# Team766/ros_vision

Measured on AMD Instinct MI355X. Metric: frames/sec + p50 per-frame latency, 1280x720 AprilTag detect at 1/2/4/8 MI355X, higher is better.
Workload: dtype u8

## Files before the change

ros_vision_amd/csrc/at_api.cpp:

```cpp
#include <hip/hip_runtime.h>

#include <algorithm>
#include <chrono>
#include <cmath>
#include <cstdio>
#include <cstdlib>
#include <cstring>
#include <map>
#include <string>
#include <thread>
#include <vector>

#include "../../include/at_api.h"
#include "at_common.h"
#include "at_gp.h"
#include "at_mjpg.h"
#include "at_mjpg_entropy.h"
#include "at_preview.h"
#include "at_rigcal.h"
#include "at_camcal.h"

namespace at {
hipError_t launch_tap_sizes(const uint8_t* thr, const uint32_t* par, const uint32_t* size, uint32_t* out, int Wd,
                            int Hd, hipStream_t st);
// ... 184 lines not shown
  int mj_ent_timed;
  at::JpgBufs jpg;
  size_t jpg_out_cap;
  uint32_t* h_jpg_total;
  uint8_t jpg_hdr[at::kJpgHeaderMax];
  size_t jpg_hdr_len;
  int jpg_hdr_q, jpg_hdr_s, jpg_hdr_w, jpg_hdr_h;
  uint64_t jpg_stats[2];
  hipEvent_t ev_jpg[2];
  at::GpParseBufs gp;
  at::GpBox* h_gp_out;
  uint32_t* h_gp_info;
  uint64_t gp_stats[4];
  hipEvent_t ev_gp[2];
  uint8_t* d_pv;
  uint64_t pv_stats[6];
  hipEvent_t ev_pv[2];
  FieldLaunch field;
  int field_on;
  int last_field;
  int field_timed;
  FpRecord* h_field;
  hipEvent_t ev_field[2];
  uint64_t field_ns;
};

static const char* knob(const char* name) {
#ifdef AT_EXPERIMENTS
  return getenv(name);
#else
  (void)name;
  return nullptr;
#endif
}
static int knob_int(const char* name, int dflt) {
  const char* v = knob(name);
  return v ? atoi(v) : dflt;
}

static int hip_fail(hipError_t e) {
  if (e != hipSuccess) {
    fprintf(stderr, "at_api: HIP error %s\n", hipGetErrorString(e));
    return AT_E_HIP;
  }
  return AT_OK;
}
#define HIPCHK(x)                          \
  do {                                     \
    hipError_t e_ = (x);                   \
    if (e_ != hipSuccess) return hip_fail(e_); \
  } while (0)

extern "C" {

int at_abi_version(void) { return AT_ABI_VERSION; }

const char* at_strerror(int code) {
  switch (code) {
    case AT_OK: return "ok";
    case AT_E_INVALID: return "invalid argument or unsupported frame geometry";
    case AT_E_HIP: return "HIP runtime error";
    case AT_E_CAPACITY: return "frame exceeded a fixed capacity";
    case AT_E_FAMILY: return "unknown tag family";
    case AT_E_NOMEM: return "out of memory";
    case AT_E_UNSUPPORTED: return "unsupported JPEG stream (not baseline 8-bit 4:4:4 / 4:2:2 / 4:2:0 / gray)";
    default: return "unknown error";
  }
}

int at_family_num_known(const char* family) {
  const FamilyInfo* f = find_family(family);
  return f ? f->ncodes : AT_E_FAMILY;
}

int at_family_entry(const char* family, int i, int* id, uint64_t* code) {
  const FamilyInfo* f = find_family(family);
  if (!f) return AT_E_FAMILY;
  if (i < 0 || i >= f->ncodes) return AT_E_INVALID;
  if (id) *id = f->codes[i].id;
  if (code) *code = f->codes[i].code;
  return AT_OK;
}

int at_config_default(at_config* cfg, int width, int height) {
  if (!cfg) return AT_E_INVALID;
  memset(cfg, 0, sizeof(*cfg));
  cfg->width = width;
  cfg->height = height;
  cfg->family = "tag36h11";
  cfg->quad_decimate = 2.0f;
  cfg->refine_edges = 1;
  cfg->decode_sharpening = 0.25;
  cfg->min_white_black_diff = 5;
  cfg->min_cluster_pixels = 5;
  cfg->max_nmaxima = 10;
  cfg->max_line_fit_mse = 10.0f;
  cfg->cos_critical_rad = cos(10.0 * M_PI / 180.0);
  cfg->device = 0;
  cfg->max_batch = 1;
  cfg->tag_size = 0.1651;
  return AT_OK;
}

void at_destroy(at_detector* d) {
  if (!d) return;
  (void)hipSetDevice(d->device);
  if (d->st) (void)hipStreamSynchronize(d->st);
  if (d->st2) (void)hipStreamSynchronize(d->st2);
  for (auto& kv : d->graphs) (void)hipGraphExecDestroy(kv.second);
  d->graphs.clear();
  for (auto& kv : d->split_graphs)
    for (auto* g : kv.second.seg) (void)hipGraphExecDestroy(g);
  d->split_graphs.clear();
  for (void* p : d->allocs) (void)hipFree(p);
  if (d->h_ftab) (void)hipHostFree(d->h_ftab);
  if (d->h_ctrl) (void)hipHostFree(d->h_ctrl);
  if (d->h_dets) (void)hipHostFree(d->h_dets);
  if (d->d_prims) (void)hipFree(d->d_prims);
  if (d->d_last) (void)hipFree(d->d_last);
  for (uint8_t* p : d->mj_host)
    if (p) (void)hipHostFree(p);
  for (hipEvent_t e : d->ev_mj)
    if (e) (void)hipEventDestroy(e);
  for (uint8_t* p : d->mj_ent_host)
    if (p) (void)hipHostFree(p);
  if (d->h_ent_info) (void)hipHostFree(d->h_ent_info);
  for (hipEvent_t e : d->ev_ent)
    if (e) (void)hipEventDestroy(e);
  for (hipEvent_t e : d->ev_jpg)
    if (e) (void)hipEventDestroy(e);
  if (d->h_jpg_total) (void)hipHostFree(d->h_jpg_total);
  for (hipEvent_t e : d->ev_gp)
    if (e) (void)hipEventDestroy(e);
  for (hipEvent_t e : d->ev_pv)
    if (e) (void)hipEventDestroy(e);
  if (d->d_pv) (void)hipFree(d->d_pv);
  for (hipEvent_t e : d->ev_field)
    if (e) (void)hipEventDestroy(e);
  if (d->h_field) (void)hipHostFree(d->h_field);
  if (d->h_gp_out) (void)hipHostFree(d->h_gp_out);
  if (d->h_gp_info) (void)hipHostFree(d->h_gp_info);
  if (d->ev_done) (void)hipEventDestroy(d->ev_done);
  if (d->ev_ext) (void)hipEventDestroy(d->ev_ext);
  for (int i = 0; i <= kNumStages; i++)
    if (d->ev_stage[i]) (void)hipEventDestroy(d->ev_stage[i]);
  if (d->kt.t0) (void)hipEventDestroy(d->kt.t0);
  if (d->kt.t1) (void)hipEventDestroy(d->kt.t1);
  if (d->ev_fork) (void)hipEventDestroy(d->ev_fork);
  if (d->ev_join) (void)hipEventDestroy(d->ev_join);
  if (d->st2) (void)hipStreamDestroy(d->st2);
  if (d->st) (void)hipStreamDestroy(d->st);
  delete d;
}

int at_create(const at_config* cfg, const at_camera* cam, at_detector** out) {
  if (!cfg || !cam || !out) return AT_E_INVALID;
  *out = nullptr;
  const FamilyInfo* fam = find_family(cfg->family);
  if (!fam || fam->ncodes > kMaxCodes) return AT_E_FAMILY;
  const int W = cfg->width, H = cfg->height;
  if (W <= 16 || H <= 16 || W % 8 || H % 8 || (long)W * H >= (1L << 22)) return AT_E_INVALID;
  if (cfg->quad_decimate != 2.0f || cfg->max_nmaxima != 10 || cfg->max_batch < 1 || cfg->max_batch > kMaxBatch)
    return AT_E_INVALID;
  if (2 * (W + H) > kSortCap) return AT_E_INVALID;
  int ndev = 0;
  if (hipGetDeviceCount(&ndev) != hipSuccess || ndev <= cfg->device) return AT_E_HIP;
  at_detector* d = new at_detector();
  d->cfg = *cfg;
  d->cfg.family = fam->name;
  d->cam = *cam;
  d->device = cfg->device;
  d->B = cfg->max_batch;
  d->mj_threads = 1;
  d->mj_subseq = at::kEntSubseqDefault;
  Geom& g = d->g;
  g.W = W; g.H = H; g.Wd = W / 2; g.Hd = H / 2;
  g.TW = g.Wd / 4; g.TH = g.Hd / 4;
  g.BW = g.Wd / 2; g.BH = g.Hd / 2;
  g.ctw = d->B < kWideBlobMaxBatch ? 32 : 64;
  if (knob("AT_CCL_TILE")) g.ctw = knob_int("AT_CCL_TILE", 64) == 32 ? 32 : 64;
  g.nlarge = g.ctw == 32 ? std::max(kNumLargeCls, std::min(kNumCls, knob_int("AT_NLARGE", kNumLargeCls)))
                        : kNumLargeCls;
  g.CTX = (g.Wd + g.ctw - 1) / g.ctw;
  g.CTY = (g.Hd + kCclTileH - 1) / kCclTileH;
  g.merge_cap = g.ctw == 64 ? std::min(kMergeCapMax, 80 * g.CTX * g.CTY) : 0;
  g.merge_lds = std::min(g.merge_cap * 12 + 8192, kMergeLdsMax);
  if (g.CTX * g.CTY > kMaxCclTiles) {
    at_destroy(d);
    return AT_E_INVALID;
  }
  g.cap_pts = 4 * (g.Wd - 2) * (g.Hd - 2);
  g.BTX = (g.Wd - 2 + 63) / 64;
  g.BTY = (g.Hd - 2 + 4 * kBndRows - 1) / (4 * kBndRows);
  g.ntb = g.BTX * g.BTY;
  g.bnd_region = kBndPts;
  g.bnd_region = std::max(kBndStage, std::min(kBndPts, knob_int("AT_BND_REGION", kBndPts)));
  if (g.ntb > kMaxTilesPerFrame) {
    at_destroy(d);
    return AT_E_INVALID;
  }
  g.min_cluster = (uint32_t)std::max(24, cfg->min_cluster_pixels);
  g.max_cluster = (uint32_t)(2 * (W + H));
  g.min_tag_width = std::max(3, (fam->d + 2) / 2);
  Params& p = d->prm;
  p.min_white_black_diff = cfg->min_white_black_diff;
  p.max_line_fit_mse = cfg->max_line_fit_mse;
  p.cos_critical_rad = cfg->cos_critical_rad;
  p.decode_sharpening = cfg->decode_sharpening;
  p.refine_edges = cfg->refine_edges;
  p.fx = cam->fx; p.fy = cam->fy; p.cx = cam->cx; p.cy = cam->cy;
  p.k1 = cam->k1; p.k2 = cam->k2; p.p1 = cam->p1; p.p2 = cam->p2; p.k3 = cam->k3;
  p.diag_stop = knob_int("AT_DIAG_BLOB_STOP", 0);
  p.probe = knob_int("AT_PHASE_PROBE", 0);
  p.taps = 0;
  p.wide_blob = knob_int("AT_WIDE_BLOB", 0);
  p.pipe_stop = knob_int("AT_DIAG_PIPE_STOP", 0);
  p.lblob_wg = knob("AT_LBLOB_WG") ? std::max(16, knob_int("AT_LBLOB_WG", 0)) : 0;
  p.sblob_wg = knob("AT_SBLOB_WG") ? std::max(16, knob_int("AT_SBLOB_WG", 0)) : 0;
  p.dec_wg = knob("AT_DEC_WG") ? std::max(16, knob_int("AT_DEC_WG", 0)) : 0;
  p.dec_lpq = knob_int("AT_DEC_LPQ", 0) == 64 ? 64 : 0;
  p.fam = family_desc(*fam);
  d->use_graphs = !knob_int("AT_NO_GRAPH", 0);
  if (!(cfg->tag_size >= 0) || !std::isfinite(cfg->tag_size)) {
    at_destroy(d);
    return AT_E_INVALID;
  }
  p.tag_size = cfg->tag_size;

  auto fail = [&](int code) {
    at_destroy(d);
    return code;
  };
  if (hipSetDevice(d->device) != hipSuccess) return fail(AT_E_HIP);
  if (hipStreamCreateWithFlags(&d->st, hipStreamNonBlocking) != hipSuccess) return fail(AT_E_HIP);
  if (hipEventCreateWithFlags(&d->ev_done, hipEventDisableTiming) != hipSuccess) return fail(AT_E_HIP);
  if (hipEventCreateWithFlags(&d->ev_ext, hipEventDisableTiming) != hipSuccess) return fail(AT_E_HIP);
  const bool fork = d->B < kWideBlobMaxBatch && !knob_int("AT_NO_FORK", 0);
  if (fork && hipStreamCreateWithFlags(&d->st2, hipStreamNonBlocking) != hipSuccess) return fail(AT_E_HIP);
  if (hipEventCreateWithFlags(&d->ev_fork, hipEventDisableTiming) != hipSuccess) return fail(AT_E_HIP);
  if (hipEventCreateWithFlags(&d->ev_join, hipEventDisableTiming) != hipSuccess) return fail(AT_E_HIP);
  d->kt.stage = -1;
  d->kt.split = nullptr;
  d->kt.ctx = nullptr;
  if (hipEventCreateWithFlags(&d->kt.t0, kTimingEventFlags) != hipSuccess ||
      hipEventCreateWithFlags(&d->kt.t1, kTimingEventFlags) != hipSuccess)
    return fail(AT_E_HIP);
  int ncu = 0;
  (void)hipDeviceGetAttribute(&ncu, hipDeviceAttributeMultiprocessorCount, d->device);
  int wclk = 0;
  (void)hipDeviceGetAttribute(&wclk, hipDeviceAttributeWallClockRate, d->device);
  d->wclk_khz = wclk > 0 ? (double)wclk : 100000.0;
  d->nblobwg = std::max(64, ncu * 2);
  if (knob("AT_BLOB_WG")) d->nblobwg = std::max(16, knob_int("AT_BLOB_WG", 0));

  const size_t B = (size_t)d->B;
  const size_t npix = (size_t)W * H, nd = (size_t)g.Wd * g.Hd, nt = (size_t)g.TW * g.TH * 2;
  bool oom = false;
  auto dalloc = [&](size_t bytes) -> void* {
    void* ptr = nullptr;
    if (hipMalloc(&ptr, std::max<size_t>(bytes, 256)) != hipSuccess) {
      oom = true;
      return nullptr;
    }
    d->allocs.push_back(ptr);
    return ptr;
  };
  d->in_stride = (npix * 3 + 255) & ~(size_t)255;
  d->d_in = (uint8_t*)dalloc(B * d->in_stride);
  DevBufs& b = d->d;
  b.gray = (uint8_t*)dalloc(B * npix);
  b.dec = (uint8_t*)dalloc(B * nd);
  b.mm = (uint8_t*)dalloc(B * nt);
  b.thr = (uint8_t*)dalloc(B * nd);
  b.par = (uint32_t*)dalloc(B * nd * 4);
  b.lroot = (uint32_t*)dalloc(B * (size_t)g.CTX * g.CTY * kCclTileNodesMax * 4);
  b.nlroot = (uint32_t*)dalloc(B * (size_t)g.CTX * g.CTY * 4);
  b.lcnt = (uint32_t*)dalloc(B * (size_t)g.CTX * g.CTY * kCclTileNodesMax * 4);
  b.cdesc = (uint32_t*)dalloc(B * (size_t)g.CTX * g.CTY * CclDesc::kWords * 4);
  b.size = (uint32_t*)dalloc(B * nd * 4);
  const size_t ntb = (size_t)g.ntb;
  b.pts = (uint64_t*)dalloc(B * ntb * (size_t)g.bnd_region * 8);
  b.tcnt = (uint32_t*)dalloc(B * ntb * 4);
  b.tent = (uint32_t*)dalloc(B * ntb * 4);
  b.grp = (uint32_t*)dalloc(B * g.cap_pts * 4);
  b.keys = (uint64_t*)dalloc(B * g.cap_pts * 8);
  b.pent_key = (uint64_t*)dalloc(B * ntb * kLdsPairSlots * 8);
  b.pent_cnt = (uint32_t*)dalloc(B * ntb * kLdsPairSlots * 4);
  b.povf_key = (uint64_t*)dalloc(B * kPairEntCap * 8);
  b.povf_cnt = (uint32_t*)dalloc(B * kPairEntCap * 4);
  b.ht_key = (uint64_t*)dalloc(B * kHashSlots * 8);
  b.ht_cnt = (uint32_t*)dalloc(B * kHashSlots * 4);
  b.ht_rank = (uint32_t*)dalloc(B * kHashSlots * 4);
  b.ht_off = (uint32_t*)dalloc(B * kHashSlots * 4);
  b.ht_cur = (uint32_t*)dalloc(B * kHashSlots * 4);
  b.pair_cnt = (uint32_t*)dalloc(B * kMaxPairs * 4);
  b.pair_off = (uint32_t*)dalloc(B * kMaxPairs * 4);
  b.pair_sel = (uint32_t*)dalloc(B * kMaxPairs * 4);
  b.wcap = (uint32_t)(B * kMaxPairs);
  b.work = (uint32_t*)dalloc((size_t)kNumCls * B * kMaxPairs * 4);
  b.probe = (uint64_t*)dalloc(kProbeWords * 8);
  b.dets = (DevDetection*)dalloc(B * kMaxDets * sizeof(DevDetection));
  b.det_work = (uint32_t*)dalloc(B * kMaxDets * 4);
  b.quads = (QuadRecord*)dalloc(B * kMaxPairs * sizeof(QuadRecord));
  b.qpend = (QuadPend*)dalloc(B * kMaxPairs * sizeof(QuadPend));
  d->kstamp_word = (kCtlPerFrame * B + kCtlScalars + 1) & ~(size_t)1;
  d->ctrl_words = d->kstamp_word + 5;
  d->d_ctrl = (uint32_t*)dalloc(((d->ctrl_words * 4 + 15) / 16) * 16);
  b.npts = d->d_ctrl + kCtlNpts * B;
  b.npairs = d->d_ctrl + kCtlNpairs * B;
  b.ndets = d->d_ctrl + kCtlNdets * B;
  b.nquads = d->d_ctrl + kCtlNquads * B;
  b.status = d->d_ctrl + kCtlStatus * B;
  b.npent = d->d_ctrl + kCtlNpent * B;
  b.qc_words = (uint32_t)(B * kQcStride);
  b.nqcand = (uint32_t*)dalloc((size_t)b.qc_words * 4);
  b.ccl_ovf = d->d_ctrl + kCtlCclOvf * B;
  b.nlr_tot = d->d_ctrl + kCtlNlr * B;
  uint32_t* sc = d->d_ctrl + kCtlPerFrame * B;
  b.workhead = sc + kCtlWorkhead;
  b.qhead = sc + kCtlQhead;
  b.workhead_small = sc + kCtlWorkheadSmall;
  b.workhead_mid = sc + kCtlWorkheadMid;
  b.blob_pts = sc + kCtlBlobPts;
  b.ncls = sc + kCtlNcls;
  b.det_head = sc + kCtlDetHead;
  b.dec_done = sc + kCtlDecDone;
  b.kt_stage = -1;
  b.kstamp = reinterpret_cast<uint64_t*>(d->d_ctrl + d->kstamp_word);
  b.kgrid = d->d_ctrl + d->kstamp_word + 4;
  b.kwg_cap = (uint32_t)(B * 1024 + 4096);
  b.kwg = (uint64_t*)dalloc((size_t)b.kwg_cap * 2 * 8);
  b.qcand_cap = (uint32_t)(B * kQuadCandPerFrame);
  b.qcand = (QuadCand*)dalloc((size_t)b.qcand_cap * sizeof(QuadCand));
  b.s_pk = (uint64_t*)dalloc((size_t)2 * d->nblobwg * (kSortCap / 2) * 8);
  b.rsamp = (double*)dalloc(decode_scratch_doubles(d->nblobwg, d->B, g.ctw == 64) * 8);
  if (oom) return fail(AT_E_NOMEM);
  if (prepare_kernels(g) != hipSuccess) return fail(AT_E_HIP);
  if (hipHostMalloc((void**)&d->h_ftab, B * sizeof(void*), hipHostMallocMapped | hipHostMallocCoherent) != hipSuccess)
    return fail(AT_E_NOMEM);
  if (hipHostGetDevicePointer((void**)&b.frames, (void*)d->h_ftab, 0) != hipSuccess) return fail(AT_E_HIP);
  d->res_idx.assign(B * kMaxDets, 0);
  d->res_n.assign(B, 0);
  d->res_base.assign(B, nullptr);
  d->res_ovf.resize(B);
  if (hipHostMalloc((void**)&d->h_ctrl, d->ctrl_words * 4, hipHostMallocMapped) != hipSuccess) return fail(AT_E_NOMEM);
  if (hipHostMalloc((void**)&d->h_dets, B * kDetPoolPerFrame * sizeof(DevDetection), hipHostMallocMapped) != hipSuccess)
    return fail(AT_E_NOMEM);
  if (hipHostGetDevicePointer((void**)&b.hdets, d->h_dets, 0) != hipSuccess ||
      hipHostGetDevicePointer((void**)&b.hctrl, d->h_ctrl, 0) != hipSuccess)
    return fail(AT_E_HIP);
  b.ctrl = d->d_ctrl;
  b.ctrl_words = (uint32_t)d->ctrl_words;
  {
    std::vector<uint64_t> codes(fam->ncodes);
    std::vector<int32_t> ids(fam->ncodes);
    for (int i = 0; i < fam->ncodes; i++) {
      codes[i] = fam->codes[i].code;
      ids[i] = fam->codes[i].id;
    }
    uint64_t* dc = (uint64_t*)dalloc(codes.size() * 8);
    int32_t* di = (int32_t*)dalloc(ids.size() * 4);
    if (oom) return fail(AT_E_NOMEM);
    if (hipMemcpy(dc, codes.data(), codes.size() * 8, hipMemcpyHostToDevice) != hipSuccess ||
        hipMemcpy(di, ids.data(), ids.size() * 4, hipMemcpyHostToDevice) != hipSuccess)
      return fail(AT_E_HIP);
    b.book_code = dc;
    b.book_id = di;
  }
  if (hipMemsetAsync(b.size, 0, B * nd * 4, d->st) != hipSuccess) return fail(AT_E_HIP);
  if (hipStreamSynchronize(d->st) != hipSuccess) return fail(AT_E_HIP);
  *out = d;
  return AT_OK;
}

}

static bool seg_intersect(const double* a0, const double* a1, const double* b0, const double* b1) {
  const double ux = a1[0] - a0[0], uy = a1[1] - a0[1];
  const double vx = b1[0] - b0[0], vy = b1[1] - b0[1];
  const double den = ux * vy - uy * vx;
  if (fabs(den) < 1e-12) return false;
  const double t = ((b0[0] - a0[0]) * vy - (b0[1] - a0[1]) * vx) / den;
  const double w = ((b0[0] - a0[0]) * uy - (b0[1] - a0[1]) * ux) / den;
  return t >= 0 && t <= 1 && w >= 0 && w <= 1;
}
static bool poly_contains(const double poly[4][2], const double* pt) {
  bool inside = false;
  for (int i = 0, j = 3; i < 4; j = i++) {
    if (((poly[i][1] > pt[1]) != (poly[j][1] > pt[1])) &&
        (pt[0] < (poly[j][0] - poly[i][0]) * (pt[1] - poly[i][1]) / (poly[j][1] - poly[i][1]) + poly[i][0]))
      inside = !inside;
  }
  return inside;
}
static bool poly_overlap(const double a[4][2], const double b[4][2]) {
  for (int i = 0; i < 4; i++)
    for (int j = 0; j < 4; j++)
      if (seg_intersect(a[i], a[(i + 1) & 3], b[j], b[(j + 1) & 3])) return true;
  return poly_contains(a, b[0]) || poly_contains(b, a[0]);
}
static int prefer_smaller(int pref, double q0, double q1) {
  if (pref) return pref;
  if (q0 < q1) return -1;
  if (q1 < q0) return 1;
  return 0;
}

static void write_detection(const DevDetection& v, at_detection* o) {
  o->id = v.id;
  o->hamming = v.hamming;
  o->decision_margin = v.decision_margin;
  memcpy(o->H, v.H, sizeof(o->H));
  memcpy(o->c, v.c, sizeof(o->c));
  memcpy(o->p, v.p, sizeof(o->p));
}

static int host_tail(const DevDetection* cand, int* idx, int ncand, at_detection* out, int cap) {
  std::stable_sort(idx, idx + ncand, [&](int a, int b) { return cand[a].blob_rank < cand[b].blob_rank; });
  int n = ncand;
  for (int i0 = 0; i0 < n; i0++) {
    for (int i1 = i0 + 1; i1 < n; i1++) {
      const DevDetection& a = cand[idx[i0]];
      const DevDetection& b = cand[idx[i1]];
      if (a.id != b.id) continue;
      if (!poly_overlap(a.p, b.p)) continue;
      int pref = 0;
      pref = prefer_smaller(pref, a.hamming, b.hamming);
      pref = prefer_smaller(pref, -a.decision_margin, -b.decision_margin);
      for (int k = 0; k < 3; k++) pref = prefer_smaller(pref, a.H[k], b.H[k]);
      if (pref < 0) {
        if (i1 < n - 1) idx[i1] = idx[n - 1];
        n--;
        i1--;
      } else {
        if (i0 < n - 1) idx[i0] = idx[n - 1];
        n--;
        i0--;
        break;
      }
    }
  }
  std::stable_sort(idx, idx + n, [&](int a, int b) { return cand[a].id < cand[b].id; });
  for (int i = 0; i < n && i < cap; i++) write_detection(cand[idx[i]], out + i);
  return n;
}

static hipError_t record_sequence(at_detector* d, int nframes, int fmt, hipStream_t st, hipEvent_t* ev,
                                  const KernelTimer* kt) {
  hipError_t e;
  DevBufs b = d->d;
  b.kt_stage = kt ? kt->stage : -1;
  FieldLaunch fl = d->field;
  fl.ev[0] = ev ? d->ev_field[0] : nullptr;
  fl.ev[1] = ev ? d->ev_field[1] : nullptr;
  if ((e = launch_pipeline(b, d->g, d->prm, nframes, fmt, d->nblobwg, st, ev, d->st2, d->ev_fork, d->ev_join, kt,
                           d->field_on ? &fl : nullptr)))
    return e;
  if (d->prm.tag_size > 0) return hipSuccess;
  return hipMemcpyAsync(d->h_ctrl, d->d_ctrl, d->ctrl_words * 4, hipMemcpyDeviceToHost, st);
}

static hipError_t split_capture(void* ctx, int ) {
  at_detector* d = (at_detector*)ctx;
  hipGraph_t g = nullptr;
  hipError_t e = hipStreamEndCapture(d->st, &g);
  if (e != hipSuccess) return e;
  d->cap_segs.push_back(g);
  return hipStreamBeginCapture(d->st, hipStreamCaptureModeThreadLocal);
}

static hipError_t instantiate(hipGraph_t g, hipGraphExec_t* exec) {
  const hipError_t e = hipGraphInstantiate(exec, g, nullptr, nullptr, 0);
  (void)hipGraphDestroy(g);
  return e;
}

static int enqueue_split(at_detector* d, int nframes, int fmt) {
  hipStream_t st = d->st;
  const int key = (nframes * 4 + fmt) * 32 + d->kt.stage;
  auto it = d->split_graphs.find(key);
  if (it == d->split_graphs.end()) {
    d->cap_segs.clear();
    KernelTimer kt = d->kt;
    kt.split = split_capture;
    kt.ctx = d;
    HIPCHK(hipStreamBeginCapture(st, hipStreamCaptureModeThreadLocal));
    hipError_t rec = record_sequence(d, nframes, fmt, st, nullptr, &kt);
    hipGraph_t last = nullptr;
    const hipError_t end = hipStreamEndCapture(st, &last);
    if (last) d->cap_segs.push_back(last);
    if (rec == hipSuccess && end == hipSuccess && d->cap_segs.size() != 3) rec = hipErrorInvalidValue;
    if (rec != hipSuccess || end != hipSuccess) {
      for (auto* g : d->cap_segs) (void)hipGraphDestroy(g);
      d->cap_segs.clear();
      HIPCHK(rec);
      HIPCHK(end);
    }
    at_detector::SplitGraphs sg{};
    hipError_t inst = hipSuccess;
    for (int i = 0; i < 3; i++) {
      const hipError_t r = instantiate(d->cap_segs[i], &sg.seg[i]);
      if (r != hipSuccess && inst == hipSuccess) inst = r;
    }
    d->cap_segs.clear();
    if (inst != hipSuccess) {
      for (auto* g : sg.seg)
        if (g) (void)hipGraphExecDestroy(g);
      HIPCHK(inst);
    }
    it = d->split_graphs.emplace(key, sg).first;
  }
  HIPCHK(hipGraphLaunch(it->second.seg[0], st));
  HIPCHK(hipEventRecord(d->kt.t0, st));
  HIPCHK(hipGraphLaunch(it->second.seg[1], st));
  HIPCHK(hipEventRecord(d->kt.t1, st));
  HIPCHK(hipGraphLaunch(it->second.seg[2], st));
  return AT_OK;
}

static int enqueue(at_detector* d, int nframes, int fmt) {
  hipStream_t st = d->st;
  const bool timed = d->kt.stage >= 0;
  const bool timed_on_fork = timed && d->st2 && (d->kt.stage == 8 || d->kt.stage == 9);
  if (d->profiling || !d->use_graphs || timed_on_fork) {
    HIPCHK(record_sequence(d, nframes, fmt, st, d->profiling ? d->ev_stage : nullptr, timed ? &d->kt : nullptr));
  } else if (timed) {
    const int rc = enqueue_split(d, nframes, fmt);
    if (rc != AT_OK) return rc;
  } else {
    const int key = nframes * 4 + fmt;
    auto it = d->graphs.find(key);
    if (it == d->graphs.end()) {
      hipGraph_t graph = nullptr;
      HIPCHK(hipStreamBeginCapture(st, hipStreamCaptureModeThreadLocal));
      const hipError_t rec = record_sequence(d, nframes, fmt, st, nullptr, nullptr);
      const hipError_t end = hipStreamEndCapture(st, &graph);
      HIPCHK(rec);
      HIPCHK(end);
      hipGraphExec_t exec = nullptr;
      HIPCHK(instantiate(graph, &exec));
      it = d->graphs.emplace(key, exec).first;
    }
    HIPCHK(hipGraphLaunch(it->second, st));
  }
  HIPCHK(hipEventRecord(d->ev_done, st));
  d->last_nframes = nframes;
  d->last_fmt = fmt;
  d->last_gray = fmt == AT_FMT_BGR8 || d->prm.taps;
  d->last_sizes = d->g.ctw == 32 || d->prm.taps;
  d->last_gp = d->prm.gp_c && fmt == AT_FMT_BGR8;
  d->last_mj_color = 0;
  d->mj_ent_batch = 0;
  d->last_field = d->field_on && d->prm.tag_size > 0;
  d->field_timed = d->last_field && d->profiling;
  d->pending = 1;
  return AT_OK;
}

static double now_us() {
  return std::chrono::duration<double, std::micro>(std::chrono::steady_clock::now().time_since_epoch()).count();
}

static int collect(at_detector* d, at_detection* out, int cap_per_frame, int* n_per_frame) {
  if (!d->pending) return AT_E_INVALID;
  const double t0 = now_us();
  HIPCHK(hipEventSynchronize(d->ev_done));
  const double t1 = now_us();
  d->host_wait_us += t1 - t0;
  d->pending = 0;
  if (d->profiling) {
    for (int i = 0; i < kNumStages; i++) {
      float ms = 0;
      HIPCHK(hipEventElapsedTime(&ms, d->ev_stage[i], d->ev_stage[i + 1]));
      d->stage_ms[i] += ms;
    }
    d->stage_batches++;
  }
  if (d->mj_timed) {
    float ms = 0;
    HIPCHK(hipEventElapsedTime(&ms, d->ev_mj[0], d->ev_mj[1]));
    d->mj_stats[4] = (uint64_t)((double)ms * 1e6);
    if (d->mj_timed == 2) {
      HIPCHK(hipEventElapsedTime(&ms, d->ev_mj[1], d->ev_mj[2]));
      d->mj_stats[5] = (uint64_t)((double)ms * 1e6);
    }
    d->mj_timed = 0;
  }
  d->field_ns = 0;
  if (d->field_timed) {
    float ms = 0;
    HIPCHK(hipEventElapsedTime(&ms, d->ev_field[0], d->ev_field[1]));
    d->field_ns = (uint64_t)((double)ms * 1e6);
    d->field_timed = 0;
  }
  if (d->mj_ent_timed) {
    float ms = 0;
    HIPCHK(hipEventElapsedTime(&ms, d->ev_ent[0], d->ev_ent[1]));
    d->mj_stats[6] = (uint64_t)((double)ms * 1e6);
    d->mj_ent_timed = 0;
  }
  if (d->mj_ent_batch) {
    uint32_t most = 0;
    for (int f = 0; f < d->last_nframes; f++) most = std::max(most, d->h_ent_info[(size_t)f * at::kEntInfoWords + 1]);
    d->mj_stats[8] = most;
  }
  if (d->kt.stage >= 0) {
    float ms = 0;
// ... 1811 lines not shown
```

ros_vision_amd/csrc/at_common.h:

```cpp
#pragma once

#include <hip/hip_runtime.h>
#include <stdint.h>

#include "at_detmath.h"
#include "at_fieldpose.h"
#include "at_rigpose.h"
#include "at_preview.h"

namespace at {

template <int TW>
struct CclTile {
  static constexpr int W = TW, H = 32;
  static constexpr int BW = TW / 2, BH = H / 2;
  static constexpr int NT = BW * BH;
  static constexpr int NODES = 3 * NT;
  static constexpr int ROW_NODES = 3 * BW;
};
constexpr int kCclTileH = 32;
constexpr int kCclTileNodesMax = CclTile<64>::NODES;
constexpr int kHashSlots = 4096;
constexpr int kHashBits = 12;
constexpr int kPairEntCap = 65536;
constexpr int kBndRows = 4;
constexpr int kBndPts = 64 * 4 * kBndRows * 4;
constexpr int kBndStage = 2048;
constexpr int kLdsPairSlots = 512;
constexpr uint32_t kTileNarrow = 0x80000000u;
constexpr int kMaxTilesPerFrame = 1024;
constexpr int kMaxCclTiles = 1024;
struct CclDesc {
  static constexpr int Tthr = 0, Bthr = 16, Lthr = 32, Rthr = 40;
  static constexpr int TsF = 48, TsL = 64, TsR = 80, BsF = 96, BsL = 112, BsR = 128;
  static constexpr int LsF = 144, LsL = 152, RsF = 160, RsR = 168;
  static constexpr int kWords = 176;
};
constexpr int kMergeCapMax = 15360;
constexpr int kMergeLdsMax = kMergeCapMax * 10;
constexpr int kMaxPairs = 4096;
constexpr int kSortCap = 8192;
constexpr int kBlobThreads = 256;
constexpr int kWideBlobMaxBatch = 8;
constexpr int kSmallBlob = 512;
constexpr int kNMaxima = 10;
constexpr int kMaxRefineSamples = 1536;
#ifndef AT_LDS_REFINE
#define AT_LDS_REFINE 256
#endif
constexpr int kLdsRefine = AT_LDS_REFINE;
constexpr int kDecodeGridPerBlobWg = 8;
inline int decode_grid(int nblobwg, int B) {
  const int hi = nblobwg * kDecodeGridPerBlobWg, want = 64 * B;
  return nblobwg * 2 > (want < hi ? want : hi) ? nblobwg * 2 : (want < hi ? want : hi);
}
constexpr int kDecRowLanes = 16;
constexpr int kRowRefine = 64;
inline size_t decode_scratch_doubles(int nblobwg, int B, bool packed) {
  const size_t one = 2 * (size_t)(kMaxRefineSamples - kLdsRefine);
  const size_t rows = (64 / kDecRowLanes) * 2 * (size_t)(kMaxRefineSamples - kRowRefine);
  return (size_t)decode_grid(nblobwg, B) * (packed && rows > one ? rows : one);
}

constexpr int kNumStages = 12;
constexpr const char* kStageNames[kNumStages] = {"k_pre",   "k_thr_ccl", "k_ccl_merge", "k_ccl_roots",
                                                 "k_boundary", "k_pairs", "k_group",     "k_extents",
                                                 "k_blob_small", "k_blob", "k_decode",   "k_pose"};

constexpr int kNumCls = 7;
constexpr int kNumLargeCls = 3;

constexpr uint32_t kStatusPairsOverflow = 1u;
constexpr uint32_t kStatusHashFull = 2u;
constexpr uint32_t kStatusDetsOverflow = 4u;
constexpr uint32_t kStatusPointsOverflow = 8u;
constexpr uint32_t kStatusQuadsOverflow = 16u;
constexpr uint32_t kStatusPairsCapped = 32u;
constexpr int kMaxBatch = 256;
constexpr int kQcStride = 32;
constexpr int kQuadCandPerFrame = kMaxPairs;
constexpr int kMaxDets = kQuadCandPerFrame;
constexpr int kDetPoolPerFrame = 128;
constexpr int kMaxCodes = 1024;
constexpr int kMaxFamilyBits = 64;

struct FamilyDesc {
  int nbits;
  int width_at_border;
  int total_width;
  int reversed_border;
  int ncodes;
  int8_t bitx[kMaxFamilyBits], bity[kMaxFamilyBits];
};

struct Geom {
  int W, H, Wd, Hd;
  int TW, TH;
  int BW, BH;
  int CTX, CTY;
  int ctw;
  int merge_cap;
  int merge_lds;
  int nlarge;
  int bnd_region;
  int cap_pts;
  int BTX, BTY, ntb;
  uint32_t min_cluster;
  uint32_t max_cluster;
  int min_tag_width;
};

struct Params {
  int min_white_black_diff;
  float max_line_fit_mse;
  double cos_critical_rad;
  double decode_sharpening;
  int refine_edges;
  double fx, fy, cx, cy, k1, k2, p1, p2, k3;
  int diag_stop;
  double tag_size;
  int probe;
  int taps;
  int wide_blob;
  int pipe_stop;
  int lblob_wg;
  int sblob_wg;
  int dec_wg;
  int dec_lpq;
  FamilyDesc fam;
  int gp_w, gp_h, gp_c;
};
constexpr int kProbeWords = 256;

#ifdef AT_EXPERIMENTS
#define AT_DIAG_STOP(prm, n) ((prm).diag_stop == (n))
#define AT_PIPE_STOP(prm) ((prm).pipe_stop)
#define AT_PROBE_ON(prm) ((prm).probe != 0)
#define AT_DIAG_ANY(prm) ((prm).diag_stop != 0)
#else
#define AT_DIAG_STOP(prm, n) false
#define AT_PIPE_STOP(prm) 0
#define AT_PROBE_ON(prm) false
#define AT_DIAG_ANY(prm) false
#endif

struct KernelTimer {
  int stage;
  hipEvent_t t0, t1;
  hipError_t (*split)(void* ctx, int which);
  void* ctx;
};

struct DevDetection {
  int32_t id;
  int16_t hamming;
  uint16_t frame;
  float decision_margin;
  int32_t blob_rank;
  double H[9];
  double c[2];
  double p[4][2];
  double pose_R[9];
  double pose_t[3];
  double pose_err[2];
};

struct QuadCand {
  uint32_t frame, rank;
  float p[4][2];
};

struct QuadRecord {
  uint32_t blob_index, valid, accepted;
  uint16_t indices[4];
  float corners[4][2];
};

struct Moments {
  int32_t Mx, My, W;
  int64_t Mxx, Myy, Mxy;
  int32_t N;
};

struct QuadPend {
  float fit[4][4];
  uint32_t blob_index, valid;
  uint16_t indices[4];
};
static_assert(sizeof(QuadPend) == 80, "QuadPend: 80 B per kept blob");


struct JpgBufs {
  int16_t* coef;
  const uint32_t* tab;
  uint32_t* blen;
  uint32_t* bits;
  size_t row_words;
  uint32_t* row_raw;
  uint32_t* row_len;
  uint8_t* out;
  uint32_t* total;
};

struct FieldBufs {
  FpLayout lay;
  FpRecord* out;
  FpRecord* hout;
};
struct FieldLaunch {
  FieldBufs b;
  hipEvent_t ev[2];
};

struct RigCamView {
  const DevDetection* dets;
  const uint32_t* ndets;
  RigCam cam;
};
struct RigBufs {
  RigCamView view[kRigMaxCams];
  FpLayout lay;
  RigRecord* out;
  RigRecord* hout;
  double tag_size;
  int n_cams;
};

struct DevBufs {
  const uint8_t* const* frames;
  uint8_t* gray;
  uint8_t* dec;
  uint8_t* mm;
  uint8_t* thr;
  uint32_t* par;
  uint32_t* lroot;
  uint32_t* nlroot;
  uint32_t* lcnt;
  uint32_t* cdesc;
  uint32_t* ccl_ovf;
  uint32_t* nlr_tot;
  uint32_t* size;
  uint64_t* pts;
  uint32_t* tcnt;
  uint32_t* tent;
  uint32_t* grp;
  uint64_t* keys;
  uint64_t* pent_key;
  uint32_t* pent_cnt;
  uint64_t* povf_key;
  uint32_t* povf_cnt;
  uint32_t* npent;
  uint64_t* ht_key;
  uint32_t* ht_cnt;
  uint32_t* ht_rank;
  uint32_t* ht_off;
  uint32_t* ht_cur;
  uint32_t* pair_cnt;
  uint32_t* pair_off;
  uint32_t* pair_sel;
  uint32_t* work;
  uint32_t wcap;
  DevDetection* dets;
  uint32_t* det_work;
  uint32_t* det_head;
  uint32_t* dec_done;
  DevDetection* hdets;
  uint32_t* hctrl;
  uint32_t* ctrl;
  uint32_t ctrl_words;
  QuadRecord* quads;
  QuadPend* qpend;
  uint32_t* npts;
  uint32_t* npairs;
  uint32_t* ndets;
  uint32_t* nquads;
  uint32_t* status;
  uint32_t* ncls;
  uint32_t* workhead;
  uint64_t* probe;
  uint32_t* blob_pts;
  uint32_t* workhead_small;
  uint32_t* workhead_mid;
  uint32_t* nqcand;
  uint32_t qc_words;
  uint32_t* qhead;
  QuadCand* qcand;
  uint32_t qcand_cap;
  double* rsamp;
  const uint64_t* book_code;
  const int32_t* book_id;
  float* gp_out;
  int32_t kt_stage;
  uint64_t* kstamp;
  uint32_t* kgrid;
  uint64_t* kwg;
  uint32_t kwg_cap;
  uint64_t* s_pk;
};

}
```

ros_vision_amd/csrc/at_kernels.hip:

```cpp
#include <limits>
#include <hip/hip_runtime.h>

#include <float.h>
#include <math.h>
#include <stdint.h>

#include "at_common.h"
#include "at_gp.h"
#include "at_mjpg.h"
#include "at_mjpg_entropy.h"
#include "at_pose.h"
#include "at_rigcal.h"
#include "at_camcal.h"


namespace at {

__device__ __forceinline__ uint32_t lane_id() { return __lane_id(); }
__device__ __attribute__((noinline)) float det_atan2f_call(float y, float x) { return det_atan2f(y, x); }

__device__ __forceinline__ uint64_t mix_hash(uint64_t k) {
  return (k * 0x9E3779B97F4A7C15ull) >> (64 - kHashBits);
}

__device__ __forceinline__ int dx_of(int dxy) { return dxy == 3 ? -1 : (dxy == 2 ? 0 : 1); }
__device__ __forceinline__ int dy_of(int dxy) { return dxy == 0 ? 0 : 1; }

template <int CTRL, int ROW_MASK, typename T>
__device__ __forceinline__ T dpp_move(T v, T old) {
  static_assert(sizeof(T) == 4 || sizeof(T) == 8, "dpp_move: 32- or 64-bit values");
  if constexpr (sizeof(T) == 4) {
    return __builtin_bit_cast(T, __builtin_amdgcn_update_dpp(__builtin_bit_cast(int, old), __builtin_bit_cast(int, v),
                                                             CTRL, ROW_MASK, 0xf, false));
  } else {
    const uint64_t u = __builtin_bit_cast(uint64_t, v), o = __builtin_bit_cast(uint64_t, old);
    const uint32_t lo = (uint32_t)__builtin_amdgcn_update_dpp((int)(uint32_t)o, (int)(uint32_t)u, CTRL, ROW_MASK, 0xf, false);
    const uint32_t hi = (uint32_t)__builtin_amdgcn_update_dpp((int)(uint32_t)(o >> 32), (int)(uint32_t)(u >> 32), CTRL,
                                                              ROW_MASK, 0xf, false);
    return __builtin_bit_cast(T, (uint64_t)lo | ((uint64_t)hi << 32));
  }
}

template <typename T, typename Op>
__device__ __forceinline__ T wave_incl_scan(T x, Op op, T id) {
  x = op(x, dpp_move<0x111, 0xf>(x, id));
  x = op(x, dpp_move<0x112, 0xf>(x, id));
  x = op(x, dpp_move<0x114, 0xf>(x, id));
  x = op(x, dpp_move<0x118, 0xf>(x, id));
  x = op(x, dpp_move<0x142, 0xa>(x, id));
  x = op(x, dpp_move<0x143, 0xc>(x, id));
  return x;
}

__device__ __forceinline__ uint32_t wave_shr1(uint32_t v, uint32_t fill) {
  return (uint32_t)__builtin_amdgcn_update_dpp((int)fill, (int)v, 0x138, 0xf, 0xf, false);
}

__device__ __forceinline__ uint32_t lanes_below(uint64_t mask) {
  return __builtin_amdgcn_mbcnt_hi((uint32_t)(mask >> 32), __builtin_amdgcn_mbcnt_lo((uint32_t)mask, 0u));
}

__device__ __forceinline__ void wave_sync() {
  __builtin_amdgcn_fence(__ATOMIC_RELEASE, "wavefront");
  __builtin_amdgcn_wave_barrier();
  __builtin_amdgcn_fence(__ATOMIC_ACQUIRE, "wavefront");
}

__device__ __forceinline__ uint32_t wave_read_next(uint32_t v) {
  return (uint32_t)__builtin_amdgcn_update_dpp(0, (int)v, 0x130, 0xf, 0xf, false);
}

template <typename T>
__device__ __forceinline__ T wave_read(T v, int l) {
  if constexpr (sizeof(T) == 4) {
    return __builtin_bit_cast(T, __builtin_amdgcn_readlane(__builtin_bit_cast(int, v), l));
  } else {
    const uint64_t u = __builtin_bit_cast(uint64_t, v);
    const uint32_t lo = (uint32_t)__builtin_amdgcn_readlane((int)(uint32_t)u, l);
    const uint32_t hi = (uint32_t)__builtin_amdgcn_readlane((int)(uint32_t)(u >> 32), l);
    return __builtin_bit_cast(T, (uint64_t)lo | ((uint64_t)hi << 32));
  }
}

struct MinOp {
  template <typename T> __device__ T operator()(T a, T c) const { return a < c ? a : c; }
  template <typename T> __device__ static T identity() { return std::numeric_limits<T>::max(); }
};
struct MaxOp {
  template <typename T> __device__ T operator()(T a, T c) const { return a > c ? a : c; }
  template <typename T> __device__ static T identity() { return std::numeric_limits<T>::lowest(); }
};
struct AddOp {
  template <typename T> __device__ T operator()(T a, T c) const { return a + c; }
  template <typename T> __device__ static T identity() { return T(0); }
};

__device__ __forceinline__ uint32_t run_len(uint64_t same_mask, uint32_t lane) {
  if (lane == 63) return 1;
  const uint64_t rest = ~(same_mask >> (lane + 1));
  return 1 + (uint32_t)__builtin_ctzll(rest);
}

template <typename T, typename Op>
__device__ T wave_reduce(T v, Op op) {
  return wave_read(wave_incl_scan(v, op, Op::template identity<T>()), 63);
}

template <typename T, typename Op>
__device__ T block_reduce(T v, Op op, T* s_tmp , int NW) {
  v = wave_reduce(v, op);
  const int w = threadIdx.x >> 6;
  __syncthreads();
  if (lane_id() == 0) s_tmp[w] = v;
  __syncthreads();
  T r = s_tmp[0];
  for (int i = 1; i < NW; i++) r = op(r, s_tmp[i]);
  return r;
}

template <typename T>
__device__ T block_incl_scan(T v, T* s_tmp, T* total, int NW) {
  const uint32_t lane = lane_id();
  v = wave_incl_scan(v, AddOp(), T(0));
  const int w = threadIdx.x >> 6;
  __syncthreads();
  if (lane == 63) s_tmp[w] = v;
  __syncthreads();
  T base = 0, tot = 0;
  for (int i = 0; i < NW; i++) {
    if (i < w) base = base + s_tmp[i];
    tot = tot + s_tmp[i];
  }
  *total = tot;
  return base + v;
}


#ifndef AT_XCD_PRE
#define AT_XCD_PRE 1
#endif
#ifndef AT_XCD_THR
#define AT_XCD_THR 1
#endif
#ifndef AT_XCD_BND
#define AT_XCD_BND 0
#endif
#ifndef AT_XCD_GRP
#define AT_XCD_GRP 0
#endif
struct TileIdx {
  int x, y, z;
};
__device__ __forceinline__ uint32_t udiv24(uint32_t a, uint32_t d) {
  uint32_t q = (uint32_t)((float)a * __builtin_amdgcn_rcpf((float)d));
  int32_t r = (int32_t)(a - q * d);
#pragma unroll
  for (int k = 0; k < 2; k++) {
    if (r < 0) { q--; r += (int32_t)d; }
    if (r >= (int32_t)d) { q++; r -= (int32_t)d; }
  }
  return q;
}
template <int MODE>
__device__ __forceinline__ TileIdx xcd_block() {
  if constexpr (MODE == 0) return TileIdx{(int)blockIdx.x, (int)blockIdx.y, (int)blockIdx.z};
  const uint32_t gx = gridDim.x, gxy = gridDim.x * gridDim.y, n = gxy * gridDim.z;
  const uint32_t lid = blockIdx.x + gx * blockIdx.y + gxy * blockIdx.z;
  uint32_t t;
  if constexpr (MODE == 1) {
    const uint32_t q = n >> 3, r = n & 7, xcd = lid & 7;
    t = xcd * q + min(xcd, r) + (lid >> 3);
  } else {
    const uint32_t rows = gridDim.y * gridDim.z, n8 = (rows & ~7u) * gx;
    if (lid < n8) {
      const uint32_t k = lid >> 3, j = udiv24(k, gx);
      t = ((j << 3) + (lid & 7)) * gx + (k - j * gx);
    } else {
      t = lid;
    }
  }
  const uint32_t z = udiv24(t, gxy), rem = t - z * gxy, y = udiv24(rem, gx);
  return TileIdx{(int)(rem - y * gx), (int)y, (int)z};
}

__device__ __forceinline__ uint32_t kt_wg_id() {
  return blockIdx.x + gridDim.x * (blockIdx.y + gridDim.y * blockIdx.z);
}
__device__ __forceinline__ void kt_begin(const DevBufs& b, int stage) {
  if (b.kt_stage != stage || threadIdx.x != 0 || threadIdx.y != 0) return;
  const uint32_t id = kt_wg_id();
  if (id == 0) *b.kgrid = gridDim.x * gridDim.y * gridDim.z;
  if (id < b.kwg_cap) b.kwg[id] = wall_clock64();
}
__device__ __forceinline__ void kt_end(const DevBufs& b, int stage) {
  if (b.kt_stage != stage) return;
  const uint32_t id = kt_wg_id();
  if (id < b.kwg_cap) b.kwg[b.kwg_cap + id] = wall_clock64();
}
constexpr int kKtSpanWgs = 32;
__global__ __launch_bounds__(256) void k_kt_span(DevBufs b) {
  const uint32_t n = min(*b.kgrid, b.kwg_cap);
  uint64_t mn = ~0ull, mx = 0;
  for (uint32_t i = blockIdx.x * 256 + threadIdx.x; i < n; i += kKtSpanWgs * 256) {
    mn = min(mn, b.kwg[i]);
    mx = max(mx, b.kwg[b.kwg_cap + i]);
  }
  mn = wave_reduce(mn, MinOp());
  mx = wave_reduce(mx, MaxOp());
  if (lane_id() == 0 && mx) {
    atomicMax((unsigned long long*)&b.kstamp[0], (unsigned long long)~mn);
    atomicMax((unsigned long long*)&b.kstamp[1], (unsigned long long)mx);
  }
}

__constant__ float c_filter[7] = {0.01110899634659290314f, 0.13533528149127960205f, 0.60653066635131835938f,
                                  1.00000000000000000000f, 0.60653066635131835938f, 0.13533528149127960205f,
                                  0.01110899634659290314f};

template <int FMT>
__device__ __forceinline__ void load_y8(const uint8_t* in, int W, int row, int x, uint32_t (&y)[8]) {
  if (FMT == 0) {
    const uint4 v = *reinterpret_cast<const uint4*>(in + ((size_t)row * W + x) * 2);
    const uint32_t w[4] = {v.x, v.y, v.z, v.w};
#pragma unroll
    for (int k = 0; k < 4; k++) {
      y[2 * k] = w[k] & 0xff;
      y[2 * k + 1] = (w[k] >> 16) & 0xff;
    }
  } else if (FMT == 1) {
    const uint8_t* p = in + ((size_t)row * W + x) * 3;
    const uint2 v0 = *reinterpret_cast<const uint2*>(p);
    const uint2 v1 = *reinterpret_cast<const uint2*>(p + 8);
    const uint2 v2 = *reinterpret_cast<const uint2*>(p + 16);
    uint8_t bytes[24];
    *reinterpret_cast<uint2*>(bytes) = v0;
    *reinterpret_cast<uint2*>(bytes + 8) = v1;
    *reinterpret_cast<uint2*>(bytes + 16) = v2;
#pragma unroll
    for (int k = 0; k < 8; k++) {
      const int bb = bytes[3 * k], gg = bytes[3 * k + 1], rr = bytes[3 * k + 2];
      y[k] = (uint32_t)((269484 * rr + 528482 * gg + 102760 * bb + (1 << 19) + (16 << 20)) >> 20);
    }
  } else {
    const uint2 v = *reinterpret_cast<const uint2*>(in + (size_t)row * W + x);
#pragma unroll
    for (int k = 0; k < 4; k++) {
      y[k] = (v.x >> (8 * k)) & 0xff;
      y[4 + k] = (v.y >> (8 * k)) & 0xff;
    }
  }
}

template <int FMT>
__global__ __launch_bounds__(256) void k_pre(DevBufs b, Geom g, int wgray) {
  const TileIdx bi = xcd_block<AT_XCD_PRE>();
  const int f = bi.z;
  const int tx = bi.x * 64 + threadIdx.x;
  const int ty = bi.y * 4 + threadIdx.y;
  if (blockIdx.x == 0 && blockIdx.y == 0 && blockIdx.z == 0) {
    for (uint32_t w = threadIdx.y * 64 + threadIdx.x; w < b.ctrl_words; w += 256) b.ctrl[w] = 0;
    for (uint32_t w = threadIdx.y * 64 + threadIdx.x; w < b.qc_words; w += 256) b.nqcand[w] = 0;
  }
  if (tx >= g.TW || ty >= g.TH) return;
  const uint8_t* in = b.frames[f];
  uint8_t* gray = b.gray + (size_t)f * g.W * g.H;
  uint8_t* dec = b.dec + (size_t)f * g.Wd * g.Hd;
  uint32_t mn = 255, mx = 0;
  const int x0 = tx * 8;
#pragma unroll
  for (int r = 0; r < 8; r++) {
    const int row = ty * 8 + r;
    uint32_t y[8];
    load_y8<FMT>(in, g.W, row, x0, y);
    if (FMT == 1 || wgray) {
      uint2 gw;
      gw.x = y[0] | (y[1] << 8) | (y[2] << 16) | (y[3] << 24);
      gw.y = y[4] | (y[5] << 8) | (y[6] << 16) | (y[7] << 24);
      *reinterpret_cast<uint2*>(gray + (size_t)row * g.W + x0) = gw;
    }
    if ((r & 1) == 0) {
      const uint32_t d = y[0] | (y[2] << 8) | (y[4] << 16) | (y[6] << 24);
      *reinterpret_cast<uint32_t*>(dec + (size_t)(row >> 1) * g.Wd + (x0 >> 1)) = d;
#pragma unroll
      for (int k = 0; k < 8; k += 2) {
        mn = min(mn, y[k]);
        mx = max(mx, y[k]);
      }
    }
  }
  uint8_t* mm = b.mm + (size_t)f * g.TW * g.TH * 2;
  *reinterpret_cast<uint16_t*>(mm + 2 * ((size_t)ty * g.TW + tx)) = (uint16_t)(mn | (mx << 8));
}

__device__ __forceinline__ uint32_t node_F(const Geom& g, int BY, int BX) { return (uint32_t)(BY * 3 * g.BW + BX); }
__device__ __forceinline__ uint32_t node_L(const Geom& g, int BY, int BX) {
  return (uint32_t)(BY * 3 * g.BW + g.BW + 2 * BX);
}
__device__ __forceinline__ uint32_t node_pixel(int BW, int Wd, uint32_t n) {
  const uint32_t by = n / (uint32_t)(3 * BW), r = n - by * (uint32_t)(3 * BW);
  return r < (uint32_t)BW ? 2 * by * (uint32_t)Wd + 2 * r : (2 * by + 1) * (uint32_t)Wd + (r - (uint32_t)BW);
}

__device__ __forceinline__ uint32_t lds_load(uint32_t* p) {
  return __hip_atomic_load(p, __ATOMIC_RELAXED, __HIP_MEMORY_SCOPE_WORKGROUP);
}
__device__ __forceinline__ uint32_t lds_find(uint32_t* par, uint32_t n) {
  uint32_t p = lds_load(par + n);
  while (p != n) {
    const uint32_t gp = lds_load(par + p);
    if (gp != p) atomicMin(&par[n], gp);
    n = p;
    p = gp;
  }
  return n;
}

__device__ __forceinline__ void lds_union(uint32_t* par, uint32_t a, uint32_t b) {
  while (true) {
    a = lds_find(par, a);
    b = lds_find(par, b);
    if (a == b) return;
    if (a < b) {
      const uint32_t old = atomicMin(&par[b], a);
      if (old == b) return;
      b = old;
    } else {
      const uint32_t old = atomicMin(&par[a], b);
      if (old == a) return;
      a = old;
    }
  }
}

template <int TW>
__device__ __forceinline__ uint32_t slot_of(int ty, int tx, int type) {
  using T = CclTile<TW>;
  return (uint32_t)(ty * T::ROW_NODES + (type == 0 ? tx : T::BW + 2 * tx + (type - 1)));
}

template <int TW>
struct BorderRoles {
  static constexpr int Top = 5 * CclTile<TW>::BW, Left = 3 * CclTile<TW>::BH, Right = CclTile<TW>::BH - 1;
  static constexpr int NT = (Top + Left + Right + 63) / 64 * 64;
};

constexpr uint32_t kKeptBit = 0x80000000u;
constexpr uint32_t kListBit = 0x40000000u;
constexpr uint32_t kTouchBit = 0x80000000u;

#ifndef AT_THR_SGPRS
#define AT_THR_SGPRS 80
#endif
template <int TWD, int PRE>
__device__ __forceinline__ void thr_ccl_tile(const DevBufs& b, const Geom& g, const Params& prm, const TileIdx bi) {
  using CT = CclTile<TWD>;
  constexpr int NT = CT::NT;
  constexpr int kCclTileW = CT::W, kCclBW = CT::BW, kCclTileNodes = CT::NODES;
  constexpr int kTW = kCclTileW / 4, kTH = kCclTileH / 4;
  constexpr int kHR = kCclTileH + 1, kHC = kCclTileW + 2;
  const int f = bi.z;
  const int tid = threadIdx.x;
  const int y0 = bi.y * kCclTileH, x0 = bi.x * kCclTileW;
  const uint8_t* dec = b.dec + (size_t)f * g.Wd * g.Hd;
  const uint8_t* mm = b.mm + (size_t)f * g.TW * g.TH * 2;
  uint8_t* thr = b.thr + (size_t)f * g.Wd * g.Hd;

  __shared__ uint8_t s_umn[kTH + 3][kTW + 4], s_umx[kTH + 3][kTW + 4];
  __shared__ uint8_t s_fmn[kTH + 1][kTW + 2], s_fmx[kTH + 1][kTW + 2];
  __shared__ __attribute__((aligned(4))) uint8_t s_t[kHR][kHC + 2];
  __shared__ uint32_t s_par[kCclTileNodes];
  __shared__ uint32_t s_cnt[kCclTileNodes];
  __shared__ uint32_t s_nlr;
// ... 1748 lines not shown
}


__device__ void redistort(const Params& p, double* x, double* y) {
  const double xP = (*x - p.cx) / p.fx, yP = (*y - p.cy) / p.fy;
  const double rSq = xP * xP + yP * yP;
  const double lin = 1 + p.k1 * rSq + p.k2 * rSq * rSq + p.k3 * rSq * rSq * rSq;
  const double xPP = xP * lin + 2 * p.p1 * xP * yP + p.p2 * (rSq + 2 * xP * xP);
  const double yPP = yP * lin + p.p1 * (rSq + 2 * yP * yP) + 2 * p.p2 * xP * yP;
  *x = xPP * p.fx + p.cx;
  *y = yPP * p.fy + p.cy;
}

__device__ void undistort(const Params& p, double* u, double* v) {
  const double xPP = (*u - p.cx) / p.fx, yPP = (*v - p.cy) / p.fy;
  double xP = xPP, yP = yPP;
  const double x0 = xP, y0 = yP;
  double prev_x, prev_y;
  int it = 0;
  do {
    prev_x = xP;
    prev_y = yP;
    const double rSq = xP * xP + yP * yP;
    const double rad = 1 + (p.k1 * rSq) + (p.k2 * rSq * rSq) + (p.k3 * rSq * rSq * rSq);
    const double rinv = 1 / rad;
    const double tdx = 2 * p.p1 * xP * yP + p.p2 * (rSq + p.k3 * rSq * rSq * rSq);
    const double tdy = p.p1 * (rSq + 2 * yP * yP) + 2 * p.p2 * xP * yP;
    xP = (x0 - tdx) * rinv;
    yP = (y0 - tdy) * rinv;
    if (it > 100) break;
    it++;
  } while (fabs(xP - prev_x) > 1e-6 || fabs(yP - prev_y) > 1e-6);
  *u = xP * p.fx + p.cx;
  *v = yP * p.fy + p.cy;
}

__device__ void hproject(const double* H, double x, double y, double* ox, double* oy) {
  const double xx = H[0] * x + H[1] * y + H[2];
  const double yy = H[3] * x + H[4] * y + H[5];
  const double zz = H[6] * x + H[7] * y + H[8];
  *ox = xx / zz;
  *oy = yy / zz;
}

__device__ int homography_wave(const float (*qc)[2], double* A, double* H) {
  const int lane = (int)lane_id();
  for (int e = lane; e < 72; e += 64) {
    const int row = e / 9, col = e % 9, i = row >> 1;
    const double c0 = (i == 0 || i == 3) ? -1 : 1, c1 = (i == 0 || i == 1) ? -1 : 1;
    const double c2 = qc[i][0], c3 = qc[i][1];
    const int k = (row & 1) ? col - 3 : col;
    const double cz = (row & 1) ? c3 : c2;
    double v = 0;
    if (k == 0) v = c0;
    else if (k == 1) v = c1;
    else if (k == 2) v = 1;
    if (col == 6) v = -c0 * cz;
    else if (col == 7) v = -c1 * cz;
    else if (col == 8) v = cz;
    A[e] = v;
  }
  team_sync<64>();
  for (int col = 0; col < 8; col++) {
    double v = -1.0;
    int row = 64;
    if (lane < 8 - col) {
      row = col + lane;
      v = fabs(A[row * 9 + col]);
      if (!(v > 0.0)) { v = -1.0; row = 64; }
    }
#pragma unroll
    for (int d = 1; d < 8; d <<= 1) {
      const double ov = __shfl_xor(v, d);
      const int orow = __shfl_xor(row, d);
      if (ov > v || (ov == v && orow < row)) { v = ov; row = orow; }
    }
    v = __shfl(v, 0);
    row = __shfl(row, 0);
    if (!(v >= 1e-10)) return -1;
    if (row != col && lane <= 8 - col) {
      const int i = col + lane;
      const double t = A[col * 9 + i];
      A[col * 9 + i] = A[row * 9 + i];
      A[row * 9 + i] = t;
    }
    team_sync<64>();
    const int nc = 8 - col;
    if (lane < (7 - col) * nc) {
      const int i = col + 1 + lane / nc, j = col + 1 + lane % nc;
      const double fct = A[i * 9 + col] / A[col * 9 + col];
      A[i * 9 + j] -= fct * A[col * 9 + j];
    }
    team_sync<64>();
  }
  double x[8];
#pragma unroll
  for (int col = 7; col >= 0; col--) {
    double sum = 0;
#pragma unroll
    for (int i = col + 1; i < 8; i++) sum += A[col * 9 + i] * x[i];
    x[col] = (A[col * 9 + 8] - sum) / A[col * 9 + col];
  }
#pragma unroll
  for (int k = 0; k < 8; k++)
    if (lane == k) H[k] = x[k];
  if (lane == 8) H[8] = 1;
  team_sync<64>();
  return 0;
}

template <int LPQ>
__device__ bool homography_rows(bool live, int rl, const float (*qc)[2], double* A, double* H) {
  static_assert(LPQ >= 16 && 64 % LPQ == 0, "a row holds the 9 lanes of a swap and of H");
  if (live) {
    for (int e = rl; e < 72; e += LPQ) {
      const int row = e / 9, col = e % 9, i = row >> 1;
      const double c0 = (i == 0 || i == 3) ? -1 : 1, c1 = (i == 0 || i == 1) ? -1 : 1;
      const double c2 = qc[i][0], c3 = qc[i][1];
      const int k = (row & 1) ? col - 3 : col;
      const double cz = (row & 1) ? c3 : c2;
      double v = 0;
      if (k == 0) v = c0;
      else if (k == 1) v = c1;
      else if (k == 2) v = 1;
      if (col == 6) v = -c0 * cz;
      else if (col == 7) v = -c1 * cz;
      else if (col == 8) v = cz;
      A[e] = v;
    }
  }
  team_sync<64>();
  for (int col = 0; col < 8; col++) {
    double v = -1.0;
    int row = 64;
    if (live && rl < 8 - col) {
      row = col + rl;
      v = fabs(A[row * 9 + col]);
      if (!(v > 0.0)) { v = -1.0; row = 64; }
    }
#pragma unroll
    for (int d = 1; d < 8; d <<= 1) {
      const double ov = __shfl_xor(v, d);
      const int orow = __shfl_xor(row, d);
      if (ov > v || (ov == v && orow < row)) { v = ov; row = orow; }
    }
    v = __shfl(v, 0, LPQ);
    row = __shfl(row, 0, LPQ);
    if (!(v >= 1e-10)) live = false;
    if (live && row != col && rl <= 8 - col) {
      const int i = col + rl;
      const double t = A[col * 9 + i];
      A[col * 9 + i] = A[row * 9 + i];
      A[row * 9 + i] = t;
    }
    team_sync<64>();
    if (live && (rl >> 1) < 7 - col) {
      const int i = col + 1 + (rl >> 1);
      const double fct = A[i * 9 + col] / A[col * 9 + col];
#pragma unroll
      for (int q = 0; q < 4; q++) {
        const int j = col + 1 + 4 * (rl & 1) + q;
        if (j <= 8) A[i * 9 + j] -= fct * A[col * 9 + j];
      }
    }
    team_sync<64>();
  }
  double x[8];
#pragma unroll
  for (int col = 7; col >= 0; col--) {
    double sum = 0;
#pragma unroll
    for (int i = col + 1; i < 8; i++) sum += A[col * 9 + i] * x[i];
    x[col] = (A[col * 9 + 8] - sum) / A[col * 9 + col];
  }
  if (live) {
#pragma unroll
    for (int k = 0; k < 8; k++)
      if (rl == k) H[k] = x[k];
    if (rl == 8) H[8] = 1;
  }
  team_sync<64>();
  return live;
}

struct GrayModel {
  double A[3][3], B[3], C[3];
};
__device__ void gm_add(GrayModel& g, double x, double y, double gray) {
  g.A[0][0] += x * x; g.A[0][1] += x * y; g.A[0][2] += x;
  g.A[1][1] += y * y; g.A[1][2] += y; g.A[2][2] += 1;
  g.B[0] += x * gray; g.B[1] += y * gray; g.B[2] += gray;
}
__device__ void gm_solve(GrayModel& g) {
  const double* A = &g.A[0][0];
  double L[9], M[9];
  L[0] = sqrt(A[0]); L[3] = A[1] / L[0]; L[6] = A[2] / L[0];
  L[4] = sqrt(A[4] - L[3] * L[3]); L[7] = (A[5] - L[3] * L[6]) / L[4];
  L[8] = sqrt(A[8] - L[6] * L[6] - L[7] * L[7]);
  M[0] = 1 / L[0]; M[3] = -L[3] * M[0] / L[4]; M[4] = 1 / L[4];
  M[6] = (-L[6] * M[0] - L[7] * M[3]) / L[8]; M[7] = -L[7] * M[4] / L[8]; M[8] = 1 / L[8];
  const double t0 = M[0] * g.B[0];
  const double t1 = M[3] * g.B[0] + M[4] * g.B[1];
  const double t2 = M[6] * g.B[0] + M[7] * g.B[1] + M[8] * g.B[2];
  g.C[0] = M[0] * t0 + M[3] * t1 + M[6] * t2;
  g.C[1] = M[4] * t1 + M[7] * t2;
  g.C[2] = M[8] * t2;
}
__device__ __forceinline__ double gm_interp(const GrayModel& g, double x, double y) {
  return g.C[0] * x + g.C[1] * y + g.C[2];
}

__constant__ uint8_t c_combo[210][4] = {{0,1,2,3},{0,1,2,4},{0,1,2,5},{0,1,2,6},{0,1,2,7},{0,1,2,8},{0,1,2,9},{0,1,3,4},{0,1,3,5},{0,1,3,6},{0,1,3,7},{0,1,3,8},{0,1,3,9},{0,1,4,5},{0,1,4,6},{0,1,4,7},{0,1,4,8},{0,1,4,9},{0,1,5,6},{0,1,5,7},{0,1,5,8},{0,1,5,9},{0,1,6,7},{0,1,6,8},{0,1,6,9},{0,1,7,8},{0,1,7,9},{0,1,8,9},{0,2,3,4},{0,2,3,5},{0,2,3,6},{0,2,3,7},{0,2,3,8},{0,2,3,9},{0,2,4,5},{0,2,4,6},{0,2,4,7},{0,2,4,8},{0,2,4,9},{0,2,5,6},{0,2,5,7},{0,2,5,8},{0,2,5,9},{0,2,6,7},{0,2,6,8},{0,2,6,9},{0,2,7,8},{0,2,7,9},{0,2,8,9},{0,3,4,5},{0,3,4,6},{0,3,4,7},{0,3,4,8},{0,3,4,9},{0,3,5,6},{0,3,5,7},{0,3,5,8},{0,3,5,9},{0,3,6,7},{0,3,6,8},{0,3,6,9},{0,3,7,8},{0,3,7,9},{0,3,8,9},{0,4,5,6},{0,4,5,7},{0,4,5,8},{0,4,5,9},{0,4,6,7},{0,4,6,8},{0,4,6,9},{0,4,7,8},{0,4,7,9},{0,4,8,9},{0,5,6,7},{0,5,6,8},{0,5,6,9},{0,5,7,8},{0,5,7,9},{0,5,8,9},{0,6,7,8},{0,6,7,9},{0,6,8,9},{0,7,8,9},{1,2,3,4},{1,2,3,5},{1,2,3,6},{1,2,3,7},{1,2,3,8},{1,2,3,9},{1,2,4,5},{1,2,4,6},{1,2,4,7},{1,2,4,8},{1,2,4,9},{1,2,5,6},{1,2,5,7},{1,2,5,8},{1,2,5,9},{1,2,6,7},{1,2,6,8},{1,2,6,9},{1,2,7,8},{1,2,7,9},{1,2,8,9},{1,3,4,5},{1,3,4,6},{1,3,4,7},{1,3,4,8},{1,3,4,9},{1,3,5,6},{1,3,5,7},{1,3,5,8},{1,3,5,9},{1,3,6,7},{1,3,6,8},{1,3,6,9},{1,3,7,8},{1,3,7,9},{1,3,8,9},{1,4,5,6},{1,4,5,7},{1,4,5,8},{1,4,5,9},{1,4,6,7},{1,4,6,8},{1,4,6,9},{1,4,7,8},{1,4,7,9},{1,4,8,9},{1,5,6,7},{1,5,6,8},{1,5,6,9},{1,5,7,8},{1,5,7,9},{1,5,8,9},{1,6,7,8},{1,6,7,9},{1,6,8,9},{1,7,8,9},{2,3,4,5},{2,3,4,6},{2,3,4,7},{2,3,4,8},{2,3,4,9},{2,3,5,6},{2,3,5,7},{2,3,5,8},{2,3,5,9},{2,3,6,7},{2,3,6,8},{2,3,6,9},{2,3,7,8},{2,3,7,9},{2,3,8,9},{2,4,5,6},{2,4,5,7},{2,4,5,8},{2,4,5,9},{2,4,6,7},{2,4,6,8},{2,4,6,9},{2,4,7,8},{2,4,7,9},{2,4,8,9},{2,5,6,7},{2,5,6,8},{2,5,6,9},{2,5,7,8},{2,5,7,9},{2,5,8,9},{2,6,7,8},{2,6,7,9},{2,6,8,9},{2,7,8,9},{3,4,5,6},{3,4,5,7},{3,4,5,8},{3,4,5,9},{3,4,6,7},{3,4,6,8},{3,4,6,9},{3,4,7,8},{3,4,7,9},{3,4,8,9},{3,5,6,7},{3,5,6,8},{3,5,6,9},{3,5,7,8},{3,5,7,9},{3,5,8,9},{3,6,7,8},{3,6,7,9},{3,6,8,9},{3,7,8,9},{4,5,6,7},{4,5,6,8},{4,5,6,9},{4,5,7,8},{4,5,7,9},{4,5,8,9},{4,6,7,8},{4,6,7,9},{4,6,8,9},{4,7,8,9},{5,6,7,8},{5,6,7,9},{5,6,8,9},{5,7,8,9},{6,7,8,9}};

__constant__ uint8_t c_colex[210] = {0,1,7,28,84,2,8,29,85,13,34,90,49,105,140,3,9,30,86,14,35,91,50,106,141,18,39,95,54,110,145,64,120,155,175,4,10,31,87,15,36,92,51,107,142,19,40,96,55,111,146,65,121,156,176,22,43,99,58,114,149,68,124,159,179,74,130,165,185,195,5,11,32,88,16,37,93,52,108,143,20,41,97,56,112,147,66,122,157,177,23,44,100,59,115,150,69,125,160,180,75,131,166,186,196,25,46,102,61,117,152,71,127,162,182,77,133,168,188,198,80,136,171,191,201,205,6,12,33,89,17,38,94,53,109,144,21,42,98,57,113,148,67,123,158,178,24,45,101,60,116,151,70,126,161,181,76,132,167,187,197,26,47,103,62,118,153,72,128,163,183,78,134,169,189,199,81,137,172,192,202,206,27,48,104,63,119,154,73,129,164,184,79,135,170,190,200,82,138,173,193,203,207,83,139,174,194,204,208,209};

struct LineFitOut {
  double err, mse;
  double p01[2], p23[2];
};

template <bool kP01, bool kP23>
__device__ __forceinline__ LineFitOut fit_line_v(const Moments& m) {
  LineFitOut o;
  fit_line(m, kP01 ? o.p01 : nullptr, kP23 ? o.p23 : nullptr, &o.err, &o.mse);
  return o;
}

struct Mom6 {
  uint32_t Mx, My, W;
  uint64_t Mxx, Myy, Mxy;
};
__device__ __forceinline__ Mom6 mom_zero() { return Mom6{0, 0, 0, 0, 0, 0}; }
__device__ __forceinline__ void mom_add(Mom6& a, const Mom6& c) {
  a.Mx += c.Mx; a.My += c.My; a.W += c.W; a.Mxx += c.Mxx; a.Myy += c.Myy; a.Mxy += c.Mxy;
}
__device__ __forceinline__ void mom_sub(Mom6& a, const Mom6& c) {
  a.Mx -= c.Mx; a.My -= c.My; a.W -= c.W; a.Mxx -= c.Mxx; a.Myy -= c.Myy; a.Mxy -= c.Mxy;
}
__device__ __forceinline__ Mom6 mom_shfl(const Mom6& m, int src) {
  Mom6 r;
  r.Mx = __shfl(m.Mx, src); r.My = __shfl(m.My, src); r.W = __shfl(m.W, src);
  r.Mxx = __shfl(m.Mxx, src); r.Myy = __shfl(m.Myy, src); r.Mxy = __shfl(m.Mxy, src);
  return r;
}
__device__ __forceinline__ Mom6 mom_shfl_up(const Mom6& m, int d) {
  Mom6 r;
  r.Mx = __shfl_up(m.Mx, d); r.My = __shfl_up(m.My, d); r.W = __shfl_up(m.W, d);
  r.Mxx = __shfl_up(m.Mxx, d); r.Myy = __shfl_up(m.Myy, d); r.Mxy = __shfl_up(m.Mxy, d);
  return r;
}

constexpr int kKeyTheta = 32;

__device__ __forceinline__ uint32_t compact_word(uint64_t sk) {
  return (uint32_t)((sk >> 10) & 0x3ff) | ((uint32_t)((sk >> 20) & 0x3ff) << 10) | ((uint32_t)((sk >> 30) & 3) << 20) |
         ((uint32_t)(sk & 0x1ff) << 22);
}

__device__ __forceinline__ Mom6 point_mom(uint32_t cw) {
  const int dxy = (int)((cw >> 20) & 3);
  const uint32_t ix2 = (cw & 0x3ff) * 2 + dx_of(dxy) + 1;
  const uint32_t iy2 = ((cw >> 10) & 0x3ff) * 2 + dy_of(dxy) + 1;
  const uint32_t Wt = cw >> 22;
  Mom6 m;
  m.Mx = Wt * ix2;
  m.My = Wt * iy2;
  m.W = Wt;
  m.Mxx = (uint64_t)(int64_t)(int32_t)(Wt * ix2 * ix2);
  m.Mxy = (uint64_t)(int64_t)(int32_t)(Wt * ix2 * iy2);
  m.Myy = (uint64_t)(int64_t)(int32_t)(Wt * iy2 * iy2);
  return m;
}

__device__ __forceinline__ Moments to_moments(const Mom6& s, int32_t N) {
  Moments m;
  m.Mx = (int32_t)s.Mx; m.My = (int32_t)s.My; m.W = (int32_t)s.W;
  m.Mxx = (int64_t)s.Mxx; m.Myy = (int64_t)s.Myy; m.Mxy = (int64_t)s.Mxy;
  m.N = N;
  return m;
}

__device__ __forceinline__ float window_err(const Mom6& s, int32_t N) {
  const Moments m = to_moments(s, N);
  const uint64_t Wl = (uint32_t)m.W;
  const int64_t Cxx = (int64_t)((uint64_t)m.Mxx * Wl - (uint64_t)((int64_t)m.Mx * (int64_t)m.Mx));
  const int64_t Cxy = (int64_t)((uint64_t)m.Mxy * Wl - (uint64_t)((int64_t)m.Mx * (int64_t)m.My));
  const int64_t Cyy = (int64_t)((uint64_t)m.Myy * Wl - (uint64_t)((int64_t)m.My * (int64_t)m.My));
  auto tof = [](int64_t v) { return (float)(double)v; };
  const float h = det_hypotf(tof(Cxx - Cyy), tof(2 * Cxy));
  const float eig = (tof(Cxx + Cyy) - h) / (float)(8u * (uint32_t)Wl * (uint32_t)Wl);
  return (float)m.N * eig;
}


template <int NT, int CAP>
constexpr int kKeySlots = (NT >= 512 && CAP <= 4096) ? 2 * CAP
                          : CAP < 400 ? 400
                                      : CAP;

struct SegFits {
  double err[kNMaxima][kNMaxima];
  double mse[kNMaxima][kNMaxima];
  double p[kNMaxima][kNMaxima][2];
};

template <int NT, int CAP>
struct BlobShared {
  uint64_t keys[kKeySlots<NT, CAP>];
  uint32_t bcnt[kKeySlots<NT, CAP> / 4];
  uint64_t pks[16];
  uint64_t wtop[NT > 64 ? NT / 64 * 10 : 1];
  uint32_t tMx[21], tMy[21], tW[21];
  uint64_t tMxx[21], tMyy[21], tMxy[21];
  uint32_t bMx[NT > 64 ? NT : 1], bMy[NT > 64 ? NT : 1], bW[NT > 64 ? NT : 1];
  uint64_t bMxx[NT > 64 ? NT : 1], bMyy[NT > 64 ? NT : 1], bMxy[NT > 64 ? NT : 1];
  Mom6 wsum[NT / 64];
  int64_t red7[NT / 64][8];
  double red_f64[16];
  uint32_t red_u32[16];
  uint32_t red_idx[16];
  uint32_t item, nwork, npeaks;
  int32_t pi[16];
  double lines[4][4];
  uint32_t pacc[22];
  uint32_t ph[10];
  uint32_t slow_dt, slow_n, slow_ph[10];
  uint64_t t_last, t_item;
};

constexpr uint64_t kThetaSpan = 50265600;

template <int NT, int CAP>
__device__ bool team_bucket_sort(BlobShared<NT, CAP>& S, int n) {
  constexpr int KEYS = kKeySlots<NT, CAP>;
  if (n < 64 || 2 * n > KEYS) return false;
  const int tid = team_rank<NT>();
  int nb = 32;
  while (2 * nb < n) nb <<= 1;
  auto bucket = [&](uint64_t k) { return (uint32_t)(((k >> kKeyTheta) * (uint64_t)nb) / kThetaSpan); };
  uint32_t* bcnt = S.bcnt;
  for (int i = tid; i < nb / 2; i += NT) bcnt[i] = 0;
  team_sync<NT>();
  for (int t = tid; t < n; t += NT) {
    const uint32_t bk = bucket(S.keys[t]);
    atomicAdd(&bcnt[bk >> 1], 1u << ((bk & 1) * 16));
  }
  team_sync<NT>();
  const int per = nb >= NT ? nb / NT : 1;
  const int b0 = tid * per;
  uint32_t loc = 0, mx = 0;
  uint32_t cval[16];
#pragma unroll
  for (int j = 0; j < 16; j++) {
    cval[j] = 0;
    if (j < per && b0 + j < nb) {
      const uint32_t bb = (uint32_t)(b0 + j);
      cval[j] = (bcnt[bb >> 1] >> ((bb & 1) * 16)) & 0xffffu;
      loc += cval[j];
      mx = cval[j] > mx ? cval[j] : mx;
    }
  }
  uint32_t tot;
  const uint32_t incl = team_incl_scan<NT>(loc, S.red_u32, &tot);
  mx = team_reduce<NT>(mx, MaxOp(), S.red_u32);
  if (mx > 32) return false;
  team_sync<NT>();
  uint32_t run = incl - loc;
#pragma unroll
  for (int j = 0; j < 16; j++) {
    if (j < per && b0 + j < nb && (j & 1) == 0) {
      const uint32_t bb = (uint32_t)(b0 + j);
      if (per >= 2) {
        const uint32_t s0 = run, s1 = run + cval[j];
        bcnt[bb >> 1] = s0 | (s1 << 16);
      }
    }
    if (j < per && b0 + j < nb) run += cval[j];
  }
  if (per == 1 && b0 < nb) {
    const uint32_t mine = incl - loc;
    const uint32_t other = __shfl_down(mine, 1);
    if ((b0 & 1) == 0) bcnt[b0 >> 1] = mine | (other << 16);
  }
  team_sync<NT>();
  uint64_t* T = S.keys + KEYS / 2;
  for (int t = tid; t < n; t += NT) {
    const uint64_t k = S.keys[t];
    const uint32_t bk = bucket(k);
    const uint32_t old = atomicAdd(&bcnt[bk >> 1], 1u << ((bk & 1) * 16));
    T[(old >> ((bk & 1) * 16)) & 0xffffu] = k;
  }
  team_sync<NT>();
  for (int s = tid; s < n; s += NT) {
    const uint64_t k = T[s];
    const uint32_t bk = bucket(k);
    int lo = s, hi = s + 1;
    while (lo > 0 && bucket(T[lo - 1]) == bk) lo--;
    while (hi < n && bucket(T[hi]) == bk) hi++;
    int r = lo;
    for (int j = lo; j < hi; j++) r += T[j] < k;
    S.keys[r] = k;
  }
  team_sync<NT>();
  return true;
}

template <bool kGlob>
__device__ __forceinline__ uint64_t pk_get(const uint64_t* lds, const uint64_t* gpk, int cap, int i) {
  if constexpr (kGlob) return i < cap ? lds[i] : gpk[i - cap];
  else return lds[i];
}
template <bool kGlob>
__device__ __forceinline__ void pk_put(uint64_t* lds, uint64_t* gpk, int cap, int i, uint64_t v) {
  if constexpr (kGlob) {
    if (i < cap) lds[i] = v;
    else gpk[i - cap] = v;
  } else {
    lds[i] = v;
  }
}
template <int NT, bool kGlob>
__device__ void team_bitonic_sort_pk(uint64_t* lds, uint64_t* gpk, int cap, int n) {
  const int r = team_rank<NT>();
  for (int k = 2; k <= n; k <<= 1) {
    for (int j = k >> 1; j > 0; j >>= 1) {
      for (int i = r; i < n; i += NT) {
        const int ixj = i ^ j;
        if (ixj > i) {
          const uint64_t a = pk_get<kGlob>(lds, gpk, cap, i), c = pk_get<kGlob>(lds, gpk, cap, ixj);
          const bool up = (i & k) == 0;
          if ((a > c) == up) {
            pk_put<kGlob>(lds, gpk, cap, i, c);
            pk_put<kGlob>(lds, gpk, cap, ixj, a);
          }
        }
      }
      team_sync<NT>();
    }
  }
}

template <int NT, int CAP>
__device__ __forceinline__ void team_extents(BlobShared<NT, CAP>& S, uint32_t& mnx, uint32_t& mxx, uint32_t& mny,
                                             uint32_t& mxy, int32_t& sgx, int32_t& sgy, int64_t& spg) {
  mnx = wave_reduce(mnx, MinOp()); mxx = wave_reduce(mxx, MaxOp());
  mny = wave_reduce(mny, MinOp()); mxy = wave_reduce(mxy, MaxOp());
  sgx = wave_reduce(sgx, AddOp()); sgy = wave_reduce(sgy, AddOp());
  spg = wave_reduce(spg, AddOp());
  if constexpr (NT > 64) {
    const int w = threadIdx.x >> 6;
    team_sync<NT>();
    if (lane_id() == 0) {
      S.red7[w][0] = mnx; S.red7[w][1] = mxx; S.red7[w][2] = mny; S.red7[w][3] = mxy;
      S.red7[w][4] = sgx; S.red7[w][5] = sgy; S.red7[w][6] = spg;
    }
    team_sync<NT>();
    for (int i = 0; i < NT / 64; i++) {
      mnx = min(mnx, (uint32_t)S.red7[i][0]); mxx = max(mxx, (uint32_t)S.red7[i][1]);
      mny = min(mny, (uint32_t)S.red7[i][2]); mxy = max(mxy, (uint32_t)S.red7[i][3]);
    }
    int32_t gx = 0, gy = 0;
    int64_t pg = 0;
    for (int i = 0; i < NT / 64; i++) {
      gx += (int32_t)S.red7[i][4]; gy += (int32_t)S.red7[i][5]; pg += S.red7[i][6];
    }
    sgx = gx; sgy = gy; spg = pg;
  }
}

template <int NT, int CAP>
__device__ __forceinline__ Mom6 team_excl_scan_mom(BlobShared<NT, CAP>& S, const Mom6& v, Mom6* total) {
  const uint32_t lane = lane_id();
  Mom6 incl;
  incl.Mx = wave_incl_scan(v.Mx, AddOp(), 0u);
  incl.My = wave_incl_scan(v.My, AddOp(), 0u);
  incl.W = wave_incl_scan(v.W, AddOp(), 0u);
  incl.Mxx = wave_incl_scan(v.Mxx, AddOp(), (uint64_t)0);
  incl.Myy = wave_incl_scan(v.Myy, AddOp(), (uint64_t)0);
  incl.Mxy = wave_incl_scan(v.Mxy, AddOp(), (uint64_t)0);
  Mom6 ex = incl;
  mom_sub(ex, v);
  if constexpr (NT > 64) {
    const int w = threadIdx.x >> 6;
    team_sync<NT>();
    if (lane == 63) S.wsum[w] = incl;
    team_sync<NT>();
    Mom6 tot = mom_zero();
    for (int i = 0; i < NT / 64; i++) {
      if (i < w) mom_add(ex, S.wsum[i]);
      mom_add(tot, S.wsum[i]);
    }
    *total = tot;
  } else {
    *total = Mom6{wave_read(incl.Mx, 63), wave_read(incl.My, 63), wave_read(incl.W, 63),
                  wave_read(incl.Mxx, 63), wave_read(incl.Myy, 63), wave_read(incl.Mxy, 63)};
  }
  return ex;
}

constexpr uint32_t kRegSortMaxBucket = 512;

template <int CAP>
__device__ bool wave_bucket_sort_kv(BlobShared<64, CAP>& S, uint64_t (&kv)[CAP / 64], int n) {
  static_assert(CAP % 64 == 0 && CAP <= 1024, "wave sort: at most 16 keys per lane");
  constexpr int PB = CAP > 512 ? 8 : 4;
  static_assert(kThetaSpan <= (1ull << 26), "theta fits 26 bits");
  constexpr int KPL = CAP / 64;
  const uint32_t lane = lane_id();
  int nb = 32;
  while (2 * nb < n) nb <<= 1;
  const int sh = 26 - __builtin_ctz((unsigned)nb);
  auto bucket = [&](uint64_t k) { return (uint32_t)((k >> kKeyTheta) >> sh); };
  uint32_t* bcnt = S.bcnt;
  for (int i = (int)lane; i < nb / 2; i += 64) bcnt[i] = 0;
  team_sync<64>();
#pragma unroll
  for (int j = 0; j < KPL; j++) {
    if (j * 64 + (int)lane < n) {
      const uint32_t bk = bucket(kv[j]);
      atomicAdd(&bcnt[bk >> 1], 1u << ((bk & 1) * 16));
    }
  }
  team_sync<64>();
  const int per = nb >= 64 ? nb / 64 : 1;
  const int b0 = (int)lane * per;
  uint32_t cval[PB], loc = 0, mx = 0;
#pragma unroll
  for (int j = 0; j < PB; j++) {
    cval[j] = 0;
    if (j < per && b0 + j < nb) {
      const uint32_t bb = (uint32_t)(b0 + j);
      cval[j] = (bcnt[bb >> 1] >> ((bb & 1) * 16)) & 0xffffu;
      loc += cval[j];
      mx = cval[j] > mx ? cval[j] : mx;
    }
  }
  const uint32_t incl = wave_incl_scan(loc, AddOp(), 0u);
  mx = wave_reduce(mx, MaxOp());
  if (mx > kRegSortMaxBucket) {
#pragma unroll
    for (int j = 0; j < KPL; j++) {
      const int t = j * 64 + (int)lane;
      if (t < n) S.keys[t] = kv[j];
    }
    team_sync<64>();
    return false;
  }
  team_sync<64>();
  uint32_t run = incl - loc;
  uint32_t st[PB];
#pragma unroll
  for (int j = 0; j < PB; j++) {
    st[j] = run;
    if (j < per && b0 + j < nb) run += cval[j];
  }
  if (per >= 2) {
#pragma unroll
    for (int j = 0; j < PB; j += 2)
      if (j < per) bcnt[(b0 + j) >> 1] = st[j] | (st[j + 1] << 16);
  } else if (b0 < nb) {
    const uint32_t other = wave_read_next(st[0]);
    if ((b0 & 1) == 0) bcnt[b0 >> 1] = st[0] | (other << 16);
  }
  team_sync<64>();
#pragma unroll
  for (int j = 0; j < KPL; j++) {
    if (j * 64 + (int)lane < n) {
      const uint32_t bk = bucket(kv[j]);
      const uint32_t old = atomicAdd(&bcnt[bk >> 1], 1u << ((bk & 1) * 16));
      S.keys[(old >> ((bk & 1) * 16)) & 0xffffu] = kv[j];
    }
  }
  team_sync<64>();
  uint32_t rk[KPL];
#pragma unroll
  for (int j = 0; j < KPL; j++) {
    rk[j] = 0;
    if (j * 64 + (int)lane < n) {
      const uint32_t bk = bucket(kv[j]);
      const uint32_t hi = (bcnt[bk >> 1] >> ((bk & 1) * 16)) & 0xffffu;
      const uint32_t lo = bk ? (bcnt[(bk - 1) >> 1] >> (((bk - 1) & 1) * 16)) & 0xffffu : 0u;
      uint32_t r = lo;
      for (uint32_t i = lo; i < hi; i++) r += S.keys[i] < kv[j];
      rk[j] = r;
    }
  }
  team_sync<64>();
#pragma unroll
  for (int j = 0; j < KPL; j++)
    if (j * 64 + (int)lane < n) S.keys[rk[j]] = kv[j];
  team_sync<64>();
  return true;
}

template <int CAP>
__device__ bool wave_bucket_sort(BlobShared<64, CAP>& S, const uint64_t* keys, int n) {
  constexpr int KPL = CAP / 64;
  const uint32_t lane = lane_id();
  uint64_t kv[KPL];
#pragma unroll
  for (int j = 0; j < KPL; j++) {
    const int t = j * 64 + (int)lane;
    kv[j] = t < n ? keys[t] : ~0ull;
  }
  return wave_bucket_sort_kv<CAP>(S, kv, n);
}

// ... 269 lines not shown
    const float theta = (float)(((double)det_atan2f(dyf, dxf) + 3.14159265358979323846) * 8e6);
    long long ti = (long long)rintf(theta);
    if (ti < 0) ti = 0;
    const int32_t ix = (int32_t)(px + 1) / 2, iy = (int32_t)(py + 1) / 2;
    int32_t Wt = 1;
    if (ix > 0 && ix + 1 < g.Wd && iy > 0 && iy + 1 < g.Hd) {
      const int32_t gxv = (int32_t)((gp[u] >> 8) & 0xff) - (int32_t)(gp[u] & 0xff);
      const int32_t gyv = (int32_t)(gp[u] >> 24) - (int32_t)((gp[u] >> 16) & 0xff);
      Wt = lf_weight(gxv, gyv);
    }
    kv[u] = ((uint64_t)(ti & 0xfffffff) << kKeyTheta) | ((uint64_t)dxy << 30) | ((uint64_t)by << 20) |
            ((uint64_t)bx << 10) | (((k >> 3) & 1) << 9) | (uint64_t)Wt;
  }
  return true;
}

struct PairInfo {
  uint32_t n, off, sel;
};
__device__ __forceinline__ PairInfo load_pair_info(const DevBufs& b, uint32_t w) {
  const size_t i = (size_t)(w >> 16) * kMaxPairs + (w & 0xffff);
  return PairInfo{b.pair_cnt[i], b.pair_off[i], b.pair_sel[i]};
}


template <int NT, int CAP, bool FUSE = false>
__device__ void blob_item(const DevBufs& b, const Geom& g, const Params& prm, BlobShared<NT, CAP>& S, uint64_t* gpk,
                          const uint32_t* combo, uint32_t w, PairInfo pi_, uint32_t* pacc) {
  constexpr int kC = (CAP + NT - 1) / NT;
  static_assert(kC <= 32, "chunk too long");
  const int tid = team_rank<NT>();
  const uint32_t lane = lane_id();
  if (AT_PROBE_ON(prm) && tid == 0) S.t_last = S.t_item = wall_clock64();
  bool big = false;
  auto phase = [&](int k) {
    if (AT_PROBE_ON(prm) && tid == 0) {
      if (k == 9) __builtin_amdgcn_s_waitcnt(0);
      const uint64_t now = wall_clock64();
      pacc[k] += (uint32_t)(now - S.t_last);
      S.ph[k] = (uint32_t)(now - S.t_last);
      pacc[10 + k] += 1;
      if (NT > 64 && big) {
        atomicAdd((unsigned long long*)&b.probe[208 + k], (unsigned long long)(now - S.t_last));
        if (k == 0) atomicAdd((unsigned long long*)&b.probe[220], 1ull);
      }
      S.t_last = now;
    }
  };
  const int f = (int)(w >> 16);
  const uint32_t rank = w & 0xffff;
  const uint32_t n = pi_.n;
  big = n > 2048;
  const uint32_t* grp = b.grp + (size_t)f * g.cap_pts + pi_.off;
  uint64_t* keys = b.keys + (size_t)f * g.cap_pts + pi_.off;

  bool sorted = false, in_lds = false;
  const uint32_t bi = rank & 0xfff;
  if constexpr (NT > 64 && FUSE) {
    uint64_t kv[CAP / NT];
    if (!large_extents_keys<NT, CAP>(b, g, S, f, rank, n, grp, kv)) return;
    if (tid == 0) pacc[20] += n;
    phase(0);
    phase(1);
    sorted = team_reg_bucket_sort_kv<NT, CAP>(S, kv, (int)n);
    in_lds = true;
  } else if constexpr (NT == 64 && FUSE) {
    uint64_t kv[kSmallBlob / 64];
    if (!small_extents_keys(b, g, f, rank, n, grp, kv)) return;
    if (tid == 0) pacc[20] += n;
    phase(0);
    phase(1);
    if (n >= 64) {
      sorted = wave_bucket_sort_kv<CAP>(S, kv, (int)n);
    } else {
#pragma unroll
      for (int j = 0; j < kSmallBlob / 64; j++)
        if (j * 64 + (int)lane < (int)n) S.keys[j * 64 + lane] = kv[j];
      team_sync<NT>();
      sorted = team_bucket_sort<NT, CAP>(S, (int)n);
    }
    in_lds = true;
  } else {
  if (pi_.sel == 0) return;
  if (tid == 0) pacc[20] += n;
  phase(0);
  if constexpr (NT == 64) {
    if (n >= 64) {
      phase(1);
      sorted = wave_bucket_sort<CAP>(S, keys, (int)n);
      in_lds = true;
    }
  } else if constexpr (CAP / NT <= 16) {
    if (n >= 64) {
      phase(1);
      sorted = team_reg_bucket_sort<NT, CAP>(S, keys, (int)n);
      in_lds = true;
    }
  }
  if (!sorted && !in_lds) {
    for (uint32_t t = tid; t < n; t += NT) S.keys[t] = keys[t];
    phase(1);
    team_sync<NT>();
    sorted = team_bucket_sort<NT, CAP>(S, (int)n);
  }
  }
  if (!sorted) {
    int np2 = 64;
    while (np2 < (int)n) np2 <<= 1;
    for (int t = (int)n + tid; t < np2; t += NT) S.keys[t] = ~0ull;
    team_sync<NT>();
    team_bitonic_sort<uint64_t, NT>(S.keys, np2);
  }
  phase(2);
  if (AT_DIAG_STOP(prm, 2)) return;

  const uint32_t c = (n + NT - 1) / NT;
  const uint32_t t0 = min(n, (uint32_t)tid * c), t1 = min(n, t0 + c);
  uint32_t* cw = reinterpret_cast<uint32_t*>(S.keys);
  float* errv = reinterpret_cast<float*>(S.keys) + CAP;
  uint32_t word[kC];
  Mom6 csum = mom_zero();
#pragma unroll
  for (int k = 0; k < kC; k++) {
    word[k] = 0;
    if (k >= (int)c) break;
    const uint32_t t = t0 + k;
    if (t < t1) {
      const uint64_t sk = S.keys[t];
      word[k] = compact_word(sk);
      const uint64_t pbits = (((sk >> 10) & 0x3ff) << 14) | (((sk >> 20) & 0x3ff) << 4) | (((sk >> 9) & 1) << 3) |
                             ((sk >> 30) & 3);
      if (prm.taps) keys[t] = ((uint64_t)bi << 52) | (((sk >> kKeyTheta) & 0xfffffff) << 24) | pbits;
      mom_add(csum, point_mom(word[k]));
    }
  }
  team_sync<NT>();
#pragma unroll
  for (int k = 0; k < kC; k++) {
    if (k >= (int)c) break;
    if (t0 + k < t1) cw[t0 + k] = word[k];
  }
  Mom6 total;
  const Mom6 cbase = team_excl_scan_mom<NT, CAP>(S, csum, &total);
  if constexpr (NT > 64) {
    S.bMx[tid] = cbase.Mx; S.bMy[tid] = cbase.My; S.bW[tid] = cbase.W;
    S.bMxx[tid] = cbase.Mxx; S.bMyy[tid] = cbase.Myy; S.bMxy[tid] = cbase.Mxy;
  }
  team_sync<NT>();
  phase(3);
  if (AT_DIAG_STOP(prm, 3)) return;

  const uint32_t ksz = n / 12 < 20 ? n / 12 : 20;
  const int32_t Nw = (int32_t)(2 * ksz + 1);
  const bool act = t0 < t1;
  {
    const int lo = (int)t0 - (int)ksz, hi = (int)t0 + (int)ksz;
    const int ia = hi >= (int)n ? hi - (int)n : hi;
    const int ib = (lo >= 0 ? lo : lo + (int)n) - 1;
    const Mom6 pa = prefix_at<NT, CAP>(S, cw, cbase, c, (uint32_t)ia, act);
    const Mom6 pb = prefix_at<NT, CAP>(S, cw, cbase, c, (uint32_t)(ib >= 0 ? ib : 0), act && ib >= 0);
    Mom6 s = pa;
    mom_sub(s, pb);
    if (lo < 0 || hi >= (int)n) mom_add(s, total);
    if (act) errv[t0] = window_err(s, Nw);
    for (uint32_t t = t0 + 1; t < t1; t++) {
      uint32_t ja = t + ksz, jr = t + n - ksz - 1;
      ja -= ja >= n ? n : 0;
      jr -= jr >= n ? n : 0;
      mom_add(s, point_mom(cw[ja]));
      mom_sub(s, point_mom(cw[jr]));
      errv[t] = window_err(s, Nw);
    }
  }
  team_sync<NT>();
  phase(4);

  constexpr int kEW = kC + 8;
  float ew[kEW];
  if (t0 < t1) {
#pragma unroll
    for (int j = 0; j < kEW; j++) {
      uint32_t idx = t0 + 2 * n + j - 4;
      idx -= idx >= n ? n : 0;
      idx -= idx >= n ? n : 0;
      idx -= idx >= n ? n : 0;
      ew[j] = errv[idx];
    }
  }
  auto filt_k = [&](int k) -> double {
    double acc = 0.0;
#pragma unroll
    for (int j = 0; j < 7; j++) acc += (double)ew[k + 1 + j] * (double)c_filter[j];
    return acc;
  };
  constexpr int kPR = (kC + 1) / 2;
  uint64_t mine[kPR];
#pragma unroll
  for (int j = 0; j < kPR; j++) mine[j] = ~0ull;
  uint32_t nmine = 0;
  if (t0 < t1) {
    double fprev = filt_k(-1), fcur = filt_k(0);
#pragma unroll
    for (int k = 0; k < kC; k++) {
      const uint32_t t = t0 + k;
      if (k >= (int)c || t >= t1) break;
      const double fnext = filt_k(k + 1);
      if (fcur > fprev && fcur > fnext) {
        const float ef = (float)(-fcur);
        uint32_t u = __float_as_uint(ef);
        u = (u & 0x80000000u) ? ~u : (u | 0x80000000u);
        mine[k >> 1] = ((uint64_t)u << 32) | t;
        nmine++;
      }
      fprev = fcur;
      fcur = fnext;
    }
  }
  const uint32_t npk = team_reduce<NT>(nmine, AddOp(), S.red_u32);
  uint64_t* pks = S.pks;
  {
    const int ntop = npk < (uint32_t)kNMaxima ? (int)npk : kNMaxima;
    uint64_t last = 0;
    if constexpr (NT == 64) {
      if (npk <= 64) {
        uint64_t* pall = reinterpret_cast<uint64_t*>(errv);
        team_sync<64>();
        uint32_t pos = wave_incl_scan(nmine, AddOp(), 0u) - nmine;
#pragma unroll
        for (int j = 0; j < kPR; j++)
          if (mine[j] != ~0ull) pall[pos++] = mine[j];
        team_sync<64>();
        if (lane < npk) {
          const uint64_t pv = pall[lane];
          uint32_t r = 0;
          for (uint32_t j = 0; j < npk; j++) r += pall[j] < pv;
          if (r < (uint32_t)kNMaxima) pks[r] = pv;
        }
      } else {
      for (int r = 0; r < ntop; r++) {
        uint64_t m = ~0ull;
#pragma unroll
        for (int j = 0; j < kPR; j++) {
          const uint64_t k = mine[j];
          if ((r == 0 || k > last) && k < m) m = k;
        }
        m = wave_reduce(m, MinOp());
        if (tid == 0) pks[r] = m;
        last = m;
      }
      }
    } else {
      const int w = tid >> 6, ln = tid & 63;
      for (int r = 0; r < ntop; r++) {
        uint64_t m = ~0ull;
#pragma unroll
        for (int j = 0; j < kPR; j++) {
          const uint64_t k = mine[j];
          if ((r == 0 || k > last) && k < m) m = k;
        }
        m = wave_reduce(m, MinOp());
        if (ln == 0) S.wtop[w * kNMaxima + r] = m;
        last = m;
      }
      team_sync<NT>();
      if (w == 0) {
        constexpr int NC = NT / 64 * kNMaxima;
        uint64_t c0 = ~0ull, c1 = ~0ull;
        if (ln < NC && (ln % kNMaxima) < ntop) c0 = S.wtop[ln];
        if (ln + 64 < NC && ((ln + 64) % kNMaxima) < ntop) c1 = S.wtop[ln + 64];
        last = 0;
        for (int r = 0; r < ntop; r++) {
          uint64_t m = ~0ull;
          if ((r == 0 || c0 > last) && c0 < m) m = c0;
          if ((r == 0 || c1 > last) && c1 < m) m = c1;
          m = wave_reduce(m, MinOp());
          if (ln == 0) pks[r] = m;
          last = m;
        }
      }
    }
    team_sync<NT>();
  }
  phase(5);
  if (AT_DIAG_STOP(prm, 4)) return;
  const int cnt = (int)npk;
  if (tid < 16) {
    const int v = (tid < cnt && tid < kNMaxima) ? (int)(pks[tid] & 0xffffffffu) : 0xffff;
    int r = 0;
    for (int j = 0; j < 16; j++) {
      const int u = (j < cnt && j < kNMaxima) ? (int)(pks[j] & 0xffffffffu) : 0xffff;
      r += (u < v) || (u == v && j < tid);
    }
    S.pi[r] = v;
  }
  team_sync<NT>();
  {
    const int k = tid;
    uint32_t idx = 0;
    bool need = false;
    if (k < 10) { need = k < cnt && k < kNMaxima; idx = need ? (uint32_t)S.pi[k] : 0; }
    else if (k < 20) { need = k - 10 < cnt && k - 10 < kNMaxima && S.pi[k - 10] > 0; idx = need ? (uint32_t)S.pi[k - 10] - 1 : 0; }
    else if (k == 20) { need = true; idx = n - 1; }
    const Mom6 p = prefix_at<NT, CAP>(S, cw, cbase, c, idx, need);
    if (need) {
      S.tMx[k] = p.Mx; S.tMy[k] = p.My; S.tW[k] = p.W;
      S.tMxx[k] = p.Mxx; S.tMyy[k] = p.Myy; S.tMxy[k] = p.Mxy;
    }
  }
  team_sync<NT>();
  phase(6);
  auto seg_moments = [&](int a, int bb) -> Moments {
    const uint32_t i0 = (uint32_t)S.pi[a], i1 = (uint32_t)S.pi[bb];
    Mom6 m = Mom6{S.tMx[bb], S.tMy[bb], S.tW[bb], S.tMxx[bb], S.tMyy[bb], S.tMxy[bb]};
    const Mom6 pm = Mom6{S.tMx[10 + a], S.tMy[10 + a], S.tW[10 + a], S.tMxx[10 + a], S.tMyy[10 + a], S.tMxy[10 + a]};
    int32_t N;
    if (i0 < i1) {
      if (i0 > 0) mom_sub(m, pm);
      N = (int32_t)(i1 - i0 + 1);
    } else {
      Mom6 z = Mom6{S.tMx[20], S.tMy[20], S.tW[20], S.tMxx[20], S.tMyy[20], S.tMxy[20]};
      mom_sub(z, pm);
      mom_add(z, m);
      m = z;
      N = (int32_t)(n - i0 + i1 + 1);
    }
    return to_moments(m, N);
  };
  SegFits& seg = *reinterpret_cast<SegFits*>(S.keys);
  static_assert(sizeof(SegFits) <= sizeof(S.keys), "segment fits must fit over the keys");
  const int cn = min(cnt, kNMaxima);
  const float rcn = 1.0f / (float)max(cn, 1);
  for (int ci = tid; cnt >= 4 && ci < cn * cn; ci += NT) {
    const int a = (int)(((float)ci + 0.5f) * rcn), bb = ci - a * cn;
    if (a != bb) {
      const LineFitOut o = fit_line_v<false, true>(seg_moments(a, bb));
      seg.err[a][bb] = o.err;
      seg.mse[a][bb] = o.mse;
      seg.p[a][bb][0] = o.p23[0];
      seg.p[a][bb][1] = o.p23[1];
    }
  }
  team_sync<NT>();
  phase(7);
  if (AT_DIAG_STOP(prm, 7)) return;
  double err = DBL_MAX;
  uint32_t bt = 0xffffffffu;
  const double mse_max = (double)prm.max_line_fit_mse;
  const int ncomb = cnt < 4 ? 0 : cnt >= kNMaxima ? 210 : (cnt * (cnt - 1) * (cnt - 2) * (cnt - 3)) / 24;
  for (int cj = tid; cj < ncomb; cj += NT) {
    double e4 = DBL_MAX;
    const int ci = (int)combo[210 + cj];
    {
      const uint32_t cb = combo[ci];
      const int m0 = cb & 0xff, m1 = (cb >> 8) & 0xff, m2 = (cb >> 16) & 0xff, m3 = cb >> 24;
      if (!(seg.mse[m0][m1] > mse_max)) {
        if (!(seg.mse[m1][m2] > mse_max)) {
          const double dot =
              seg.p[m0][m1][0] * seg.p[m1][m2][0] + seg.p[m0][m1][1] * seg.p[m1][m2][1];
          if (!(fabs(dot) > prm.cos_critical_rad)) {
            if (!(seg.mse[m2][m3] > mse_max) && !(seg.mse[m3][m0] > mse_max))
              e4 = seg.err[m0][m1] + seg.err[m1][m2] + seg.err[m2][m3] + seg.err[m3][m0];
          }
        }
      }
    }
    if (bt == 0xffffffffu || e4 < err || (e4 == err && (uint32_t)ci < bt)) { err = e4; bt = (uint32_t)ci; }
  }
#pragma unroll
  for (int d = 32; d > 0; d >>= 1) {
    const double oe = __shfl_xor(err, d);
    const uint32_t ot = __shfl_xor(bt, d);
    if (oe < err || (oe == err && ot < bt)) { err = oe; bt = ot; }
  }
  if constexpr (NT > 64) {
    if (lane == 0) { S.red_f64[tid >> 6] = err; S.red_idx[tid >> 6] = bt; }
    team_sync<NT>();
    err = S.red_f64[0];
    bt = S.red_idx[0];
    for (int i = 1; i < NT / 64; i++)
      if (S.red_f64[i] < err || (S.red_f64[i] == err && S.red_idx[i] < bt)) { err = S.red_f64[i]; bt = S.red_idx[i]; }
  }
  phase(8);
  if (AT_DIAG_STOP(prm, 8)) return;
  const double best = err;
  if (bt >= 210) bt = 0;
  const bool valid = best < (double)(prm.max_line_fit_mse * (float)n);
  uint16_t qidx[4];
  const uint32_t cbt = combo[bt];
  for (int k = 0; k < 4; k++) qidx[k] = (uint16_t)S.pi[(cbt >> (8 * k)) & 0xff];
  if constexpr (!FUSE) {
    QuadPend& qp = b.qpend[(size_t)f * kMaxPairs + rank];
    if (valid && tid < 4) {
      float pre[4];
      double e_, m_;
      fit_line(seg_moments((cbt >> (8 * tid)) & 0xff, (cbt >> (8 * ((tid + 1) & 3))) & 0xff), nullptr, nullptr, &e_, &m_,
               pre);
      *reinterpret_cast<float4*>(qp.fit[tid]) = make_float4(pre[0], pre[1], pre[2], pre[3]);
    }
    if (tid == 0) {
      qp.blob_index = bi;
      qp.valid = valid;
      for (int k = 0; k < 4; k++) qp.indices[k] = qidx[k];
      pacc[21] += 1;
    }
    phase(9);
    team_sync<NT>();
    return;
  }
  if (valid && tid < 4) {
    const LineFitOut o =
        fit_line_v<true, true>(seg_moments((cbt >> (8 * tid)) & 0xff, (cbt >> (8 * ((tid + 1) & 3))) & 0xff));
    S.lines[tid][0] = o.p01[0];
    S.lines[tid][1] = o.p01[1];
    S.lines[tid][2] = o.p23[0];
    S.lines[tid][3] = o.p23[1];
  }
  team_sync<NT>();
  if (tid < 64) {
    const uint32_t ln = lane_id();
    float cxk = 0.f, cyk = 0.f;
    bool cok = true;
    if (valid && ln < 4) {
      const int k = (int)ln, k1 = (k + 1) & 3;
      const double A00 = S.lines[k][3], A01 = -S.lines[k1][3];
      const double A10 = -S.lines[k][2], A11 = S.lines[k1][2];
      const double B0 = -S.lines[k][0] + S.lines[k1][0];
      const double B1 = -S.lines[k][1] + S.lines[k1][1];
      const double det = A00 * A11 - A10 * A01;
      const double W00 = A11 / det, W01 = -A01 / det;
      cok = !(fabs(det) < 0.001);
      if (cok) {
        const double L0 = W00 * B0 + W01 * B1;
        cxk = (float)(S.lines[k][0] + L0 * A00);
        cyk = (float)(S.lines[k][1] + L0 * A10);
      }
    }
    int ok = valid && __ballot(ln < 4 && !cok) == 0;
    float qc[4][2];
#pragma unroll
    for (int k = 0; k < 4; k++) {
      qc[k][0] = wave_read(cxk, k);
      qc[k][1] = wave_read(cyk, k);
    }
    if (ok) {
      float lj = 0.f;
      if (ln < 6) {
        const int a2 = ln == 0 ? 0 : ln == 1 ? 1 : ln == 2 ? 2 : ln == 3 ? 2 : ln == 4 ? 3 : 0;
        const int b2 = ln == 0 ? 1 : ln == 1 ? 2 : ln == 2 ? 0 : ln == 3 ? 3 : ln == 4 ? 0 : 2;
        const float xa = a2 == 0 ? qc[0][0] : a2 == 1 ? qc[1][0] : a2 == 2 ? qc[2][0] : qc[3][0];
        const float ya = a2 == 0 ? qc[0][1] : a2 == 1 ? qc[1][1] : a2 == 2 ? qc[2][1] : qc[3][1];
        const float xb = b2 == 0 ? qc[0][0] : b2 == 1 ? qc[1][0] : b2 == 2 ? qc[2][0] : qc[3][0];
        const float yb = b2 == 0 ? qc[0][1] : b2 == 1 ? qc[1][1] : b2 == 2 ? qc[2][1] : qc[3][1];
        lj = det_hypotf(xb - xa, yb - ya);
      }
      float len[6];
#pragma unroll
      for (int j = 0; j < 6; j++) len[j] = wave_read(lj, j);
      float area = 0, pp;
      pp = (len[0] + len[1] + len[2]) / 2;
      area += sqrtf(pp * (pp - len[0]) * (pp - len[1]) * (pp - len[2]));
      pp = (len[3] + len[4] + len[5]) / 2;
      area += sqrtf(pp * (pp - len[3]) * (pp - len[4]) * (pp - len[5]));
      if ((double)area < 0.95 * g.min_tag_width * g.min_tag_width) ok = 0;
    }
    if (ok) {
      bool abad = false;
      if (ln < 4) {
        const int i0 = (int)ln, i1 = (i0 + 1) & 3, i2 = (i0 + 2) & 3;
        auto cx = [&](int i) { return i == 0 ? qc[0][0] : i == 1 ? qc[1][0] : i == 2 ? qc[2][0] : qc[3][0]; };
        auto cy = [&](int i) { return i == 0 ? qc[0][1] : i == 1 ? qc[1][1] : i == 2 ? qc[2][1] : qc[3][1]; };
        const float dx1 = cx(i1) - cx(i0), dy1 = cy(i1) - cy(i0);
        const float dx2 = cx(i2) - cx(i1), dy2 = cy(i2) - cy(i1);
        const float cosd = (dx1 * dx2 + dy1 * dy2) / sqrtf((dx1 * dx1 + dy1 * dy1) * (dx2 * dx2 + dy2 * dy2));
        abad = (double)fabsf(cosd) > prm.cos_critical_rad || dx1 * dy2 < dy1 * dx2;
      }
      if (__ballot(abad)) ok = 0;
    }
  if (ln == 0) {
    QuadRecord rec;
    rec.blob_index = bi;
    rec.valid = valid;
    for (int k = 0; k < 4; k++) rec.indices[k] = qidx[k];
    QuadCand qcand;
    for (int k = 0; k < 4; k++) {
      const float x = ok ? (qc[k][0] - 0.5f) * 2.0f + 0.5f : 0.f;
      const float y = ok ? (qc[k][1] - 0.5f) * 2.0f + 0.5f : 0.f;
      rec.corners[k][0] = qcand.p[k][0] = x;
      rec.corners[k][1] = qcand.p[k][1] = y;
    }
    rec.accepted = ok;
    if (prm.taps) b.quads[(size_t)f * kMaxPairs + rank] = rec;
    pacc[21] += 1;
    if (ok && !AT_DIAG_STOP(prm, 5)) {
      qcand.frame = (uint32_t)f;
      qcand.rank = rank;
      const uint32_t ci = atomicAdd(b.nqcand + (size_t)f * kQcStride, 1u);
      if (ci < (uint32_t)kQuadCandPerFrame) b.qcand[(size_t)f * kQuadCandPerFrame + ci] = qcand;
      else atomicOr(b.status + f, kStatusQuadsOverflow);
    }
  }
  }
  phase(9);
  if (AT_PROBE_ON(prm) && tid == 0) {
    const uint32_t dt = (uint32_t)(S.t_last - S.t_item);
    if (dt > S.slow_dt) {
      S.slow_dt = dt;
      S.slow_n = n;
      for (int k = 0; k < 10; k++) S.slow_ph[k] = S.ph[k];
    }
  }
  team_sync<NT>();
}

__device__ __forceinline__ void load_combos(uint32_t* s_combo, int tid, int nt) {
  for (int i = tid; i < 210; i += nt) {
    s_combo[i] = (uint32_t)c_combo[i][0] | ((uint32_t)c_combo[i][1] << 8) | ((uint32_t)c_combo[i][2] << 16) |
                 ((uint32_t)c_combo[i][3] << 24);
    s_combo[210 + i] = c_colex[i];
  }
}

__device__ __forceinline__ bool work_item(const DevBufs& b, const uint32_t* cnt, int c0, int c1, uint32_t it,
                                          uint32_t* w) {
  for (int c = c0; c < c1; c++) {
    if (it < cnt[c]) {
      *w = b.work[(size_t)c * b.wcap + it];
      return true;
    }
    it -= cnt[c];
  }
  return false;
}

template <int NT>
__device__ __forceinline__ void extents_item(const DevBufs& b, const Geom& g, uint32_t w, int64_t (*red)[8]) {
  const int tid = team_rank<NT>();
  const int f = (int)(w >> 16);
  const uint32_t rank = w & 0xffff;
  const uint32_t n = b.pair_cnt[(size_t)f * kMaxPairs + rank];
  const size_t so = (size_t)f * g.cap_pts + b.pair_off[(size_t)f * kMaxPairs + rank];
  const uint32_t* grp = b.grp + so;
  uint64_t* keys = b.keys + so;
  const uint8_t* dec = b.dec + (size_t)f * g.Wd * g.Hd;
  uint32_t mnx = 0xffff, mny = 0xffff, mxx = 0, mxy = 0;
  int32_t sgx = 0, sgy = 0;
  int64_t spg = 0;
#ifndef AT_EXT_U
#define AT_EXT_U 4
#endif
  constexpr int U = AT_EXT_U;
#ifndef AT_EXT_KEY_UNROLL
#define AT_EXT_KEY_UNROLL 4
#endif
#ifndef AT_EXT_KR
#define AT_EXT_KR 1
#endif
  uint32_t kr[U];
  for (uint32_t base = 0; base < n; base += NT * U) {
    uint32_t kk[U];
#pragma unroll
    for (int u = 0; u < U; u++) {
      const uint32_t t = base + u * NT + tid;
      kk[u] = t < n ? grp[t] : 0;
    }
#pragma unroll
    for (int u = 0; u < U; u++) {
      if (AT_EXT_KR && base == 0) kr[u] = kk[u];
      if (base + u * NT + tid >= n) continue;
      const uint64_t k = kk[u];
      const int dxy = (int)(k & 3);
      const uint32_t px = ((k >> 14) & 0x3ff) * 2 + dx_of(dxy);
      const uint32_t py = ((k >> 4) & 0x3ff) * 2 + dy_of(dxy);
      const bool b2w = (k & 8) != 0;
      const int gx = b2w ? dx_of(dxy) : -dx_of(dxy), gy = b2w ? dy_of(dxy) : -dy_of(dxy);
      mnx = min(mnx, px); mxx = max(mxx, px); mny = min(mny, py); mxy = max(mxy, py);
      sgx += gx; sgy += gy;
      spg += (int64_t)px * gx + (int64_t)py * gy;
    }
  }
  mnx = wave_reduce(mnx, MinOp()); mxx = wave_reduce(mxx, MaxOp());
  mny = wave_reduce(mny, MinOp()); mxy = wave_reduce(mxy, MaxOp());
  sgx = wave_reduce(sgx, AddOp()); sgy = wave_reduce(sgy, AddOp());
  spg = wave_reduce(spg, AddOp());
  if constexpr (NT > 64) {
    const int wv = threadIdx.x >> 6;
    if (lane_id() == 0) {
      red[wv][0] = mnx; red[wv][1] = mxx; red[wv][2] = mny; red[wv][3] = mxy;
      red[wv][4] = sgx; red[wv][5] = sgy; red[wv][6] = spg;
    }
    __syncthreads();
    int32_t gx = 0, gy = 0;
    int64_t pg = 0;
    for (int i = 0; i < NT / 64; i++) {
      mnx = min(mnx, (uint32_t)red[i][0]); mxx = max(mxx, (uint32_t)red[i][1]);
      mny = min(mny, (uint32_t)red[i][2]); mxy = max(mxy, (uint32_t)red[i][3]);
      gx += (int32_t)red[i][4]; gy += (int32_t)red[i][5]; pg += red[i][6];
    }
    sgx = gx; sgy = gy; spg = pg;
    __syncthreads();
  }
  Ext e;
  e.min_x = mnx; e.max_x = mxx; e.min_y = mny; e.max_y = mxy;
  e.gx_sum = sgx; e.gy_sum = sgy; e.pg_sum = spg;
  e.count = n;
  bool keep = (int)((e.max_x - e.min_x) * (e.max_y - e.min_y)) >= g.min_tag_width;
  keep = keep && !((double)ext_dot(e) < 0.0);
  if (!keep) return;
  if (tid == 0) b.pair_sel[(size_t)f * kMaxPairs + rank] = 1;
  const double cx = ext_cx(e), cy = ext_cy(e);
  for (uint32_t base = 0; base < n; base += NT * U) {
    uint32_t kk[U];
    uint32_t gp[U];
#pragma unroll
    for (int u = 0; u < U; u++) {
      const uint32_t t = base + u * NT + tid;
      kk[u] = (AT_EXT_KR && base == 0) ? kr[u] : (t < n ? grp[t] : 0);
    }
#pragma unroll
    for (int u = 0; u < U; u++) {
      const uint64_t k = kk[u];
      const int dxy = (int)(k & 3);
      const int32_t ix = (int32_t)(((k >> 14) & 0x3ff) * 2 + dx_of(dxy) + 1) / 2;
      const int32_t iy = (int32_t)(((k >> 4) & 0x3ff) * 2 + dy_of(dxy) + 1) / 2;
      const bool in = base + u * NT + tid < n && ix > 0 && ix + 1 < g.Wd && iy > 0 && iy + 1 < g.Hd;
      const int32_t at = in ? iy * g.Wd + ix : g.Wd + 1;
      gp[u] = (uint32_t)dec[at - 1] | ((uint32_t)dec[at + 1] << 8) | ((uint32_t)dec[at - g.Wd] << 16) |
              ((uint32_t)dec[at + g.Wd] << 24);
    }
#pragma unroll AT_EXT_KEY_UNROLL
    for (int u = 0; u < U; u++) {
      const uint32_t t = base + u * NT + tid;
      if (t >= n) continue;
      const uint64_t k = kk[u];
      const int dxy = (int)(k & 3);
      const uint32_t bx = (k >> 14) & 0x3ff, by = (k >> 4) & 0x3ff;
      const uint32_t px = bx * 2 + dx_of(dxy), py = by * 2 + dy_of(dxy);
      const float dyf = (float)((double)py - cy);
      const float dxf = (float)((double)px - cx);
      const float theta = (float)(((double)det_atan2f(dyf, dxf) + 3.14159265358979323846) * 8e6);
      long long ti = (long long)rintf(theta);
      if (ti < 0) ti = 0;
      const int32_t ix = (int32_t)(px + 1) / 2, iy = (int32_t)(py + 1) / 2;
      int32_t Wt = 1;
      if (ix > 0 && ix + 1 < g.Wd && iy > 0 && iy + 1 < g.Hd) {
        const int32_t gxv = (int32_t)((gp[u] >> 8) & 0xff) - (int32_t)(gp[u] & 0xff);
        const int32_t gyv = (int32_t)(gp[u] >> 24) - (int32_t)((gp[u] >> 16) & 0xff);
        Wt = lf_weight(gxv, gyv);
      }
      keys[t] = ((uint64_t)(ti & 0xfffffff) << kKeyTheta) | ((uint64_t)dxy << 30) | ((uint64_t)by << 20) |
               ((uint64_t)bx << 10) | (((k >> 3) & 1) << 9) | (uint64_t)Wt;
    }
  }
}

#ifndef AT_EXT_WAVES
#define AT_EXT_WAVES 5
#endif
#ifndef AT_EXT_GRID
#define AT_EXT_GRID 2560
#endif
__global__ __launch_bounds__(256) __attribute__((amdgpu_waves_per_eu(AT_EXT_WAVES))) void k_extents(DevBufs b, Geom g) {
  __shared__ int64_t s_red[4][8];
  kt_begin(b, 7);
  uint32_t cnt[kNumCls], total = 0, nlarge = 0;
#pragma unroll
  for (int c = 0; c < kNumCls; c++) {
    cnt[c] = min(b.ncls[c], b.wcap);
    total += cnt[c];
    if (c < g.nlarge) nlarge += cnt[c];
  }
  for (uint32_t it = blockIdx.x; it < nlarge; it += gridDim.x) {
    uint32_t w = 0;
    work_item(b, cnt, 0, kNumCls, it, &w);
    extents_item<256>(b, g, w, s_red);
  }
  if (g.ctw != 32) {
    const uint32_t gw = blockIdx.x * 4 + (threadIdx.x >> 6), nw = gridDim.x * 4;
    for (uint32_t it = nlarge + gw; it < total; it += nw) {
      uint32_t w = 0;
      work_item(b, cnt, 0, kNumCls, it, &w);
      extents_item<64>(b, g, w, nullptr);
    }
  }
  __syncthreads();
  if (threadIdx.x == 0) kt_end(b, 7);
}

template <int NT, int CAP>
__device__ __forceinline__ void probe_flush_slow(const DevBufs& b, const Params& prm, const BlobShared<NT, CAP>& S,
                                                 bool leader) {
  if (!AT_PROBE_ON(prm) || !leader || !S.slow_dt) return;
  atomicMax((unsigned long long*)&b.probe[NT == 64 ? 200 : 201], ((unsigned long long)S.slow_dt << 20) | S.slow_n);
  if (NT == 64) {
    for (int k = 0; k < 10; k++) atomicAdd((unsigned long long*)&b.probe[224 + k], (unsigned long long)S.slow_ph[k]);
    atomicAdd((unsigned long long*)&b.probe[234], 1ull);
  }
}

__device__ __forceinline__ void probe_flush(const DevBufs& b, const Params& prm, const uint32_t* pacc, int base,
                                            bool leader) {
  if (!AT_PROBE_ON(prm) || !leader) return;
  for (int k = 0; k < 10; k++) {
    if (pacc[k]) atomicAdd((unsigned long long*)&b.probe[base + k], (unsigned long long)pacc[k]);
    if (pacc[10 + k]) atomicAdd((unsigned long long*)&b.probe[base + 32 + k], (unsigned long long)pacc[10 + k]);
  }
}

template <int NT, int CAP, bool FUSE>
__device__ __forceinline__ void large_blob_loop(const DevBufs& b, const Geom& g, const Params& prm, BlobShared<NT, CAP>& S,
                                const uint32_t* s_combo, const uint32_t* s_cnt, uint32_t nlo, uint32_t slot,
                                int c0, int c1, int launch) {
  const int tid = threadIdx.x;
  uint32_t* pacc = S.pacc;
  if (tid < 22) pacc[tid] = 0;
  if (tid == 0) S.slow_dt = 0;
  uint64_t* gpk = b.s_pk + (size_t)slot * (kSortCap / 2);
  __syncthreads();
  uint32_t nwork = 0;
  for (int c = c0; c < c1; c++) nwork += s_cnt[c];
  uint32_t* head = launch == 0 ? b.workhead : launch == 1 ? b.workhead_small : b.workhead_mid;
  while (true) {
    if (tid == 0) S.item = atomicAdd(head, 1u);
    __syncthreads();
    const uint32_t item = S.item;
    __syncthreads();
    if (item >= nwork) break;
    uint32_t w = 0;
    work_item(b, s_cnt, c0, c1, item, &w);
    const PairInfo pi = FUSE ? PairInfo{b.pair_cnt[(size_t)(w >> 16) * kMaxPairs + (w & 0xffff)], b.pair_off[(size_t)(w >> 16) * kMaxPairs + (w & 0xffff)], 0u} : load_pair_info(b, w);
    if (pi.n > (uint32_t)CAP || pi.n <= nlo) continue;
    blob_item<NT, CAP, FUSE>(b, g, prm, S, gpk, s_combo, w, pi, pacc);
  }
  __syncthreads();
  probe_flush(b, prm, pacc, 80, tid == 0);
  probe_flush_slow(b, prm, S, tid == 0);
  if (tid == 0 && pacc[20]) atomicAdd(b.blob_pts + 1, pacc[20]);
  if (tid == 0 && pacc[21]) atomicAdd(b.nquads, pacc[21]);
}

template <bool FUSE, int CAP = kSmallBlob>
__device__ __forceinline__ void small_blob_loop(const DevBufs& b, const Geom& g, const Params& prm, BlobShared<64, CAP>& S,
                                const uint32_t* s_combo, const uint32_t* s_cnt, uint32_t wv, uint32_t nwaves,
                                int c0, int c1) {
  const uint32_t lane = lane_id();
  uint32_t* pacc = S.pacc;
  if (lane < 22) pacc[lane] = 0;
  if (lane == 0) S.slow_dt = 0;
  uint32_t nwork = 0;
  for (int c = c0; c < c1; c++) nwork += s_cnt[c];
  uint32_t item = wv;
  uint32_t w = 0, w1 = 0;
  PairInfo pi = {0, 0, 0};
  if (item < nwork) {
    work_item(b, s_cnt, c0, c1, item, &w);
    pi = load_pair_info(b, w);
  }
  if (item + nwaves < nwork) work_item(b, s_cnt, c0, c1, item + nwaves, &w1);
  for (; item < nwork; item += nwaves) {
    const bool has1 = item + nwaves < nwork;
    const PairInfo pi1 = has1 ? load_pair_info(b, w1) : PairInfo{0, 0, 0};
    uint32_t w2 = 0;
    if (item + 2 * nwaves < nwork) work_item(b, s_cnt, c0, c1, item + 2 * nwaves, &w2);
    [[clang::always_inline]] blob_item<64, CAP, FUSE>(b, g, prm, S, nullptr, s_combo, w, pi, pacc);
    w = w1;
    pi = pi1;
    w1 = w2;
  }
  probe_flush(b, prm, pacc, 64, lane == 0);
  probe_flush_slow(b, prm, S, lane == 0);
  if (lane == 0 && pacc[20]) atomicAdd(b.blob_pts + 0, pacc[20]);
  if (lane == 0 && pacc[21]) atomicAdd(b.nquads, pacc[21]);
}

template <int NT, int CAP, bool FUSE = false>
__global__ __launch_bounds__(NT) __attribute__((amdgpu_waves_per_eu(NT == 256 && CAP == 4096 && !FUSE ? 3 : 1))) void k_blob(DevBufs b, Geom g, Params prm, uint32_t nlo, int c0, int c1, int launch) {
  __shared__ BlobShared<NT, CAP> S;
  const int tid = threadIdx.x;
  uint32_t kt_slot = ~0u;
  if (!launch) {
    kt_begin(b, 9);
  } else if (b.kt_stage == 9 && tid == 0) {
    kt_slot = atomicAdd(b.kgrid, 1u);
    if (kt_slot < b.kwg_cap) b.kwg[kt_slot] = wall_clock64();
  }
  __shared__ uint32_t s_combo[420], s_cnt[kNumCls];
  load_combos(s_combo, tid, NT);
  if (tid < kNumCls) s_cnt[tid] = min(b.ncls[tid], b.wcap);
  large_blob_loop<NT, CAP, FUSE>(b, g, prm, S, s_combo, s_cnt, nlo, blockIdx.x, c0, c1, launch);
  if (tid == 0 && !launch) kt_end(b, 9);
  if (tid == 0 && launch && kt_slot < b.kwg_cap) b.kwg[b.kwg_cap + kt_slot] = wall_clock64();
}

#ifndef AT_BS_WAVES
#define AT_BS_WAVES 4
#endif

template <bool FUSE, int CAP = kSmallBlob, int WAVES = AT_BS_WAVES, int STAGE = 8>
__global__ __launch_bounds__(256) __attribute__((amdgpu_waves_per_eu(FUSE ? 2 : WAVES))) void k_blob_small(DevBufs b, Geom g, Params prm,
                                                                                                         int c0, int c1, int launch) {
  __shared__ BlobShared<64, CAP> Ss[4];
  const int wave = threadIdx.x >> 6;
  uint32_t kt_slot = ~0u;
  if (!launch) {
    kt_begin(b, STAGE);
  } else if (b.kt_stage == STAGE && threadIdx.x == 0) {
    kt_slot = atomicAdd(b.kgrid, 1u);
    if (kt_slot < b.kwg_cap) b.kwg[kt_slot] = wall_clock64();
  }
  __shared__ uint32_t s_combo[420], s_cnt[kNumCls];
  load_combos(s_combo, threadIdx.x, 256);
  if (threadIdx.x < kNumCls) s_cnt[threadIdx.x] = min(b.ncls[threadIdx.x], b.wcap);
  __syncthreads();
  small_blob_loop<FUSE, CAP>(b, g, prm, Ss[wave], s_combo, s_cnt, blockIdx.x * 4 + wave, gridDim.x * 4, c0, c1);
  if (b.kt_stage == STAGE) {
    __syncthreads();
    if (threadIdx.x == 0 && !launch) kt_end(b, STAGE);
    if (threadIdx.x == 0 && launch && kt_slot < b.kwg_cap) b.kwg[b.kwg_cap + kt_slot] = wall_clock64();
  }
}

__global__ __launch_bounds__(512) void k_blob_lat(DevBufs b, Geom g, Params prm) {
  using SL = BlobShared<512, 4096>;
  using SS = BlobShared<64, kSmallBlob>;
  static_assert(8 * sizeof(SS) <= sizeof(SL), "eight small-blob waves fit in a large team's LDS");
  __shared__ __attribute__((aligned(16))) unsigned char s_raw[sizeof(SL)];
  __shared__ uint32_t s_combo[420], s_cnt[kNumCls];
  const int tid = threadIdx.x;
  kt_begin(b, 9);
  load_combos(s_combo, tid, 512);
  if (tid < kNumCls) s_cnt[tid] = min(b.ncls[tid], b.wcap);
  const uint32_t team = blockIdx.x >> 1, nteam = gridDim.x >> 1;
  if ((blockIdx.x & 1) == 0) {
    large_blob_loop<512, 4096, true>(b, g, prm, *reinterpret_cast<SL*>(s_raw), s_combo, s_cnt, 0u, team, 0, g.nlarge, 0);
  } else {
    __syncthreads();
    const int wave = tid >> 6;
    small_blob_loop<true>(b, g, prm, reinterpret_cast<SS*>(s_raw)[wave], s_combo, s_cnt, team * 8 + wave, nteam * 8,
                          g.nlarge, kNumCls);
  }
  if (b.kt_stage == 9) {
    __syncthreads();
    if (tid == 0) kt_end(b, 9);
  }
}

__global__ __launch_bounds__(256) void k_quad_fin(DevBufs b, Geom g, Params prm, int c0, int c1) {
  __shared__ uint32_t s_cnt[kNumCls];
  if (threadIdx.x < kNumCls) s_cnt[threadIdx.x] = min(b.ncls[threadIdx.x], b.wcap);
  __syncthreads();
  uint32_t nwork = 0;
  for (int c = c0; c < c1; c++) nwork += s_cnt[c];
  const uint32_t lane = lane_id(), base = lane & ~3u;
  const int k = (int)(lane & 3);
  auto from = [&](double v, int j) { return __shfl(v, (int)base + j); };
  auto fromf = [&](float v, int j) { return __shfl(v, (int)base + j); };
  auto quad_or = [&](int v) {
    v |= __shfl_xor(v, 1);
    return v | __shfl_xor(v, 2);
  };
  for (uint32_t it = (blockIdx.x * 256 + threadIdx.x) >> 2; it < nwork; it += gridDim.x * 64) {
    uint32_t w = 0;
    work_item(b, s_cnt, c0, c1, it, &w);
    const uint32_t f = w >> 16, rank = w & 0xffff;
    const size_t slot = (size_t)f * kMaxPairs + rank;
    if (b.pair_sel[slot] == 0) continue;
    const QuadPend& qp = b.qpend[slot];
    const bool valid = qp.valid != 0;
    float cx = 0.f, cy = 0.f;
    int bad = 0;
    {
      double l[4] = {0, 0, 0, 0};
      if (valid) {
        const float4 pre = *reinterpret_cast<const float4*>(qp.fit[k]);
        l[0] = (double)pre.z;
        l[1] = (double)pre.w;
        line_normal(pre.x, pre.y, det_hypotf(pre.x, pre.y), l + 2);
      }
      double m[4];
#pragma unroll
      for (int j = 0; j < 4; j++) m[j] = from(l[j], (k + 1) & 3);
      if (valid) {
        const double A00 = l[3], A01 = -m[3];
        const double A10 = -l[2], A11 = m[2];
        const double B0 = -l[0] + m[0];
        const double B1 = -l[1] + m[1];
        const double det = A00 * A11 - A10 * A01;
        const double W00 = A11 / det, W01 = -A01 / det;
        if (fabs(det) < 0.001) {
          bad = 1;
        } else {
          const double L0 = W00 * B0 + W01 * B1;
          cx = (float)(l[0] + L0 * A00);
          cy = (float)(l[1] + L0 * A10);
        }
      }
    }
    bool ok = valid && !quad_or(bad);
    float qc[4][2];
#pragma unroll
    for (int j = 0; j < 4; j++) {
      qc[j][0] = fromf(cx, j);
      qc[j][1] = fromf(cy, j);
    }
    if (ok) {
      auto side = [&](int j) {
        const int a2 = j == 0 ? 0 : j == 1 ? 1 : j == 2 ? 2 : j == 3 ? 2 : j == 4 ? 3 : 0;
        const int b2 = j == 0 ? 1 : j == 1 ? 2 : j == 2 ? 0 : j == 3 ? 3 : j == 4 ? 0 : 2;
        return det_hypotf(qc[b2][0] - qc[a2][0], qc[b2][1] - qc[a2][1]);
      };
      const float s0 = side(k), s1 = side(4 + (k & 1));
      float len[6];
#pragma unroll
      for (int j = 0; j < 4; j++) len[j] = fromf(s0, j);
      len[4] = fromf(s1, 0);
      len[5] = fromf(s1, 1);
      float area = 0, pp;
      pp = (len[0] + len[1] + len[2]) / 2;
      area += sqrtf(pp * (pp - len[0]) * (pp - len[1]) * (pp - len[2]));
      pp = (len[3] + len[4] + len[5]) / 2;
      area += sqrtf(pp * (pp - len[3]) * (pp - len[4]) * (pp - len[5]));
      if ((double)area < 0.95 * g.min_tag_width * g.min_tag_width) ok = false;
    }
    if (ok) {
      const int i0 = k, i1 = (i0 + 1) & 3, i2 = (i0 + 2) & 3;
      const float dx1 = qc[i1][0] - qc[i0][0], dy1 = qc[i1][1] - qc[i0][1];
      const float dx2 = qc[i2][0] - qc[i1][0], dy2 = qc[i2][1] - qc[i1][1];
      const float cosd = (dx1 * dx2 + dy1 * dy2) / sqrtf((dx1 * dx1 + dy1 * dy1) * (dx2 * dx2 + dy2 * dy2));
      const int abad = (double)fabsf(cosd) > prm.cos_critical_rad || dx1 * dy2 < dy1 * dx2;
      if (quad_or(abad)) ok = false;
    }
    if (k == 0) {
      QuadRecord rec;
      rec.blob_index = qp.blob_index;
      rec.valid = valid;
      for (int j = 0; j < 4; j++) rec.indices[j] = qp.indices[j];
      QuadCand qcand;
      for (int j = 0; j < 4; j++) {
        const float x = ok ? (qc[j][0] - 0.5f) * 2.0f + 0.5f : 0.f;
        const float y = ok ? (qc[j][1] - 0.5f) * 2.0f + 0.5f : 0.f;
        rec.corners[j][0] = qcand.p[j][0] = x;
        rec.corners[j][1] = qcand.p[j][1] = y;
      }
      rec.accepted = ok;
      if (prm.taps) b.quads[slot] = rec;
      if (ok && !AT_DIAG_STOP(prm, 5)) {
        qcand.frame = f;
        qcand.rank = rank;
        const uint32_t ci = atomicAdd(b.nqcand + (size_t)f * kQcStride, 1u);
        if (ci < (uint32_t)kQuadCandPerFrame) b.qcand[(size_t)f * kQuadCandPerFrame + ci] = qcand;
        else atomicOr(b.status + f, kStatusQuadsOverflow);
      }
    }
  }
}

constexpr int kDecodeThreads = 64;
__device__ __forceinline__ void border_pattern(int p, float wab, float& x0, float& y0, float& dx, float& dy) {
  const float far_ = (p & 1) ? wab - 0.5f : wab + 0.5f;
  const float near_ = (p & 1) ? 0.5f : -0.5f;
  const int side = p >> 1;
  const float a = (side == 0 || side == 2) ? near_ : far_;
  if (side < 2) { x0 = a; y0 = 0.5f; dx = 0; dy = 1; }
  else { x0 = 0.5f; y0 = a; dx = 1; dy = 0; }
}

__device__ __forceinline__ uint64_t rotate90_n(uint64_t w, int nbits) {
  int p = nbits;
  uint64_t l = 0;
  if (nbits % 4 == 1) { p = nbits - 1; l = 1; }
  w = ((w >> l) << (p / 4 + l)) | (w >> (3 * p / 4 + l) << l) | (w & l);
  return w & ((1ull << nbits) - 1);
}
constexpr int kMaxTotalWidth = 12;

__device__ __forceinline__ double readlane_f64(double v, int l) {
  const uint64_t u = __builtin_bit_cast(uint64_t, v);
  const uint32_t lo = (uint32_t)__builtin_amdgcn_readlane((int)(uint32_t)u, l);
  const uint32_t hi = (uint32_t)__builtin_amdgcn_readlane((int)(uint32_t)(u >> 32), l);
  return __builtin_bit_cast(double, (uint64_t)lo | ((uint64_t)hi << 32));
}
__constant__ double c_rot_c[4] = {1.0, 6.123233995736766e-17, -1.0, -1.8369701987210297e-16};
__constant__ double c_rot_s[4] = {0.0, 1.0, 1.2246467991473532e-16, -1.0};

struct DecodeShared {
  double sx[kLdsRefine], sy[kLdsRefine];
  float qc[4][2];
  int nsamp[4], samp_off[4];
  float enx[4], eny[4];
  double lines[4][4];
  double H[9];
  double A[72];
  double gmx[64], gmy[64], gmv[64];
  int gmvalid[64];
  double wC[3], bC[3];
  double values[kMaxTotalWidth * kMaxTotalWidth];
  int ok;
  uint32_t item;
  uint32_t qpre[kMaxBatch + 1];
};

struct PoseHandoff {
  double H[9], p[4][2];
  double R[9], t[3], err[2];
  uint32_t seq, ack, exit;
};
__device__ void pose_worker(PoseHandoff& P, const Params& prm) {
  const uint32_t lane = lane_id();
  uint32_t seen = 0;
  while (true) {
    uint32_t sq;
    bool done = false;
    while ((sq = __hip_atomic_load(&P.seq, __ATOMIC_ACQUIRE, __HIP_MEMORY_SCOPE_WORKGROUP)) == seen) {
      if (__hip_atomic_load(&P.exit, __ATOMIC_ACQUIRE, __HIP_MEMORY_SCOPE_WORKGROUP)) { done = true; break; }
      __builtin_amdgcn_s_sleep(1);
    }
    if (done) return;
    seen = sq;
    double H[9], pc[4][2];
#pragma unroll
    for (int k = 0; k < 9; k++) H[k] = P.H[k];
#pragma unroll
    for (int k = 0; k < 4; k++) { pc[k][0] = P.p[k][0]; pc[k][1] = P.p[k][1]; }
    double R[9], t[3], err[2];
    pose::estimate_tag_pose<true>(H, pc, prm.fx, prm.fy, prm.cx, prm.cy, prm.tag_size, R, t, err, (int)(lane & 3));
    if (lane == 0) {
#pragma unroll
      for (int k = 0; k < 9; k++) P.R[k] = R[k];
#pragma unroll
      for (int k = 0; k < 3; k++) P.t[k] = t[k];
      P.err[0] = err[0];
      P.err[1] = err[1];
      __hip_atomic_store(&P.ack, seen, __ATOMIC_RELEASE, __HIP_MEMORY_SCOPE_WORKGROUP);
    }
  }
}
__device__ void decode_finish(const DevBufs& b, int lane, uint32_t nq) {
  const uint32_t nwg = min(gridDim.x, nq);
  if (blockIdx.x >= max(nwg, 1u)) return;
  uint32_t last = nwg == 0;
  if (lane == 0 && nwg) {
    __threadfence();
    last = atomicAdd(b.dec_done, 1u) == nwg - 1;
  }
  last = __shfl(last, 0);
  if (!last) return;
  __threadfence();
  for (uint32_t w = (uint32_t)lane; w < b.ctrl_words; w += 64)
    b.hctrl[w] = __hip_atomic_load(b.ctrl + w, __ATOMIC_RELAXED, __HIP_MEMORY_SCOPE_AGENT);
}

#ifndef AT_BIG_BLOB_WG
#define AT_BIG_BLOB_WG 256
#endif
#ifndef AT_BIG_NT
#define AT_BIG_NT 512
#endif
#ifndef AT_FORK_SMALL
#define AT_FORK_SMALL 1
#endif
#ifndef AT_POSE_IN_DECODE
#define AT_POSE_IN_DECODE 1
#endif
#ifndef AT_DEC_WAVES
#define AT_DEC_WAVES 4
#endif

struct DecodeRow {
  union {
    struct { double sx[kRowRefine], sy[kRowRefine]; } ref;
    double A[72];
    struct { double x[64], y[64], v[64]; uint8_t valid[64]; } gm;
    double values[kMaxTotalWidth * kMaxTotalWidth];
  } u;
  float qc[4][2];
  int nsamp[4], samp_off[4];
  float enx[4], eny[4];
  double lines[4][4];
  double H[9];
  double wC[3], bC[3];
  int f;
  uint32_t rank;
};

template <int LPQ>
__device__ __forceinline__ void decode_rows(const DevBufs& b, const Geom& g, const Params& prm, int B, int fmt) {
  constexpr int NR = 64 / LPQ;
  constexpr int RCAP = kMaxRefineSamples;
  constexpr int kBitRounds = kMaxFamilyBits / LPQ;
  __shared__ DecodeRow rows[NR];
  __shared__ uint32_t qpre[kMaxBatch + 1];
  const int tid = threadIdx.x;
  const int row = tid / LPQ, rl = tid % LPQ;
  kt_begin(b, 10);
  constexpr int kGy = kMaxRefineSamples - kRowRefine;
  {
    uint32_t c[kMaxBatch / 64], sum = 0;
#pragma unroll
    for (int k = 0; k < kMaxBatch / 64; k++) {
      const int f = tid * (kMaxBatch / 64) + k;
      c[k] = f < B ? min(b.nqcand[(size_t)f * kQcStride], (uint32_t)kQuadCandPerFrame) : 0u;
      sum += c[k];
    }
    const uint32_t incl = wave_incl_scan(sum, AddOp(), 0u);
    uint32_t acc = incl - sum;
#pragma unroll
    for (int k = 0; k < kMaxBatch / 64; k++) {
      const int f = tid * (kMaxBatch / 64) + k;
      if (f < B) qpre[f] = acc;
      acc += c[k];
    }
    if (tid == 63) qpre[B] = incl;
  }
  team_sync<64>();
  const uint32_t nq = qpre[B];

  uint32_t pacc[21] = {0};
  uint64_t t_last = 0;
  auto phase = [&](int k) {
    if (AT_PROBE_ON(prm) && tid == 0) {
      const uint64_t now = wall_clock64();
      if (k > 0) {
        pacc[k] += (uint32_t)(now - t_last);
        pacc[10 + k] += 1;
      }
      t_last = now;
    }
  };
  struct ItemPre {
    int f;
    uint32_t rank;
    float px, py;
    const uint8_t* gsrc;
  };
  auto prefetch = [&](uint32_t it, int rl) -> ItemPre {
    ItemPre p = {};
    if (it < nq) {
      int lo = 0, hi = B - 1;
      while (lo < hi) {
        const int mid = (lo + hi + 1) >> 1;
        if (qpre[mid] <= it) lo = mid;
        else hi = mid - 1;
      }
      const QuadCand* q = &b.qcand[(size_t)lo * kQuadCandPerFrame + (it - qpre[lo])];
      p.f = lo;
      p.rank = q->rank;
      p.px = rl < 4 ? q->p[rl & 3][0] : 0.f;
      p.py = rl < 4 ? q->p[rl & 3][1] : 0.f;
      p.gsrc = fmt == 1 ? b.gray + (size_t)lo * g.W * g.H : b.frames[lo];
    }
    return p;
  };
  const uint32_t G = gridDim.x;
  const int wab = prm.fam.width_at_border, tw = prm.fam.total_width, nbits = prm.fam.nbits;
  const int minc = (wab - tw) / 2;
  const uint32_t gsh = fmt == 0 ? 1 : 0, wsh = (uint32_t)g.W << gsh;
  ItemPre nxt = prefetch(NR * blockIdx.x + row, rl);
  for (uint32_t base = NR * blockIdx.x; base < nq; base += NR * G) {
    int tq = tid;
    __asm__ volatile("" : "+v"(tq));
    const int rowq = tq / LPQ;
    int rlq = tq % LPQ;
    DecodeRow& S = rows[rowq];
    auto gref = [&](int i) -> double* {
      return b.rsamp + ((size_t)blockIdx.x * NR + rowq) * (2 * kGy) + (i - kRowRefine);
    };
    const uint32_t item = base + rowq;
    const ItemPre cur = nxt;
    bool live = item < nq;
    const uint8_t* gsrc = cur.gsrc;
    typedef const __attribute__((address_space(1))) uint8_t* gbytes;
    auto pix = [&](int x, int y) -> uint32_t { return ((gbytes)gsrc)[(uint32_t)y * wsh + ((uint32_t)x << gsh)]; };
    if (live && rlq < 4) { S.qc[rlq][0] = cur.px; S.qc[rlq][1] = cur.py; }
    if (live && rlq == 0) { S.f = cur.f; S.rank = cur.rank; }
    team_sync<64>();
    phase(0);
    if (prm.refine_edges) {
      if (live && rlq < 4) {
        const int a2 = rlq, b2 = (rlq + 1) & 3;
        float nx = S.qc[b2][1] - S.qc[a2][1];
        float ny = -S.qc[b2][0] + S.qc[a2][0];
        const float mag = sqrtf(nx * nx + ny * ny);
        nx /= mag;
        ny /= mag;
        const int nsf = (int)(mag / 8);
        S.nsamp[rlq] = nsf > 16 ? nsf : 16;
        S.enx[rlq] = nx;
        S.eny[rlq] = ny;
      }
      team_sync<64>();
      if (live && rlq == 0) {
        int acc = 0;
        for (int k = 0; k < 4; k++) { S.samp_off[k] = acc; acc += S.nsamp[k]; }
      }
      team_sync<64>();
      const int want = live ? S.samp_off[3] + S.nsamp[3] : 0;
      const int total = min(want, RCAP);
      if (rlq == 0 && want > RCAP) atomicOr(b.status + S.f, kStatusQuadsOverflow);
      for (int t = rlq; t < total; t += LPQ) {
        int edge = 0;
        while (edge < 3 && t >= S.samp_off[edge + 1]) edge++;
        const int s = t - S.samp_off[edge];
        const int a2 = edge, b2 = (edge + 1) & 3;
        const int nsamples = S.nsamp[edge];
        const float nx = S.enx[edge], ny = S.eny[edge];
        const double alpha = (1.0 + s) / (nsamples + 1);
        const double x0 = alpha * S.qc[a2][0] + (1 - alpha) * S.qc[b2][0];
        const double y0 = alpha * S.qc[a2][1] + (1 - alpha) * S.qc[b2][1];
        constexpr int kSteps = 25, kPos = kSteps + 8;
        int pv[kPos];
        int xp = 0, yp = 0;
#pragma unroll
        for (int j = 0; j < kPos; j++) {
          const double m = -4.0 + 0.25 * j;
          const int x = (int)(x0 + m * nx);
          const int y = (int)(y0 + m * ny);
          const bool same = j > 0 && x == xp && y == yp;
          pv[j] = same ? -2 : -1;
          if (!same && !(x < 0 || x >= g.W || y < 0 || y >= g.H)) pv[j] = (int)pix(x, y);
          xp = x;
          yp = y;
        }
#pragma unroll
        for (int j = 1; j < kPos; j++)
          if (pv[j] == -2) pv[j] = pv[j - 1];
        double Mn = 0, Mcount = 0;
#pragma unroll
        for (int k = 0; k < kSteps; k++) {
          const double nn = -3.0 + 0.25 * k;
          const int g1 = pv[k + 8], g2 = pv[k];
          if (g1 < 0 || g2 < 0 || g1 < g2) continue;
          const double weight = (double)((g2 - g1) * (g2 - g1));
          Mn += weight * nn;
          Mcount += weight;
        }
        double bx = __longlong_as_double(0x7ff8deadbeef0000ll), by = 0;
        if (Mcount != 0) {
          const double n0 = Mn / Mcount;
          bx = x0 + n0 * nx;
          by = y0 + n0 * ny;
          undistort(prm, &bx, &by);
        }
        if (t < kRowRefine) {
          S.u.ref.sx[t] = bx;
          S.u.ref.sy[t] = by;
        } else {
          gref(t)[0] = bx;
          gref(t)[kGy] = by;
        }
      }
      team_sync<64>();
      phase(1);
      if (live && rlq < 4) {
        double Mx = 0, My = 0, Mxx = 0, Mxy = 0, Myy = 0, N = 0;
        const int o = S.samp_off[rlq];
// ... 1881 lines not shown
  hipLaunchKernelGGL(k_jpg_ff, dim3(g.mcuy), dim3(256), 0, st, b);
  hipLaunchKernelGGL(k_jpg_pack, dim3(g.mcuy), dim3(256), 0, st, b, g.mcuy);
  return hipGetLastError();
}

__global__ __launch_bounds__(256) void k_gp_cand(const float* __restrict__ raw, size_t frame_stride, int P, int C,
                                                 float conf_thr, GpParseBufs b) {
  const int f = blockIdx.y;
  const size_t i = (size_t)blockIdx.x * 256 + threadIdx.x;
  bool cand = false;
  float best = 0.0f;
  int32_t cls = 0;
  if (i < (size_t)P) {
    gp_candidate(raw + (size_t)f * frame_stride, (size_t)P, C, i, &best, &cls);
    cand = !gp_dropped(best, conf_thr);
  }
  __shared__ uint32_t s_cnt[4], s_base;
  const uint64_t m = __ballot(cand);
  const uint32_t wave = threadIdx.x >> 6;
  if (lane_id() == 0) s_cnt[wave] = (uint32_t)__popcll(m);
  __syncthreads();
  if (threadIdx.x == 0) {
    const uint32_t tot = s_cnt[0] + s_cnt[1] + s_cnt[2] + s_cnt[3];
    s_base = tot ? atomicAdd(b.cnt + (size_t)f * kGpCntStride, tot) : 0u;
  }
  __syncthreads();
  uint32_t base = s_base;
  for (uint32_t w = 0; w < wave; w++) base += s_cnt[w];
  const uint32_t slot = base + lanes_below(m);
  if (cand && slot < (uint32_t)kGpMaxCand) {
    b.key[(size_t)f * kGpMaxCand + slot] = gp_key(best, (uint32_t)i);
    b.cls[(size_t)f * kGpMaxCand + slot] = cls;
  }
}

constexpr int kGpNmsThreads = 1024;
constexpr int kGpPer = kGpMaxCand / kGpNmsThreads;
constexpr int kGpLiveWords = kGpMaxCand / 64;
constexpr int kGpWaves = kGpNmsThreads / 64;
static_assert(kGpLiveWords == 64 && kGpPer * kGpWaves == kGpLiveWords, "k_gp_nms: one live word per (k, wave)");

__global__ __launch_bounds__(kGpNmsThreads) void k_gp_nms(const float* __restrict__ raw, size_t frame_stride, int P,
                                                          float iou_thr, float sx, float sy, GpParseBufs b) {
  __shared__ uint64_t s_key[kGpMaxCand];
  __shared__ uint16_t s_slot[kGpMaxCand];
  __shared__ uint64_t s_live[kGpLiveWords];
  __shared__ uint32_t s_rank[kGpLiveWords];
  __shared__ GpCorners s_piv;
  __shared__ uint32_t s_n;
  const int f = blockIdx.x, tid = threadIdx.x;
  const uint32_t lane = lane_id(), wave = (uint32_t)tid >> 6;
  if (tid == 0) {
    const uint32_t c = b.cnt[(size_t)f * kGpCntStride];
    s_n = c;
    b.cnt[(size_t)f * kGpCntStride] = 0;
    b.info[2 * f + 1] = c;
    if (c == 0 || c > (uint32_t)kGpMaxCand) b.info[2 * f] = 0;
  }
  __syncthreads();
  const uint32_t ncand = s_n;
  if (ncand == 0 || ncand > (uint32_t)kGpMaxCand) return;

  const uint64_t* gkey = b.key + (size_t)f * kGpMaxCand;
  uint32_t n2 = 2;
  if (ncand <= (uint32_t)kGpNmsThreads) {
    const uint64_t mine = (uint32_t)tid < ncand ? gkey[tid] : ~0ull;
    if ((uint32_t)tid < ncand) s_key[tid] = mine;
    __syncthreads();
    uint32_t rank = 0;
    if ((uint32_t)tid < ncand) {
#pragma unroll 8
      for (uint32_t i = 0; i < ncand; i++) rank += s_key[i] < mine ? 1u : 0u;
    }
    __syncthreads();
    if ((uint32_t)tid < ncand) {
      s_key[rank] = mine;
      s_slot[rank] = (uint16_t)tid;
    }
    __syncthreads();
    n2 = 0;
  } else {
    while (n2 < ncand) n2 <<= 1;
    for (uint32_t j = tid; j < n2; j += kGpNmsThreads) {
      s_key[j] = j < ncand ? gkey[j] : ~0ull;
      s_slot[j] = (uint16_t)j;
    }
    __syncthreads();
  }
  for (uint32_t k = 2; k <= n2; k <<= 1) {
    for (uint32_t j = k >> 1; j > 0; j >>= 1) {
      for (uint32_t i = tid; i < n2; i += kGpNmsThreads) {
        const uint32_t ixj = i ^ j;
        if (ixj > i) {
          const uint64_t a = s_key[i], c = s_key[ixj];
          const bool up = (i & k) == 0;
          if ((a > c) == up) {
            s_key[i] = c;
            s_key[ixj] = a;
            const uint16_t t = s_slot[i];
            s_slot[i] = s_slot[ixj];
            s_slot[ixj] = t;
          }
        }
      }
      __syncthreads();
    }
  }

  const float* fr = raw + (size_t)f * frame_stride;
  const int32_t* gcls = b.cls + (size_t)f * kGpMaxCand;
  float bx[kGpPer], by[kGpPer], bw[kGpPer], bh[kGpPer], bconf[kGpPer];
  GpCorners bc[kGpPer];
  bool live[kGpPer];
#pragma unroll
  for (int k = 0; k < kGpPer; k++) {
    const uint32_t j = (uint32_t)tid + (uint32_t)k * kGpNmsThreads;
    live[k] = j < ncand;
    bx[k] = by[k] = bw[k] = bh[k] = bconf[k] = 0.0f;
    int32_t c = 0;
    if (live[k]) {
      const uint64_t key = s_key[j];
      const size_t i = gp_key_index(key);
      bconf[k] = gp_key_conf(key);
      bx[k] = fr[i];
      by[k] = fr[(size_t)P + i];
      bw[k] = fr[2 * (size_t)P + i];
      bh[k] = fr[3 * (size_t)P + i];
      c = gcls[s_slot[j]];
    }
    bc[k] = gp_corners(bx[k], by[k], bw[k], bh[k], c);
    const uint64_t m = __ballot(live[k]);
    if (lane == 0) s_live[k * kGpWaves + wave] = m;
  }

  const uint32_t nwords = (ncand + 63) >> 6;
  uint32_t pos = 0;
  for (;;) {
    __syncthreads();
    int p = -1;
    for (uint32_t w = pos >> 6; w < nwords; w++) {
      uint64_t m = s_live[w];
      if (w == (pos >> 6)) m &= ~0ull << (pos & 63);
      if (m) {
        p = (int)(w * 64 + (uint32_t)__builtin_ctzll(m));
        break;
      }
    }
    if (p < 0) break;
#pragma unroll
    for (int k = 0; k < kGpPer; k++)
      if ((uint32_t)p == (uint32_t)tid + (uint32_t)k * kGpNmsThreads) s_piv = bc[k];
    __syncthreads();
    const GpCorners a = s_piv;
#pragma unroll
    for (int k = 0; k < kGpPer; k++) {
      const uint32_t j = (uint32_t)tid + (uint32_t)k * kGpNmsThreads;
      const bool sup = live[k] && j > (uint32_t)p && gp_suppresses(a, bc[k], iou_thr);
      const uint64_t m = __ballot(sup);
      if (m && lane == 0) s_live[k * kGpWaves + wave] &= ~m;
      if (sup) live[k] = false;
    }
    pos = (uint32_t)p + 1;
  }

  if (wave == 0) {
    const uint32_t c = lane < nwords ? (uint32_t)__popcll(s_live[lane]) : 0u;
    const uint32_t incl = wave_incl_scan(c, AddOp(), 0u);
    s_rank[lane] = incl - c;
    if (lane == 63) b.info[2 * f] = incl;
  }
  __syncthreads();
  GpBox* out = b.out + (size_t)f * kGpMaxCand;
#pragma unroll
  for (int k = 0; k < kGpPer; k++) {
    if (!live[k]) continue;
    const uint32_t w = k * kGpWaves + wave;
    const uint32_t r = s_rank[w] + (uint32_t)__popcll(s_live[w] & ((1ull << lane) - 1));
    out[r] = gp_scaled(bx[k], by[k], bw[k], bh[k], bconf[k], bc[k].cls, sx, sy);
  }
}

hipError_t launch_gp_parse(const float* raw, size_t frame_stride, int nframes, int P, int C, float conf_thr,
                           float iou_thr, float sx, float sy, const GpParseBufs& b, hipStream_t st) {
  hipLaunchKernelGGL(k_gp_cand, dim3(((unsigned)P + 255u) / 256u, nframes), dim3(256), 0, st, raw, frame_stride, P, C,
                     conf_thr, b);
  hipLaunchKernelGGL(k_gp_nms, dim3(nframes), dim3(kGpNmsThreads), 0, st, raw, frame_stride, P, iou_thr, sx, sy, b);
  return hipGetLastError();
}

static size_t merge_lds_bytes(const Geom& g) { return (size_t)g.merge_lds; }

hipError_t prepare_kernels(const Geom& g) {
  if (!g.merge_cap) return hipSuccess;
  return hipFuncSetAttribute((const void*)k_ccl_merge<64>, hipFuncAttributeMaxDynamicSharedMemorySize,
                             kMergeLdsMax);
}

hipError_t launch_pipeline(const DevBufs& b, const Geom& g, const Params& prm, int B, int fmt, int nblobwg,
                           hipStream_t st, hipEvent_t* ev, hipStream_t st2, hipEvent_t fork, hipEvent_t join,
                           const KernelTimer* kt, const FieldLaunch* field) {
  int e = 0;
  auto on = [&](int stage) { return AT_PIPE_STOP(prm) <= 0 || stage < AT_PIPE_STOP(prm); };
  auto mark = [&]() {
    if (ev) (void)hipEventRecord(ev[e++], st);
  };
  hipError_t split_err = hipSuccess;
  auto tk = [&](int stage, hipStream_t s, int which) {
    if (!kt || kt->stage != stage) return;
    if (kt->split) {
      const hipError_t r = kt->split(kt->ctx, which);
      if (r != hipSuccess && split_err == hipSuccess) split_err = r;
    } else {
      (void)hipEventRecord(which ? kt->t1 : kt->t0, s);
    }
  };
  mark();
  {
    dim3 blk(64, 4), grd((g.TW + 63) / 64, (g.TH + 3) / 4, B);
    tk(0, st, 0);
    if (!on(0) || g.ctw == 32) {}
    else if (fmt == 0) hipLaunchKernelGGL(k_pre<0>, grd, blk, 0, st, b, g, prm.taps);
    else if (fmt == 1) hipLaunchKernelGGL(k_pre<1>, grd, blk, 0, st, b, g, 1);
    else hipLaunchKernelGGL(k_pre<2>, grd, blk, 0, st, b, g, prm.taps);
    tk(0, st, 1);
    if (on(0) && prm.gp_c && fmt == 1)
      hipLaunchKernelGGL(k_gp_pre, dim3((prm.gp_w + 63) / 64, (prm.gp_h + 3) / 4, B), dim3(64, 4), 0, st, b, g, prm);
  }
  mark();
  {
    dim3 grd(g.CTX, g.CTY, B);
    tk(1, st, 0);
    if (!on(1)) {}
    else if (g.ctw != 32) hipLaunchKernelGGL((k_thr_ccl<64, -1>), grd, dim3(CclTile<64>::NT), 0, st, b, g, prm);
    else if (fmt == 0) hipLaunchKernelGGL((k_thr_ccl<32, 0>), grd, dim3(CclTile<32>::NT), 0, st, b, g, prm);
    else if (fmt == 1) hipLaunchKernelGGL((k_thr_ccl<32, 1>), grd, dim3(CclTile<32>::NT), 0, st, b, g, prm);
    else hipLaunchKernelGGL((k_thr_ccl<32, 2>), grd, dim3(CclTile<32>::NT), 0, st, b, g, prm);
    tk(1, st, 1);
    mark();
    tk(2, st, 0);
    if (!on(2)) {}
    else if (g.ctw == 32) hipLaunchKernelGGL(k_ccl_border<32>, grd, dim3(BorderRoles<32>::NT), 0, st, b, g);
    else hipLaunchKernelGGL(k_ccl_merge<64>, dim3(B), dim3(1024), merge_lds_bytes(g), st, b, g, prm);
    tk(2, st, 1);
    mark();
  }
  tk(3, st, 0);
  if (on(3) && g.ctw == 32)
    hipLaunchKernelGGL(k_ccl_roots, dim3(g.CTX * g.CTY, B), dim3(64), 0, st, b, g);
  tk(3, st, 1);
  mark();
  {
    dim3 blk(64, 4), grd(g.BTX, g.BTY, B);
    tk(4, st, 0);
    if (!on(4)) {}
    else if (g.ctw != 32) hipLaunchKernelGGL(k_boundary<true>, grd, blk, 0, st, b, g);
    else hipLaunchKernelGGL(k_boundary<false>, grd, blk, 0, st, b, g);
    tk(4, st, 1);
    mark();
  }
  tk(5, st, 0);
  if (on(5)) hipLaunchKernelGGL(k_pairs, dim3(B), dim3(1024), 0, st, b, g, AT_PROBE_ON(prm));
  tk(5, st, 1);
  mark();
  tk(6, st, 0);
  if (on(6)) hipLaunchKernelGGL(k_group, dim3(g.ntb, B), dim3(256), 0, st, b, g);
  tk(6, st, 1);
  mark();
  tk(7, st, 0);
  const bool fuse_small = g.ctw == 32;
  const bool lat_fused = g.ctw == 32 && g.max_cluster <= 4096 && !ev && !kt;
  if (on(7) && !(g.ctw == 32 && g.max_cluster <= 4096)) hipLaunchKernelGGL(k_extents, dim3(std::max(16, std::min(AT_EXT_GRID, 96 * B))), dim3(256), 0, st, b, g);
  tk(7, st, 1);
  mark();
  auto blob_large = [&](hipStream_t s) {
    tk(9, s, 0);
    const bool cap4k = g.max_cluster <= 4096;
    if (!on(9)) return;
    if (lat_fused) {
      hipLaunchKernelGGL(k_blob_lat, dim3(nblobwg), dim3(512), 0, s, b, g, prm);
    } else if (g.ctw == 32 && cap4k) {
      hipLaunchKernelGGL((k_blob<512, 4096, true>), dim3(nblobwg), dim3(512), 0, s, b, g, prm, 0u, 0, g.nlarge, 0);
    } else if (B < kWideBlobMaxBatch || prm.wide_blob) {
      if (cap4k) hipLaunchKernelGGL((k_blob<512, 4096>), dim3(nblobwg), dim3(512), 0, s, b, g, prm, 0u, 0, g.nlarge, 0);
      else hipLaunchKernelGGL((k_blob<512, kSortCap>), dim3(nblobwg), dim3(512), 0, s, b, g, prm, 0u, 0, g.nlarge, 0);
    } else {
      const int lo = prm.lblob_wg ? std::min(prm.lblob_wg, nblobwg) : nblobwg;
      hipLaunchKernelGGL((k_blob<256, 4096>), dim3(lo), dim3(256), 0, s, b, g, prm, 0u, 0, g.nlarge - 1, 0);
      hipLaunchKernelGGL((k_blob_small<false, 1024, 3, 9>), dim3(nblobwg), dim3(256), 0, s, b, g, prm, g.nlarge - 1, g.nlarge, 1);
      if (!cap4k)
        hipLaunchKernelGGL((k_blob<AT_BIG_NT, kSortCap>), dim3(std::min(nblobwg, AT_BIG_BLOB_WG)), dim3(AT_BIG_NT), 0, s, b, g,
                           prm, 4096u, 0, 1, 2);
    }
    tk(9, s, 1);
  };
  auto blob_small = [&](hipStream_t s) {
    tk(8, s, 0);
    if (!on(8) || lat_fused) {}
    else if (fuse_small) hipLaunchKernelGGL(k_blob_small<true>, dim3(nblobwg * 2), dim3(256), 0, s, b, g, prm, g.nlarge, kNumCls, 0);
    else hipLaunchKernelGGL(k_blob_small<false>, dim3(prm.sblob_wg ? prm.sblob_wg : nblobwg * 2), dim3(256), 0, s, b, g, prm, g.nlarge, kNumCls, 0);
    tk(8, s, 1);
  };
  const int fin_c1 = g.ctw != 32 ? kNumCls : g.max_cluster > 4096 ? g.nlarge : 0;
  auto quad_fin = [&](hipStream_t s) {
    if (fin_c1 > 0 && on(9) && (!AT_DIAG_ANY(prm) || AT_DIAG_STOP(prm, 5)))
      hipLaunchKernelGGL(k_quad_fin, dim3(std::max(1, std::min(2048, 8 * B))), dim3(256), 0, s, b, g, prm, 0, fin_c1);
  };
  if (ev || !st2 || lat_fused) {
    blob_small(st);
    mark();
    blob_large(st);
    quad_fin(st);
    mark();
  } else {
    hipError_t e;
    if ((e = hipEventRecord(fork, st))) return e;
    if ((e = hipStreamWaitEvent(st2, fork, 0))) return e;
    if (AT_FORK_SMALL) {
      blob_large(st);
      blob_small(st2);
    } else {
      blob_small(st);
      blob_large(st2);
    }
    if ((e = hipEventRecord(join, st2))) return e;
    if ((e = hipStreamWaitEvent(st, join, 0))) return e;
    quad_fin(st);
  }
  const bool pose_fused = AT_POSE_IN_DECODE && prm.tag_size > 0 && on(11) && B < kWideBlobMaxBatch && !ev && b.kt_stage < 0 && !kt;
  tk(10, st, 0);
  {
    const dim3 grd(prm.dec_wg ? std::min(prm.dec_wg, decode_grid(nblobwg, B)) : decode_grid(nblobwg, B));
    const bool rows = g.ctw == 64 && !pose_fused && prm.dec_lpq != 64;
    if (on(10) && pose_fused) hipLaunchKernelGGL(k_decode<true>, grd, dim3(128), 0, st, b, g, prm, B, fmt);
    else if (on(10) && rows) hipLaunchKernelGGL((k_decode<false, kDecRowLanes>), grd, dim3(kDecodeThreads), 0, st, b, g, prm, B, fmt);
    else if (on(10)) hipLaunchKernelGGL(k_decode<false>, grd, dim3(kDecodeThreads), 0, st, b, g, prm, B, fmt);
  }
  tk(10, st, 1);
  mark();
  if (b.kt_stage >= 1 && b.kt_stage <= 10 && b.kt_stage != 3 && b.kt_stage != 5 && b.kt_stage != 6)
    hipLaunchKernelGGL(k_kt_span, dim3(kKtSpanWgs), dim3(256), 0, st, b);
  tk(11, st, 0);
  if (prm.tag_size > 0 && on(11) && !pose_fused) {
    if (B < kWideBlobMaxBatch) hipLaunchKernelGGL(k_pose<true>, dim3(32 * B), dim3(64), 0, st, b, prm);
    else hipLaunchKernelGGL(k_pose<false>, dim3(kPoseGroupsPerFrame * B), dim3(64), 0, st, b, prm);
  }
  tk(11, st, 1);
  mark();
  if (field && prm.tag_size > 0 && on(11)) {
    if (field->ev[0]) (void)hipEventRecord(field->ev[0], st);
    hipLaunchKernelGGL(k_field, dim3(B), dim3(64), 0, st, b, field->b, prm, B);
    if (field->ev[1]) (void)hipEventRecord(field->ev[1], st);
  }
  if (split_err != hipSuccess) return split_err;
  return hipGetLastError();
}

}
```

Before: 155,200.

## Move segment line fits and quad combo search into a new k_fit_quads kernel

In the non-fused blob path, blob_item now stops after computing the prefix moments and writes them to a per-blob FitPend record. It no longer does the segment line fits, the 4-corner combination search and the final fit in place. A new k_fit_quads kernel runs those steps with 16 lanes per blob, keeping the segment fits as float4 in LDS, and then does the corner intersection and quad validation. Separately, the extents and blob_small kernels now pass wave-uniform values through readfirstlane and use 32-bit key arithmetic. The aim is to shorten the busy blob kernel and give the fit work better lane utilisation. The cost is larger per-blob global records (800 B instead of 80 B) and reduced fit-result precision.

```diff
diff --git a/ros_vision_amd/csrc/at_api.cpp b/ros_vision_amd/csrc/at_api.cpp
--- a/ros_vision_amd/csrc/at_api.cpp
+++ b/ros_vision_amd/csrc/at_api.cpp
@@ -510,7 +510,7 @@
   b.dets = (DevDetection*)dalloc(B * kMaxDets * sizeof(DevDetection));
   b.det_work = (uint32_t*)dalloc(B * kMaxDets * 4);
   b.quads = (QuadRecord*)dalloc(B * kMaxPairs * sizeof(QuadRecord));
-  b.qpend = (QuadPend*)dalloc(B * kMaxPairs * sizeof(QuadPend));
+  b.fpend = (FitPend*)dalloc(B * kMaxPairs * sizeof(FitPend));
   d->kstamp_word = (kCtlPerFrame * B + kCtlScalars + 1) & ~(size_t)1;
   d->ctrl_words = d->kstamp_word + 5;
   d->d_ctrl = (uint32_t*)dalloc(((d->ctrl_words * 4 + 15) / 16) * 16);
diff --git a/ros_vision_amd/csrc/at_common.h b/ros_vision_amd/csrc/at_common.h
--- a/ros_vision_amd/csrc/at_common.h
+++ b/ros_vision_amd/csrc/at_common.h
@@ -182,12 +182,15 @@
   int32_t N;
 };
 
-struct QuadPend {
-  float fit[4][4];
-  uint32_t blob_index, valid;
-  uint16_t indices[4];
-};
-static_assert(sizeof(QuadPend) == 80, "QuadPend: 80 B per kept blob");
+struct alignas(16) FitPend {
+  uint32_t n, cnt, blob_index;
+  uint16_t pi[kNMaxima];
+  uint32_t tMx[21], tMy[21], tW[21];
+  uint32_t pad0;
+  uint64_t tMxx[21], tMyy[21], tMxy[21];
+  uint64_t pad1;
+};
+static_assert(sizeof(FitPend) == 800, "FitPend: 800 B per kept blob");
 
 
 struct JpgBufs {
@@ -269,7 +272,7 @@
   uint32_t* ctrl;
   uint32_t ctrl_words;
   QuadRecord* quads;
-  QuadPend* qpend;
+  FitPend* fpend;
   uint32_t* npts;
   uint32_t* npairs;
   uint32_t* ndets;
diff --git a/ros_vision_amd/csrc/at_kernels.hip b/ros_vision_amd/csrc/at_kernels.hip
--- a/ros_vision_amd/csrc/at_kernels.hip
+++ b/ros_vision_amd/csrc/at_kernels.hip
@@ -68,6 +68,10 @@
 
 __device__ __forceinline__ uint32_t wave_read_next(uint32_t v) {
   return (uint32_t)__builtin_amdgcn_update_dpp(0, (int)v, 0x130, 0xf, 0xf, false);
+}
+
+__device__ __forceinline__ uint32_t wave_uniform(uint32_t v) {
+  return (uint32_t)__builtin_amdgcn_readfirstlane((int)v);
 }
 
 template <typename T>
@@ -2422,7 +2426,63 @@
   double err[kNMaxima][kNMaxima];
   double mse[kNMaxima][kNMaxima];
   double p[kNMaxima][kNMaxima][2];
+  __device__ __forceinline__ void put(int a, int bb, const LineFitOut& o) {
+    err[a][bb] = o.err; mse[a][bb] = o.mse; p[a][bb][0] = o.p23[0]; p[a][bb][1] = o.p23[1];
+  }
+  __device__ __forceinline__ double e(int a, int bb) const { return err[a][bb]; }
+  __device__ __forceinline__ double m(int a, int bb) const { return mse[a][bb]; }
+  __device__ __forceinline__ double nx(int a, int bb) const { return p[a][bb][0]; }
+  __device__ __forceinline__ double ny(int a, int bb) const { return p[a][bb][1]; }
 };
+struct SegFitsF {
+  float4 v[kNMaxima][kNMaxima];
+  __device__ __forceinline__ void put(int a, int bb, const LineFitOut& o) {
+    v[a][bb] = make_float4((float)o.err, (float)o.mse, (float)o.p23[0], (float)o.p23[1]);
+  }
+  __device__ __forceinline__ double e(int a, int bb) const { return (double)v[a][bb].x; }
+  __device__ __forceinline__ double m(int a, int bb) const { return (double)v[a][bb].y; }
+  __device__ __forceinline__ double nx(int a, int bb) const { return (double)v[a][bb].z; }
+  __device__ __forceinline__ double ny(int a, int bb) const { return (double)v[a][bb].w; }
+};
+
+template <typename P>
+__device__ __forceinline__ Moments seg_moments(const P& S, uint32_t n, int a, int bb) {
+  const uint32_t i0 = (uint32_t)S.pi[a], i1 = (uint32_t)S.pi[bb];
+  Mom6 m = Mom6{S.tMx[bb], S.tMy[bb], S.tW[bb], S.tMxx[bb], S.tMyy[bb], S.tMxy[bb]};
+  const Mom6 pm = Mom6{S.tMx[10 + a], S.tMy[10 + a], S.tW[10 + a], S.tMxx[10 + a], S.tMyy[10 + a], S.tMxy[10 + a]};
+  int32_t N;
+  if (i0 < i1) {
+    if (i0 > 0) mom_sub(m, pm);
+    N = (int32_t)(i1 - i0 + 1);
+  } else {
+    Mom6 z = Mom6{S.tMx[20], S.tMy[20], S.tW[20], S.tMxx[20], S.tMyy[20], S.tMxy[20]};
+    mom_sub(z, pm);
+    mom_add(z, m);
+    m = z;
+    N = (int32_t)(n - i0 + i1 + 1);
+  }
+  return to_moments(m, N);
+}
+
+template <typename SF>
+__device__ __forceinline__ double combo_err(const SF& seg, uint32_t cb, double mse_max, double cos_critical) {
+  const int m0 = cb & 0xff, m1 = (cb >> 8) & 0xff, m2 = (cb >> 16) & 0xff, m3 = cb >> 24;
+  double e4 = DBL_MAX;
+  if (!(seg.m(m0, m1) > mse_max)) {
+    if (!(seg.m(m1, m2) > mse_max)) {
+      const double dot = seg.nx(m0, m1) * seg.nx(m1, m2) + seg.ny(m0, m1) * seg.ny(m1, m2);
+      if (!(fabs(dot) > cos_critical)) {
+        if (!(seg.m(m2, m3) > mse_max) && !(seg.m(m3, m0) > mse_max))
+          e4 = seg.e(m0, m1) + seg.e(m1, m2) + seg.e(m2, m3) + seg.e(m3, m0);
+      }
+    }
+  }
+  return e4;
+}
+
+__device__ __forceinline__ int num_combos(int cnt) {
+  return cnt < 4 ? 0 : cnt >= kNMaxima ? 210 : (cnt * (cnt - 1) * (cnt - 2) * (cnt - 3)) / 24;
+}
 
 template <int NT, int CAP>
 struct BlobShared {
@@ -3298,6 +3358,24 @@
     else if (k < 20) { need = k - 10 < cnt && k - 10 < kNMaxima && S.pi[k - 10] > 0; idx = need ? (uint32_t)S.pi[k - 10] - 1 : 0; }
     else if (k == 20) { need = true; idx = n - 1; }
     const Mom6 p = prefix_at<NT, CAP>(S, cw, cbase, c, idx, need);
+    if constexpr (!FUSE) {
+      FitPend& fp = b.fpend[(size_t)f * kMaxPairs + rank];
+      if (need) {
+        fp.tMx[k] = p.Mx; fp.tMy[k] = p.My; fp.tW[k] = p.W;
+        fp.tMxx[k] = p.Mxx; fp.tMyy[k] = p.Myy; fp.tMxy[k] = p.Mxy;
+      }
+      if (k < kNMaxima) fp.pi[k] = (uint16_t)S.pi[k];
+      if (tid == 0) {
+        fp.n = n;
+        fp.cnt = npk;
+        fp.blob_index = bi;
+        pacc[21] += 1;
+      }
+      phase(6);
+      phase(9);
+      team_sync<NT>();
+      return;
+    }
     if (need) {
       S.tMx[k] = p.Mx; S.tMy[k] = p.My; S.tW[k] = p.W;
       S.tMxx[k] = p.Mxx; S.tMyy[k] = p.Myy; S.tMxy[k] = p.Mxy;
@@ -3305,23 +3383,6 @@
   }
   team_sync<NT>();
   phase(6);
-  auto seg_moments = [&](int a, int bb) -> Moments {
-    const uint32_t i0 = (uint32_t)S.pi[a], i1 = (uint32_t)S.pi[bb];
-    Mom6 m = Mom6{S.tMx[bb], S.tMy[bb], S.tW[bb], S.tMxx[bb], S.tMyy[bb], S.tMxy[bb]};
-    const Mom6 pm = Mom6{S.tMx[10 + a], S.tMy[10 + a], S.tW[10 + a], S.tMxx[10 + a], S.tMyy[10 + a], S.tMxy[10 + a]};
-    int32_t N;
-    if (i0 < i1) {
-      if (i0 > 0) mom_sub(m, pm);
-      N = (int32_t)(i1 - i0 + 1);
-    } else {
-      Mom6 z = Mom6{S.tMx[20], S.tMy[20], S.tW[20], S.tMxx[20], S.tMyy[20], S.tMxy[20]};
-      mom_sub(z, pm);
-      mom_add(z, m);
-      m = z;
-      N = (int32_t)(n - i0 + i1 + 1);
-    }
-    return to_moments(m, N);
-  };
   SegFits& seg = *reinterpret_cast<SegFits*>(S.keys);
   static_assert(sizeof(SegFits) <= sizeof(S.keys), "segment fits must fit over the keys");
   const int cn = min(cnt, kNMaxima);
@@ -3329,11 +3390,7 @@
   for (int ci = tid; cnt >= 4 && ci < cn * cn; ci += NT) {
     const int a = (int)(((float)ci + 0.5f) * rcn), bb = ci - a * cn;
     if (a != bb) {
-      const LineFitOut o = fit_line_v<false, true>(seg_moments(a, bb));
-      seg.err[a][bb] = o.err;
-      seg.mse[a][bb] = o.mse;
-      seg.p[a][bb][0] = o.p23[0];
-      seg.p[a][bb][1] = o.p23[1];
+      seg.put(a, bb, fit_line_v<false, true>(seg_moments(S, n, a, bb)));
     }
   }
   team_sync<NT>();
@@ -3342,24 +3399,10 @@
   double err = DBL_MAX;
   uint32_t bt = 0xffffffffu;
   const double mse_max = (double)prm.max_line_fit_mse;
-  const int ncomb = cnt < 4 ? 0 : cnt >= kNMaxima ? 210 : (cnt * (cnt - 1) * (cnt - 2) * (cnt - 3)) / 24;
+  const int ncomb = num_combos(cnt);
   for (int cj = tid; cj < ncomb; cj += NT) {
-    double e4 = DBL_MAX;
     const int ci = (int)combo[210 + cj];
-    {
-      const uint32_t cb = combo[ci];
-      const int m0 = cb & 0xff, m1 = (cb >> 8) & 0xff, m2 = (cb >> 16) & 0xff, m3 = cb >> 24;
-      if (!(seg.mse[m0][m1] > mse_max)) {
-        if (!(seg.mse[m1][m2] > mse_max)) {
-          const double dot =
-              seg.p[m0][m1][0] * seg.p[m1][m2][0] + seg.p[m0][m1][1] * seg.p[m1][m2][1];
-          if (!(fabs(dot) > prm.cos_critical_rad)) {
-            if (!(seg.mse[m2][m3] > mse_max) && !(seg.mse[m3][m0] > mse_max))
-              e4 = seg.err[m0][m1] + seg.err[m1][m2] + seg.err[m2][m3] + seg.err[m3][m0];
-          }
-        }
-      }
-    }
+    const double e4 = combo_err(seg, combo[ci], mse_max, prm.cos_critical_rad);
     if (bt == 0xffffffffu || e4 < err || (e4 == err && (uint32_t)ci < bt)) { err = e4; bt = (uint32_t)ci; }
   }
 #pragma unroll
@@ -3384,28 +3427,9 @@
   uint16_t qidx[4];
   const uint32_t cbt = combo[bt];
   for (int k = 0; k < 4; k++) qidx[k] = (uint16_t)S.pi[(cbt >> (8 * k)) & 0xff];
-  if constexpr (!FUSE) {
-    QuadPend& qp = b.qpend[(size_t)f * kMaxPairs + rank];
-    if (valid && tid < 4) {
-      float pre[4];
-      double e_, m_;
-      fit_line(seg_moments((cbt >> (8 * tid)) & 0xff, (cbt >> (8 * ((tid + 1) & 3))) & 0xff), nullptr, nullptr, &e_, &m_,
-               pre);
-      *reinterpret_cast<float4*>(qp.fit[tid]) = make_float4(pre[0], pre[1], pre[2], pre[3]);
-    }
-    if (tid == 0) {
-      qp.blob_index = bi;
-      qp.valid = valid;
-      for (int k = 0; k < 4; k++) qp.indices[k] = qidx[k];
-      pacc[21] += 1;
-    }
-    phase(9);
-    team_sync<NT>();
-    return;
-  }
   if (valid && tid < 4) {
     const LineFitOut o =
-        fit_line_v<true, true>(seg_moments((cbt >> (8 * tid)) & 0xff, (cbt >> (8 * ((tid + 1) & 3))) & 0xff));
+        fit_line_v<true, true>(seg_moments(S, n, (cbt >> (8 * tid)) & 0xff, (cbt >> (8 * ((tid + 1) & 3))) & 0xff));
     S.lines[tid][0] = o.p01[0];
     S.lines[tid][1] = o.p01[1];
     S.lines[tid][2] = o.p23[0];
@@ -3529,12 +3553,12 @@
 }
 
 template <int NT>
-__device__ __forceinline__ void extents_item(const DevBufs& b, const Geom& g, uint32_t w, int64_t (*red)[8]) {
-  const int tid = team_rank<NT>();
+__device__ __forceinline__ void extents_item(const DevBufs& b, const Geom& g, uint32_t w, uint32_t n, uint32_t off,
+                                             int64_t (*red)[8]) {
+  const uint32_t tid = (uint32_t)team_rank<NT>();
   const int f = (int)(w >> 16);
   const uint32_t rank = w & 0xffff;
-  const uint32_t n = b.pair_cnt[(size_t)f * kMaxPairs + rank];
-  const size_t so = (size_t)f * g.cap_pts + b.pair_off[(size_t)f * kMaxPairs + rank];
+  const size_t so = (size_t)f * g.cap_pts + off;
   const uint32_t* grp = b.grp + so;
   uint64_t* keys = b.keys + so;
   const uint8_t* dec = b.dec + (size_t)f * g.Wd * g.Hd;
@@ -3604,9 +3628,11 @@
   if (!keep) return;
   if (tid == 0) b.pair_sel[(size_t)f * kMaxPairs + rank] = 1;
   const double cx = ext_cx(e), cy = ext_cy(e);
+  const uint32_t Wd = (uint32_t)g.Wd;
   for (uint32_t base = 0; base < n; base += NT * U) {
     uint32_t kk[U];
     uint32_t gp[U];
+    uint32_t pxy[U];
 #pragma unroll
     for (int u = 0; u < U; u++) {
       const uint32_t t = base + u * NT + tid;
@@ -3614,37 +3640,37 @@
     }
 #pragma unroll
     for (int u = 0; u < U; u++) {
-      const uint64_t k = kk[u];
+      const uint32_t k = kk[u];
       const int dxy = (int)(k & 3);
-      const int32_t ix = (int32_t)(((k >> 14) & 0x3ff) * 2 + dx_of(dxy) + 1) / 2;
-      const int32_t iy = (int32_t)(((k >> 4) & 0x3ff) * 2 + dy_of(dxy) + 1) / 2;
-      const bool in = base + u * NT + tid < n && ix > 0 && ix + 1 < g.Wd && iy > 0 && iy + 1 < g.Hd;
-      const int32_t at = in ? iy * g.Wd + ix : g.Wd + 1;
-      gp[u] = (uint32_t)dec[at - 1] | ((uint32_t)dec[at + 1] << 8) | ((uint32_t)dec[at - g.Wd] << 16) |
-              ((uint32_t)dec[at + g.Wd] << 24);
+      const uint32_t px = ((k >> 14) & 0x3ff) * 2 + dx_of(dxy), py = ((k >> 4) & 0x3ff) * 2 + dy_of(dxy);
+      const uint32_t ix = (px + 1) / 2, iy = (py + 1) / 2;
+      const bool img = ix > 0 && ix + 1 < Wd && iy > 0 && iy + 1 < (uint32_t)g.Hd;
+      const bool in = base + u * NT + tid < n && img;
+      pxy[u] = (px & 0xfff) | ((py & 0xfff) << 12) | ((uint32_t)img << 31);
+      const uint32_t at = in ? iy * Wd + ix : Wd + 1;
+      const uint8_t* hp = dec + (at - 1);
+      gp[u] = (uint32_t)hp[0] | ((uint32_t)hp[2] << 8) | ((uint32_t)dec[at - Wd] << 16) | ((uint32_t)dec[at + Wd] << 24);
     }
 #pragma unroll AT_EXT_KEY_UNROLL
     for (int u = 0; u < U; u++) {
       const uint32_t t = base + u * NT + tid;
       if (t >= n) continue;
-      const uint64_t k = kk[u];
-      const int dxy = (int)(k & 3);
+      const uint32_t k = kk[u];
+      const uint32_t dxy = k & 3;
       const uint32_t bx = (k >> 14) & 0x3ff, by = (k >> 4) & 0x3ff;
-      const uint32_t px = bx * 2 + dx_of(dxy), py = by * 2 + dy_of(dxy);
+      const uint32_t px = pxy[u] & 0xfff, py = (pxy[u] >> 12) & 0xfff;
       const float dyf = (float)((double)py - cy);
       const float dxf = (float)((double)px - cx);
       const float theta = (float)(((double)det_atan2f(dyf, dxf) + 3.14159265358979323846) * 8e6);
-      long long ti = (long long)rintf(theta);
-      if (ti < 0) ti = 0;
-      const int32_t ix = (int32_t)(px + 1) / 2, iy = (int32_t)(py + 1) / 2;
+      const uint32_t ti = (uint32_t)max((int32_t)rintf(theta), 0);
       int32_t Wt = 1;
-      if (ix > 0 && ix + 1 < g.Wd && iy > 0 && iy + 1 < g.Hd) {
+      if (pxy[u] >> 31) {
         const int32_t gxv = (int32_t)((gp[u] >> 8) & 0xff) - (int32_t)(gp[u] & 0xff);
         const int32_t gyv = (int32_t)(gp[u] >> 24) - (int32_t)((gp[u] >> 16) & 0xff);
         Wt = lf_weight(gxv, gyv);
       }
-      keys[t] = ((uint64_t)(ti & 0xfffffff) << kKeyTheta) | ((uint64_t)dxy << 30) | ((uint64_t)by << 20) |
-               ((uint64_t)bx << 10) | (((k >> 3) & 1) << 9) | (uint64_t)Wt;
+      const uint32_t lo = (dxy << 30) | (by << 20) | (bx << 10) | (((k >> 3) & 1) << 9) | (uint32_t)Wt;
+      keys[t] = ((uint64_t)(ti & 0xfffffff) << kKeyTheta) | lo;
     }
   }
 }
@@ -3668,14 +3694,17 @@
   for (uint32_t it = blockIdx.x; it < nlarge; it += gridDim.x) {
     uint32_t w = 0;
     work_item(b, cnt, 0, kNumCls, it, &w);
-    extents_item<256>(b, g, w, s_red);
+    const size_t pr = (size_t)(w >> 16) * kMaxPairs + (w & 0xffff);
+    extents_item<256>(b, g, w, b.pair_cnt[pr], b.pair_off[pr], s_red);
   }
   if (g.ctw != 32) {
-    const uint32_t gw = blockIdx.x * 4 + (threadIdx.x >> 6), nw = gridDim.x * 4;
+    const uint32_t gw = blockIdx.x * 4 + wave_uniform(threadIdx.x >> 6), nw = gridDim.x * 4;
     for (uint32_t it = nlarge + gw; it < total; it += nw) {
       uint32_t w = 0;
       work_item(b, cnt, 0, kNumCls, it, &w);
-      extents_item<64>(b, g, w, nullptr);
+      w = wave_uniform(w);
+      const size_t pr = (size_t)(w >> 16) * kMaxPairs + (w & 0xffff);
+      extents_item<64>(b, g, w, wave_uniform(b.pair_cnt[pr]), wave_uniform(b.pair_off[pr]), nullptr);
     }
   }
   __syncthreads();
@@ -3744,19 +3773,24 @@
   if (lane == 0) S.slow_dt = 0;
   uint32_t nwork = 0;
   for (int c = c0; c < c1; c++) nwork += s_cnt[c];
-  uint32_t item = wv;
+  auto uni = [](uint32_t v) { return FUSE ? v : wave_uniform(v); };
+  auto uni_pair = [&](const PairInfo& p) { return PairInfo{uni(p.n), uni(p.off), uni(p.sel)}; };
+  uint32_t item = uni(wv);
   uint32_t w = 0, w1 = 0;
   PairInfo pi = {0, 0, 0};
   if (item < nwork) {
     work_item(b, s_cnt, c0, c1, item, &w);
-    pi = load_pair_info(b, w);
+    w = uni(w);
+    pi = uni_pair(load_pair_info(b, w));
   }
   if (item + nwaves < nwork) work_item(b, s_cnt, c0, c1, item + nwaves, &w1);
   for (; item < nwork; item += nwaves) {
     const bool has1 = item + nwaves < nwork;
+    w1 = uni(w1);
     const PairInfo pi1 = has1 ? load_pair_info(b, w1) : PairInfo{0, 0, 0};
     uint32_t w2 = 0;
     if (item + 2 * nwaves < nwork) work_item(b, s_cnt, c0, c1, item + 2 * nwaves, &w2);
+    pi = uni_pair(pi);
     [[clang::always_inline]] blob_item<64, CAP, FUSE>(b, g, prm, S, nullptr, s_combo, w, pi, pacc);
     w = w1;
     pi = pi1;
@@ -3795,7 +3829,7 @@
 __global__ __launch_bounds__(256) __attribute__((amdgpu_waves_per_eu(FUSE ? 2 : WAVES))) void k_blob_small(DevBufs b, Geom g, Params prm,
                                                                                                          int c0, int c1, int launch) {
   __shared__ BlobShared<64, CAP> Ss[4];
-  const int wave = threadIdx.x >> 6;
+  const int wave = FUSE ? (int)(threadIdx.x >> 6) : (int)wave_uniform(threadIdx.x >> 6);
   uint32_t kt_slot = ~0u;
   if (!launch) {
     kt_begin(b, STAGE);
@@ -3840,112 +3874,200 @@
   }
 }
 
-__global__ __launch_bounds__(256) void k_quad_fin(DevBufs b, Geom g, Params prm, int c0, int c1) {
-  __shared__ uint32_t s_cnt[kNumCls];
+struct FitRow {
+  FitPend rec;
+  SegFitsF seg;
+};
+constexpr int kFitFwd = kNMaxima * (kNMaxima - 1) / 2, kFitCls = (kNMaxima - 3) * (kNMaxima - 2) / 2;
+#ifndef AT_FQ_ITEMS
+#define AT_FQ_ITEMS 32
+#endif
+__global__ __launch_bounds__(256) void k_fit_quads(DevBufs b, Geom g, Params prm, int c0, int c1) {
+  __shared__ FitRow s_row[16];
+  __shared__ uint32_t s_combo[420], s_cnt[kNumCls];
+  __shared__ uint16_t s_pair[kFitFwd + kFitCls];
+  load_combos(s_combo, threadIdx.x, 256);
+  if (threadIdx.x < kFitFwd) {
+    int bb = 1;
+    while (bb * (bb + 1) / 2 <= (int)threadIdx.x) bb++;
+    s_pair[threadIdx.x] = (uint16_t)((threadIdx.x - bb * (bb - 1) / 2) | (bb << 8));
+  } else if (threadIdx.x < kFitFwd + kFitCls) {
+    const int u = (int)threadIdx.x - kFitFwd;
+    int a = 3;
+    while ((a - 2) * (a - 1) / 2 <= u) a++;
+    s_pair[threadIdx.x] = (uint16_t)(a | ((u - (a - 3) * (a - 2) / 2) << 8));
+  }
   if (threadIdx.x < kNumCls) s_cnt[threadIdx.x] = min(b.ncls[threadIdx.x], b.wcap);
   __syncthreads();
   uint32_t nwork = 0;
   for (int c = c0; c < c1; c++) nwork += s_cnt[c];
-  const uint32_t lane = lane_id(), base = lane & ~3u;
-  const int k = (int)(lane & 3);
+  const uint32_t lane = lane_id(), base = lane & ~15u;
+  const int rl = (int)(lane & 15), row = (int)(lane >> 4);
+  const int k = rl & 3;
+  const uint32_t wv = wave_uniform(blockIdx.x * 4 + (threadIdx.x >> 6));
+  FitRow& R = s_row[threadIdx.x >> 4];
+  const double mse_max = (double)prm.max_line_fit_mse;
   auto from = [&](double v, int j) { return __shfl(v, (int)base + j); };
   auto fromf = [&](float v, int j) { return __shfl(v, (int)base + j); };
   auto quad_or = [&](int v) {
     v |= __shfl_xor(v, 1);
     return v | __shfl_xor(v, 2);
   };
-  for (uint32_t it = (blockIdx.x * 256 + threadIdx.x) >> 2; it < nwork; it += gridDim.x * 64) {
-    uint32_t w = 0;
-    work_item(b, s_cnt, c0, c1, it, &w);
-    const uint32_t f = w >> 16, rank = w & 0xffff;
-    const size_t slot = (size_t)f * kMaxPairs + rank;
-    if (b.pair_sel[slot] == 0) continue;
-    const QuadPend& qp = b.qpend[slot];
-    const bool valid = qp.valid != 0;
-    float cx = 0.f, cy = 0.f;
-    int bad = 0;
-    {
-      double l[4] = {0, 0, 0, 0};
-      if (valid) {
-        const float4 pre = *reinterpret_cast<const float4*>(qp.fit[k]);
-        l[0] = (double)pre.z;
-        l[1] = (double)pre.w;
-        line_normal(pre.x, pre.y, det_hypotf(pre.x, pre.y), l + 2);
-      }
-      double m[4];
-#pragma unroll
-      for (int j = 0; j < 4; j++) m[j] = from(l[j], (k + 1) & 3);
-      if (valid) {
-        const double A00 = l[3], A01 = -m[3];
-        const double A10 = -l[2], A11 = m[2];
-        const double B0 = -l[0] + m[0];
-        const double B1 = -l[1] + m[1];
-        const double det = A00 * A11 - A10 * A01;
-        const double W00 = A11 / det, W01 = -A01 / det;
-        if (fabs(det) < 0.001) {
-          bad = 1;
-        } else {
-          const double L0 = W00 * B0 + W01 * B1;
-          cx = (float)(l[0] + L0 * A00);
-          cy = (float)(l[1] + L0 * A10);
+  for (uint32_t it0 = wv * AT_FQ_ITEMS; it0 < nwork; it0 += gridDim.x * 4 * AT_FQ_ITEMS) {
+    uint32_t wl = 0;
+    bool sel = false;
+    if (lane < AT_FQ_ITEMS && it0 + lane < nwork) {
+      work_item(b, s_cnt, c0, c1, it0 + lane, &wl);
+      sel = b.pair_sel[(size_t)(wl >> 16) * kMaxPairs + (wl & 0xffff)] != 0;
+    }
+    uint64_t todo = __ballot(sel);
+    while (todo) {
+      int src = -1;
+#pragma unroll
+      for (int r = 0; r < 4; r++) {
+        if (todo) {
+          if (row == r) src = __builtin_ctzll(todo);
+          todo &= todo - 1;
         }
       }
-    }
-    bool ok = valid && !quad_or(bad);
-    float qc[4][2];
-#pragma unroll
-    for (int j = 0; j < 4; j++) {
-      qc[j][0] = fromf(cx, j);
-      qc[j][1] = fromf(cy, j);
-    }
-    if (ok) {
-      auto side = [&](int j) {
-        const int a2 = j == 0 ? 0 : j == 1 ? 1 : j == 2 ? 2 : j == 3 ? 2 : j == 4 ? 3 : 0;
-        const int b2 = j == 0 ? 1 : j == 1 ? 2 : j == 2 ? 0 : j == 3 ? 3 : j == 4 ? 0 : 2;
-        return det_hypotf(qc[b2][0] - qc[a2][0], qc[b2][1] - qc[a2][1]);
-      };
-      const float s0 = side(k), s1 = side(4 + (k & 1));
-      float len[6];
-#pragma unroll
-      for (int j = 0; j < 4; j++) len[j] = fromf(s0, j);
-      len[4] = fromf(s1, 0);
-      len[5] = fromf(s1, 1);
-      float area = 0, pp;
-      pp = (len[0] + len[1] + len[2]) / 2;
-      area += sqrtf(pp * (pp - len[0]) * (pp - len[1]) * (pp - len[2]));
-      pp = (len[3] + len[4] + len[5]) / 2;
-      area += sqrtf(pp * (pp - len[3]) * (pp - len[4]) * (pp - len[5]));
-      if ((double)area < 0.95 * g.min_tag_width * g.min_tag_width) ok = false;
-    }
-    if (ok) {
-      const int i0 = k, i1 = (i0 + 1) & 3, i2 = (i0 + 2) & 3;
-      const float dx1 = qc[i1][0] - qc[i0][0], dy1 = qc[i1][1] - qc[i0][1];
-      const float dx2 = qc[i2][0] - qc[i1][0], dy2 = qc[i2][1] - qc[i1][1];
-      const float cosd = (dx1 * dx2 + dy1 * dy2) / sqrtf((dx1 * dx1 + dy1 * dy1) * (dx2 * dx2 + dy2 * dy2));
-      const int abad = (double)fabsf(cosd) > prm.cos_critical_rad || dx1 * dy2 < dy1 * dx2;
-      if (quad_or(abad)) ok = false;
-    }
-    if (k == 0) {
-      QuadRecord rec;
-      rec.blob_index = qp.blob_index;
-      rec.valid = valid;
-      for (int j = 0; j < 4; j++) rec.indices[j] = qp.indices[j];
-      QuadCand qcand;
-      for (int j = 0; j < 4; j++) {
-        const float x = ok ? (qc[j][0] - 0.5f) * 2.0f + 0.5f : 0.f;
-        const float y = ok ? (qc[j][1] - 0.5f) * 2.0f + 0.5f : 0.f;
-        rec.corners[j][0] = qcand.p[j][0] = x;
-        rec.corners[j][1] = qcand.p[j][1] = y;
-      }
-      rec.accepted = ok;
-      if (prm.taps) b.quads[slot] = rec;
-      if (ok && !AT_DIAG_STOP(prm, 5)) {
-        qcand.frame = f;
-        qcand.rank = rank;
-        const uint32_t ci = atomicAdd(b.nqcand + (size_t)f * kQcStride, 1u);
-        if (ci < (uint32_t)kQuadCandPerFrame) b.qcand[(size_t)f * kQuadCandPerFrame + ci] = qcand;
-        else atomicOr(b.status + f, kStatusQuadsOverflow);
-      }
+      const bool live = src >= 0;
+      const uint32_t w = __shfl(wl, live ? src : 0);
+      const uint32_t f = w >> 16, rank = w & 0xffff;
+      const size_t slot = (size_t)f * kMaxPairs + rank;
+      if (live) {
+        const uint4* rec4 = reinterpret_cast<const uint4*>(b.fpend + slot);
+        uint4* lds4 = reinterpret_cast<uint4*>(&R.rec);
+        for (int j = rl; j < (int)(sizeof(FitPend) / 16); j += 16) lds4[j] = rec4[j];
+      }
+      wave_sync();
+      const uint32_t n = live ? R.rec.n : 0;
+      const int cnt = live ? (int)R.rec.cnt : 0;
+      const int cn = min(cnt, kNMaxima);
+      const int nfwd = cnt >= 4 ? cn * (cn - 1) / 2 : 0;
+      const int nfit = cnt >= 4 ? nfwd + (cn - 3) * (cn - 2) / 2 : 0;
+      for (int ci = rl; ci < nfit; ci += 16) {
+        const uint32_t ab = s_pair[ci < nfwd ? ci : kFitFwd + ci - nfwd];
+        const int a = (int)(ab & 0xff), bb = (int)(ab >> 8);
+        const Moments mo = seg_moments(R.rec, n, a, bb);
+        LineFitOut o;
+        o.p23[0] = o.p23[1] = 0.0;
+        if (ci < nfwd) o = fit_line_v<false, true>(mo);
+        else fit_line(mo, nullptr, nullptr, &o.err, &o.mse);
+        R.seg.put(a, bb, o);
+      }
+      wave_sync();
+      if (AT_DIAG_STOP(prm, 7)) continue;
+      double err = DBL_MAX;
+      uint32_t bt = 0xffffffffu;
+      const int ncomb = num_combos(cnt);
+      for (int cj = rl; cj < ncomb; cj += 16) {
+        const int ci = (int)s_combo[210 + cj];
+        const double e4 = combo_err(R.seg, s_combo[ci], mse_max, prm.cos_critical_rad);
+        if (bt == 0xffffffffu || e4 < err || (e4 == err && (uint32_t)ci < bt)) { err = e4; bt = (uint32_t)ci; }
+      }
+#pragma unroll
+      for (int d = 8; d > 0; d >>= 1) {
+        const double oe = __shfl_xor(err, d);
+        const uint32_t ot = __shfl_xor(bt, d);
+        if (oe < err || (oe == err && ot < bt)) { err = oe; bt = ot; }
+      }
+      if (AT_DIAG_STOP(prm, 8)) continue;
+      if (bt >= 210) bt = 0;
+      const bool valid = live && err < (double)(prm.max_line_fit_mse * (float)n);
+      const uint32_t cbt = s_combo[bt];
+      if (live && rl < 4) {
+        float cx = 0.f, cy = 0.f;
+        int bad = 0;
+        {
+          double l[4] = {0, 0, 0, 0};
+          if (valid) {
+            float pre[4];
+            double e_, m_;
+            fit_line(seg_moments(R.rec, n, (cbt >> (8 * k)) & 0xff, (cbt >> (8 * ((k + 1) & 3))) & 0xff), nullptr, nullptr, &e_,
+                     &m_, pre);
+            l[0] = (double)pre[2];
+            l[1] = (double)pre[3];
+            line_normal(pre[0], pre[1], det_hypotf(pre[0], pre[1]), l + 2);
+          }
+          double m[4];
+#pragma unroll
+          for (int j = 0; j < 4; j++) m[j] = from(l[j], (k + 1) & 3);
+          if (valid) {
+            const double A00 = l[3], A01 = -m[3];
+            const double A10 = -l[2], A11 = m[2];
+            const double B0 = -l[0] + m[0];
+            const double B1 = -l[1] + m[1];
+            const double det = A00 * A11 - A10 * A01;
+            const double W00 = A11 / det, W01 = -A01 / det;
+            if (fabs(det) < 0.001) {
+              bad = 1;
+            } else {
+              const double L0 = W00 * B0 + W01 * B1;
+              cx = (float)(l[0] + L0 * A00);
+              cy = (float)(l[1] + L0 * A10);
+            }
+          }
+        }
+        bool ok = valid && !quad_or(bad);
+        float qc[4][2];
+#pragma unroll
+        for (int j = 0; j < 4; j++) {
+          qc[j][0] = fromf(cx, j);
+          qc[j][1] = fromf(cy, j);
+        }
+        auto qx = [&](int i) { return fromf(cx, i); };
+        auto qy = [&](int i) { return fromf(cy, i); };
+        if (ok) {
+          auto side = [&](int j) {
+            const int a2 = j == 0 ? 0 : j == 1 ? 1 : j == 2 ? 2 : j == 3 ? 2 : j == 4 ? 3 : 0;
+            const int b2 = j == 0 ? 1 : j == 1 ? 2 : j == 2 ? 0 : j == 3 ? 3 : j == 4 ? 0 : 2;
+            return det_hypotf(qx(b2) - qx(a2), qy(b2) - qy(a2));
+          };
+          const float s0 = side(k), s1 = side(4 + (k & 1));
+          float len[6];
+#pragma unroll
+          for (int j = 0; j < 4; j++) len[j] = fromf(s0, j);
+          len[4] = fromf(s1, 0);
+          len[5] = fromf(s1, 1);
+          float area = 0, pp;
+          pp = (len[0] + len[1] + len[2]) / 2;
+          area += sqrtf(pp * (pp - len[0]) * (pp - len[1]) * (pp - len[2]));
+          pp = (len[3] + len[4] + len[5]) / 2;
+          area += sqrtf(pp * (pp - len[3]) * (pp - len[4]) * (pp - len[5]));
+          if ((double)area < 0.95 * g.min_tag_width * g.min_tag_width) ok = false;
+        }
+        if (ok) {
+          const int i0 = k, i1 = (i0 + 1) & 3, i2 = (i0 + 2) & 3;
+          const float dx1 = qx(i1) - qx(i0), dy1 = qy(i1) - qy(i0);
+          const float dx2 = qx(i2) - qx(i1), dy2 = qy(i2) - qy(i1);
+          const float cosd = (dx1 * dx2 + dy1 * dy2) / sqrtf((dx1 * dx1 + dy1 * dy1) * (dx2 * dx2 + dy2 * dy2));
+          const int abad = (double)fabsf(cosd) > prm.cos_critical_rad || dx1 * dy2 < dy1 * dx2;
+          if (quad_or(abad)) ok = false;
+        }
+        if (k == 0) {
+          QuadRecord rec;
+          rec.blob_index = R.rec.blob_index;
+          rec.valid = valid;
+          for (int j = 0; j < 4; j++) rec.indices[j] = R.rec.pi[(cbt >> (8 * j)) & 0xff];
+          QuadCand qcand;
+          for (int j = 0; j < 4; j++) {
+            const float x = ok ? (qc[j][0] - 0.5f) * 2.0f + 0.5f : 0.f;
+            const float y = ok ? (qc[j][1] - 0.5f) * 2.0f + 0.5f : 0.f;
+            rec.corners[j][0] = qcand.p[j][0] = x;
+            rec.corners[j][1] = qcand.p[j][1] = y;
+          }
+          rec.accepted = ok;
+          if (prm.taps) b.quads[slot] = rec;
+          if (ok && !AT_DIAG_STOP(prm, 5)) {
+            qcand.frame = f;
+            qcand.rank = rank;
+            const uint32_t ci = atomicAdd(b.nqcand + (size_t)f * kQcStride, 1u);
+            if (ci < (uint32_t)kQuadCandPerFrame) b.qcand[(size_t)f * kQuadCandPerFrame + ci] = qcand;
+            else atomicOr(b.status + f, kStatusQuadsOverflow);
+          }
+        }
+      }
+      wave_sync();
     }
   }
 }
@@ -6433,8 +6555,8 @@
   };
   const int fin_c1 = g.ctw != 32 ? kNumCls : g.max_cluster > 4096 ? g.nlarge : 0;
   auto quad_fin = [&](hipStream_t s) {
-    if (fin_c1 > 0 && on(9) && (!AT_DIAG_ANY(prm) || AT_DIAG_STOP(prm, 5)))
-      hipLaunchKernelGGL(k_quad_fin, dim3(std::max(1, std::min(2048, 8 * B))), dim3(256), 0, s, b, g, prm, 0, fin_c1);
+    if (fin_c1 > 0 && on(9) && (!AT_DIAG_ANY(prm) || AT_DIAG_STOP(prm, 5) || AT_DIAG_STOP(prm, 7) || AT_DIAG_STOP(prm, 8)))
+      hipLaunchKernelGGL(k_fit_quads, dim3(std::max(1, std::min(2048, 8 * B))), dim3(256), 0, s, b, g, prm, 0, fin_c1);
   };
   if (ev || !st2 || lat_fused) {
     blob_small(st);
```

After: 160,900 (median of 6 runs). +3.7%, better.
